# Wenri/taichi_3d_gaussian_splatting

Measured on AMD Instinct MI355X. Metric: fps fwd+bwd @1920x1080 (run as 1920x1088), 5e5 Gaussians, higher is better.
Workload: dtype f32; 1 GPU; cfg3_headline: synth(N=500000, 1920x1088, sigma0=0.02, sh_deg=3, seed 0), fwd+bwd, 1 view(s) per GPU per step, the 8 poses of BASELINE config 4 cycled (rank r, step k: pose (r + k) mod 8); points=500000, parallelism=view-parallel x1, 1 view(s) per rank per step, all-reduce per step, views_per_rank=1, poses_cycled=8, forward_sizing=predicted, rehearsal=False, backward_hook=True

## Files before the change

### taichi_3d_gaussian_splatting_amd/csrc/gs_api.hip

```cpp
#include "../../include/gs_channels.h"
#include "../../include/gs_sparse.h"
#include "gs_host.h"
#include "gs_sort_key.h"

#include <algorithm>
#include <atomic>
#include <chrono>
#include <cstring>
#include <cstdlib>

thread_local std::string g_last_error;

struct FrameBufs {
    DevBuf mask, ids, cam_index, rec, box, ntiles, depth_codes, offsets, keys_a, keys_b, vals_a, vals_b, tile_start, pose, tile_order, cuts, cut_mag;
    void release(int64_t* total)
    {
        DevBuf* all[] = { &mask, &ids, &cam_index, &rec, &box, &ntiles, &depth_codes, &offsets, &keys_a, &keys_b, &vals_a, &vals_b,
                          &tile_start, &pose, &tile_order, &cuts, &cut_mag };
        for (DevBuf* b : all) b->release(total);
    }
};

struct Frame {
    FrameBufs bufs;
    gs_frame_info info{};
    int depth_bits = 0;
    void* keys_sorted = nullptr;
    int key_bytes = 4;
    int32_t* vals_sorted = nullptr;
    bool live = false;
    int cut_cap = 0;
    int bwd_reference_order = 0;
    int n_objects = 0;
    bool rgb_only = false;
    bool max_tiles_known = false;
    uint32_t generation = 0;
    uint64_t bwd_serial = 0;
    int pending_slot = -1;
    int32_t pending_ticket = 0;
    hipStream_t pending_stream = nullptr;
};

int gs_prof_begin(GsProf* p, int kid, hipStream_t s)
{
    if (!p || !((p->mask >> kid) & 1ull)) return -1;
    GsProf::Rec r; r.kid = kid;
    hipEvent_t* ev[2] = { &r.a, &r.b };
    for (hipEvent_t* e : ev) {
        if (!p->spare.empty()) { *e = p->spare.back(); p->spare.pop_back(); }
        else if (hipEventCreate(e) != hipSuccess) return -1;
    }
    (void)hipEventRecord(r.a, s);
    p->recs.push_back(r);
    return (int)p->recs.size() - 1;
}

void gs_prof_end(GsProf* p, int rec, hipStream_t s)
{
    if (!p || rec < 0) return;
    (void)hipEventRecord(p->recs[rec].b, s);
}

extern "C" int gs_abi_version(void) { return GS_ABI_VERSION; }
extern "C" const char* gs_last_error(void) { return g_last_error.c_str(); }

extern "C" const char* gs_kernel_names(void)
{
    return "k_filter,k_scan_tiles_publish,k_project,k_keygen,k_sort_hist,"
           "k_sort_rowscan,k_sort_scatter,k_blend_fwd,k_blend_bwd_tile,k_bwd_points,k_sum_rows,k_tile_order,k_blend_bwd_repair";
}

extern "C" int gs_create(int32_t device, gs_ctx** out)
{
    if (!out) return fail(GS_ERR_INVALID_ARGUMENT, "gs_create: out is NULL");
    int count = 0;
    HIP_TRY(hipGetDeviceCount(&count));
    if (device < 0 || device >= count) return fail(GS_ERR_INVALID_ARGUMENT, "gs_create: no such HIP device");
    HIP_TRY(hipSetDevice(device));
    gs_ctx* c = new gs_ctx();
    c->device = device;
    hipError_t e = hipHostMalloc(reinterpret_cast<void**>(&c->host_counters), sizeof(GsCounters) * GS_COUNTER_SLOTS, hipHostMallocMapped | hipHostMallocCoherent);
    if (e != hipSuccess) { delete c; return fail(GS_ERR_HIP, std::string("hipHostMalloc: ") + hipGetErrorString(e)); }
    std::memset(c->host_counters, 0, sizeof(GsCounters) * GS_COUNTER_SLOTS);
    e = hipHostGetDevicePointer(reinterpret_cast<void**>(&c->host_counters_dev), c->host_counters, 0);
    if (e != hipSuccess) { (void)hipHostFree(c->host_counters); delete c; return fail(GS_ERR_HIP, std::string("hipHostGetDevicePointer: ") + hipGetErrorString(e)); }
    e = c->counters.ensure(sizeof(GsCounters), &c->device_bytes);
    if (e == hipSuccess) e = hipMemset(c->counters.p, 0, sizeof(GsCounters));
    if (e == hipSuccess) e = hipEventCreateWithFlags(&c->switch_event, hipEventDisableTiming);
    if (e != hipSuccess) { c->counters.release(&c->device_bytes); (void)hipHostFree(c->host_counters); delete c; return fail(GS_ERR_OUT_OF_MEMORY, "gs_create: counters"); }
    *out = c;
    return GS_OK;
}

extern "C" int gs_destroy(gs_ctx* c)
{
    if (!c) return GS_OK;
    (void)hipSetDevice(c->device);
    (void)hipDeviceSynchronize();
    for (Frame* f : c->frames) { f->bufs.release(&c->device_bytes); delete f; }
    DevBuf* all[] = { &c->block_counts, &c->block_offsets, &c->tile_block_sums, &c->hist, &c->scan_tmp, &c->first_hist,
                      &c->counters, &c->partial, &c->visited, &c->zero_row, &c->sums, &c->loss_ws, &c->order_hint, &c->pose_scratch,
                      &c->ch_partial, &c->ch_flags, &c->row_block_totals, &c->merge_tags, &c->merge_ids,
                      &c->knn_sort, &c->knn_hist, &c->knn_points, &c->knn_tree, &c->mix_records, &c->mix_sums, &c->mix_partial,
                      &c->mixg_queries, &c->mixg_partial, &c->mixg_sums, &c->mixg_x_partial, &c->mcmc_ws, &c->appearance_ws, &c->bilateral_ws, &c->depth_ws,
                      &c->geometry_ws };
    for (DevBuf* b : all) b->release(&c->device_bytes);
    for (ResampleTable* rt : c->resample_tables) { rt->buf.release(&c->device_bytes); delete rt; }
    for (GsProf::Rec& r : c->prof.recs) { (void)hipEventDestroy(r.a); (void)hipEventDestroy(r.b); }
    for (hipEvent_t e : c->prof.spare) (void)hipEventDestroy(e);
    if (c->switch_event) (void)hipEventDestroy(c->switch_event);
    if (c->host_counters) (void)hipHostFree(c->host_counters);
    delete c;
    return GS_OK;
}

extern "C" int gs_profile_enable(gs_ctx* c, uint64_t kernel_mask)
{
    if (!c) return fail(GS_ERR_INVALID_ARGUMENT, "gs_profile_enable: ctx is NULL");
    std::lock_guard<std::mutex> lock(c->mu);
    c->prof.mask = kernel_mask;
    return GS_OK;
}

extern "C" int gs_profile_read(gs_ctx* c, double* total_ms, int64_t* launches, int32_t n, int32_t reset)
{
    if (!c || !total_ms || !launches) return fail(GS_ERR_INVALID_ARGUMENT, "gs_profile_read: NULL argument");
    std::lock_guard<std::mutex> lock(c->mu);
    HIP_TRY(hipSetDevice(c->device));
    GsProf& p = c->prof;
    for (GsProf::Rec& r : p.recs) {
        HIP_TRY(hipEventSynchronize(r.b));
        float ms = 0.0f;
        HIP_TRY(hipEventElapsedTime(&ms, r.a, r.b));
        p.total_ms[r.kid] += ms; p.launches[r.kid] += 1;
        p.spare.push_back(r.a); p.spare.push_back(r.b);
    }
    p.recs.clear();
    for (int i = 0; i < n && i < KID_COUNT_; ++i) { total_ms[i] = p.total_ms[i]; launches[i] = p.launches[i]; }
    if (reset) for (int i = 0; i < KID_COUNT_; ++i) { p.total_ms[i] = 0.0; p.launches[i] = 0; }
    return GS_OK;
}

extern "C" int64_t gs_ctx_device_bytes(const gs_ctx* c) { return c ? c->device_bytes : 0; }
extern "C" int64_t gs_ctx_counter_wait_ns(const gs_ctx* c) { return c ? c->counter_wait_ns : 0; }
static gs_frame* ticket_of(int slot, uint32_t generation)
{
    return reinterpret_cast<gs_frame*>((uintptr_t)(((uint64_t)generation << 32) | (uint64_t)(uint32_t)(slot + 1)));
}

static Frame* resolve(gs_ctx* c, const gs_frame* h)
{
    const uint64_t v = (uint64_t)(uintptr_t)h;
    const uint32_t lo = (uint32_t)v, gen = (uint32_t)(v >> 32);
    if (lo == 0 || lo > c->frames.size()) return nullptr;
    Frame* f = c->frames[lo - 1];
    if (!f->live || f->generation != gen) return nullptr;
    return f;
}

static Frame* acquire_frame(gs_ctx* c, int* slot)
{
    for (size_t i = 0; i < c->frames.size(); ++i)
        if (!c->frames[i]->live) { Frame* f = c->frames[i]; f->live = true; f->generation += 1; if (f->generation == 0) f->generation = 1; *slot = (int)i; return f; }
    Frame* f = new Frame();
    f->live = true; f->generation = 1;
    c->frames.push_back(f);
    *slot = (int)c->frames.size() - 1;
    return f;
}

static void drop_frame(gs_ctx* c, Frame* f)
{
    if (!f || !f->live) return;
    if (f->pending_slot > 0) c->slots_busy &= ~(1ull << f->pending_slot);
    f->pending_slot = -1;
    f->live = false;
    for (size_t i = 0; i < c->frames.size(); ++i) if (c->frames[i] == f && c->transient == (int)i) c->transient = -1;
}

static Frame* begin_frame(gs_ctx* c, const gs_camera* cam, int T, int keep, int* slot)
{
    if (c->transient >= 0) drop_frame(c, c->frames[c->transient]);
    Frame* f = acquire_frame(c, slot);
    f->info = gs_frame_info{};
    f->bwd_serial = 0;
    f->info.kept_for_backward = keep ? 1 : 0;
    f->info.n_tiles = T; f->info.camera_height = cam->camera_height; f->info.camera_width = cam->camera_width;
    return f;
}

static void finish_frame(gs_ctx* c, Frame* f, int slot, int64_t N, int M, uint32_t K, int stages, gs_frame** frame_out)
{
    f->info.n_points = N; f->info.n_points_in_camera = M; f->info.n_keys = K;
    f->info.stages = stages;
    if (!f->info.kept_for_backward) c->transient = slot;
    *frame_out = ticket_of(slot, f->generation);
}

static GsFrameView frame_view(const Frame& f)
{
    const FrameBufs& B = f.bufs;
    const int T = f.info.n_tiles;
    GsFrameView v{};
    float4* rec = B.rec.as<float4>();
    v.PA = rec; v.PB = rec + 1; v.PC = rec + 2; v.PD = rec + 3;
    v.box = B.box.as<ushort4>(); v.ntiles = B.ntiles.as<int32_t>(); v.depth_codes = B.depth_codes.as<int32_t>(); v.offsets = B.offsets.as<uint32_t>();
    v.ids = B.ids.as<int32_t>(); v.cam_index = B.cam_index.as<int32_t>(); v.mask = B.mask.as<int8_t>(); v.pose = B.pose.as<GsPose>();
    v.T = T;
    int32_t* tiles = B.tile_start.as<int32_t>();
    v.tile_start = tiles; v.tile_end = tiles + T; v.tile_work = tiles + 2 * (size_t)T; v.tile_cut = tiles + 3 * (size_t)T;
    v.max_tiles = tiles + GS_TILE_INTS(T) - GS_TILE_SPARE_MAX_TILES;
    v.tile_ints = (int)GS_TILE_INTS(T);
    v.tile_order = B.tile_order.as<int32_t>(); v.n_heavy = v.tile_order + T;
    v.keys_sorted = f.keys_sorted; v.vals_sorted = f.vals_sorted;
    v.cuts = f.cut_cap > 0 ? B.cuts.as<float4>() : nullptr; v.cut_mag = B.cut_mag.as<float2>();
    return v;
}

static int waves_per_tile(int n_tiles);
static int bits_for(uint32_t v) { int b = 0; while (v) { ++b; v >>= 1; } return b < 1 ? 1 : b; }

static int read_counters(gs_ctx* c, hipStream_t s, int32_t ticket, int slot, GsCounters* out)
{
    volatile GsCounters* hc = c->host_counters + slot;
    const auto t0 = std::chrono::steady_clock::now();
    for (uint32_t spin = 0; hc->reserved != ticket; ++spin) {
        if ((spin & 0xfffu) == 0xfffu) {
            const hipError_t q = hipStreamQuery(s);
            if (q == hipSuccess) {
                if (hc->reserved != ticket) return fail(GS_ERR_HIP, "frame counters were not published");
                break;
            }
            if (q != hipErrorNotReady) return fail(GS_ERR_HIP, std::string("waiting for the frame counters: ") + hipGetErrorString(q));
            if (std::chrono::steady_clock::now() - t0 > std::chrono::seconds(30))
                return fail(GS_ERR_HIP, "timed out waiting for the frame counters");
        }
    }
    std::atomic_thread_fence(std::memory_order_acquire);
    c->counter_wait_ns += std::chrono::duration_cast<std::chrono::nanoseconds>(std::chrono::steady_clock::now() - t0).count();
    *out = c->host_counters[slot];
    if (out->bad_object_ids != 0)
        return fail(GS_ERR_INVALID_ARGUMENT, "point_object_id holds " + std::to_string(out->bad_object_ids) +
                                             " value(s) outside [0, n_objects) on valid rows");
    return GS_OK;
}

static int resolve_pending(gs_ctx* c, Frame* f)
{
    if (f->pending_slot <= 0) return GS_OK;
    HIP_TRY(hipSetDevice(c->device));
    GsCounters hc;
    const int rc = read_counters(c, f->pending_stream, f->pending_ticket, f->pending_slot, &hc);
    if (rc != GS_OK) { drop_frame(c, f); return rc; }
    c->slots_busy &= ~(1ull << f->pending_slot);
    f->pending_slot = -1;
    f->info.n_points_in_camera = hc.M;
    f->info.n_keys = hc.K;
    return GS_OK;
}

static int lookup(gs_ctx* c, const gs_frame* h, const char* who, bool pending, Frame** out)
{
    Frame* f = resolve(c, h);
    if (!f) return fail(GS_ERR_STATE, who, "not a live frame of this context");
    if (pending)
        if (const int rc = resolve_pending(c, f)) return rc;
    *out = f;
    return GS_OK;
}

static int check_geometry(const gs_camera* cam, const gs_config* cfg, const char* who, int* tiles_x, int* tiles_y)
{
    const int H = cam->camera_height, W = cam->camera_width;
    if (W <= 0 || H <= 0 || (!cfg->allow_partial_tiles && (W % GS_TILE != 0 || H % GS_TILE != 0)))
        return fail(GS_ERR_INVALID_ARGUMENT, who, "camera_width and camera_height must be positive multiples of 16 "
                                             "(or set gs_config.allow_partial_tiles)");
    *tiles_x = (W + GS_TILE - 1) / GS_TILE; *tiles_y = (H + GS_TILE - 1) / GS_TILE;
    if (*tiles_x > 65535 || *tiles_y > 65535) return fail(GS_ERR_INVALID_ARGUMENT, who, "image too large");
    return GS_OK;
}

static int check_scene(const gs_scene* sc, const gs_camera* cam, const char* who)
{
    const int64_t N = sc->n_points;
    if (N < 0 || N >= (int64_t)1 << 31) return fail(GS_ERR_INVALID_ARGUMENT, who, "n_points out of range");
    if (cam->n_objects <= 0) return fail(GS_ERR_INVALID_ARGUMENT, who, "n_objects must be >= 1");
    if (N > 0 && (!sc->point_cloud || !sc->point_cloud_features || !sc->point_invalid_mask || !sc->point_object_id))
        return fail(GS_ERR_INVALID_ARGUMENT, who, "NULL scene array");
    if (!cam->q_pointcloud_camera || !cam->t_pointcloud_camera || !cam->camera_intrinsics)
        return fail(GS_ERR_INVALID_ARGUMENT, who, "NULL camera array");
    if (((uintptr_t)sc->point_cloud_features & 15u) != 0)
        return fail(GS_ERR_INVALID_ARGUMENT, who, "point_cloud_features must be 16-byte aligned");
    return GS_OK;
}

static int check_forward_out(const gs_forward_out* out, const gs_config* cfg, int keep, const char* who)
{
    if (!out->rasterized_image) return fail(GS_ERR_INVALID_ARGUMENT, who, "rasterized_image is NULL");
    if (!cfg->rgb_only && (!out->rasterized_depth || !out->pixel_accumulated_alpha ||
                           !out->pixel_offset_of_last_effective_point || !out->pixel_valid_point_count))
        return fail(GS_ERR_INVALID_ARGUMENT, who, "an output is NULL although rgb_only is false");
    if (keep && cfg->rgb_only) return fail(GS_ERR_INVALID_ARGUMENT, who, "rgb_only frames cannot be kept for backward (RAST:478-484)");
    return GS_OK;
}

#define GS_FIRST_PASS_MAX_BLOCKS 4096
static bool sort_first_pass_enabled(int64_t rows)
{
    if ((rows + 255) / 256 > GS_FIRST_PASS_MAX_BLOCKS) return false;
    const char* e = getenv("GS_SORT_FIRST_PASS");
    return !(e && e[0] == '0');
}

#define GS_NARROW_KEYS_DEFAULT 1
enum NarrowKeys { NARROW_OFF, NARROW_ON, NARROW_REQUIRED };
static NarrowKeys sort_narrow_keys()
{
    const char* e = getenv("GS_SORT_NARROW_KEYS");
    if (!e || !e[0]) return GS_NARROW_KEYS_DEFAULT ? NARROW_ON : NARROW_OFF;
    if (e[0] == '0') return NARROW_OFF;
    return strcmp(e, "require") == 0 ? NARROW_REQUIRED : NARROW_ON;
}
static int check_required_key_class(const Frame* f)
{
    if (sort_narrow_keys() == NARROW_REQUIRED && f->key_bytes != 2)
        return fail(GS_ERR_STATE, "GS_SORT_NARROW_KEYS=require: the frame's sort keys are " + std::to_string(f->key_bytes) + " bytes wide");
    return GS_OK;
}

enum CounterWait { WAIT_NOW, WAIT_LATER, WAIT_FRAME };

static int run_project_stage(gs_ctx* c, Frame* f, const gs_scene* sc, const gs_camera* cam, const gs_config* cfg, hipStream_t s,
                             CounterWait wait, GsProjectArgs* pa_out, int* M_out, uint32_t* K_out)
{
    FrameBufs& B = f->bufs;
    const int64_t N = sc->n_points;
    const int T = f->info.n_tiles;
    const size_t nb = (size_t)((N + 255) / 256);
    const size_t Np = (size_t)(N > 0 ? N : 1);
    int rc = grow(c, "forward", { NEED(B.mask, Np), NEED(B.ids, 4 * Np), NEED(B.cam_index, 4 * Np),
                       NEED(B.rec, 64 * Np),
                       NEED(B.box, 8 * Np), NEED(B.ntiles, 4 * Np), NEED(B.depth_codes, 4 * Np), NEED(B.offsets, 4 * Np),
                       NEED(B.tile_start, 4 * GS_TILE_INTS(T)),
                       NEED(B.tile_order, 4 * GS_ORDER_INTS(T)),
                       NEED(B.pose, sizeof(GsPose) * (size_t)cam->n_objects),
                       NEED(c->block_counts, 4 * (nb + 1)), NEED(c->block_offsets, 4 * (nb + 1)),
                       NEED(c->tile_block_sums, 4 * (nb + 1)) });
    if (rc != GS_OK) return rc;
    const bool first_pass = wait == WAIT_LATER && sort_first_pass_enabled(N);
    if (first_pass && (rc = grow(c, "forward", { NEED(c->first_hist, 4 * gs_first_hist_elems(N)) })) != GS_OK) return rc;
    f->n_objects = cam->n_objects;

    GsProjectArgs pa{};
    pa.prof = &c->prof;
    pa.point_cloud = sc->point_cloud; pa.features = sc->point_cloud_features; pa.invalid = sc->point_invalid_mask;
    pa.object_id = sc->point_object_id; pa.N = N; pa.q_pc = cam->q_pointcloud_camera; pa.t_pc = cam->t_pointcloud_camera;
    pa.n_objects = cam->n_objects; pa.Kmat = cam->camera_intrinsics; pa.H = cam->camera_height; pa.W = cam->camera_width;
    pa.near_plane = cfg->near_plane; pa.far_plane = cfg->far_plane; pa.depth_scale = cfg->depth_to_sort_key_scale;
    pa.v = frame_view(*f);
    pa.block_counts = c->block_counts.as<int32_t>(); pa.block_offsets = c->block_offsets.as<int32_t>();
    pa.tile_block_sums = c->tile_block_sums.as<uint32_t>();
    pa.first_hist = first_pass ? c->first_hist.as<uint32_t>() : nullptr;
    pa.counters = c->counters.as<GsCounters>();
    int slot = 0;
    if (wait == WAIT_FRAME && N > 0) {
        const uint64_t free_slots = ~c->slots_busy;
        if (free_slots != 0ull) { slot = __builtin_ctzll(free_slots); c->slots_busy |= 1ull << slot; }
    }
    pa.host_mirror = c->host_counters_dev + slot; pa.ticket = ++c->ticket;
    if (c->ticket == 0x7fffffff) c->ticket = 0;
    gs_launch_project(pa, s, wait != WAIT_LATER);
    f->max_tiles_known = true;
    HIP_TRY(hipGetLastError());
    *pa_out = pa;
    *M_out = 0; *K_out = 0u;
    if (slot > 0) {
        f->pending_slot = slot; f->pending_ticket = pa.ticket; f->pending_stream = s;
        return GS_OK;
    }
    if (N > 0 && wait != WAIT_LATER) {
        GsCounters hc;
        if ((rc = read_counters(c, s, pa.ticket, 0, &hc)) != GS_OK) return rc;
        *M_out = hc.M; *K_out = hc.K;
    }
    return GS_OK;
}

static int run_records_stage(gs_ctx* c, Frame* f, const float* records, int64_t m, const gs_config* cfg, hipStream_t s,
                             GsProjectArgs* pa_out)
{
    FrameBufs& B = f->bufs;
    const int T = f->info.n_tiles;
    const size_t Mp = (size_t)(m > 0 ? m : 1);
    const size_t nb = (size_t)((m + 255) / 256);
    const int rc = grow(c, "forward", { NEED(B.rec, 64 * Mp), NEED(B.box, 8 * Mp), NEED(B.ntiles, 4 * Mp), NEED(B.depth_codes, 4 * Mp), NEED(B.offsets, 4 * Mp),
                             NEED(B.tile_start, 4 * GS_TILE_INTS(T)), NEED(B.tile_order, 4 * GS_ORDER_INTS(T)),
                             NEED(c->tile_block_sums, 4 * (nb + 1)) });
    if (rc != GS_OK) return rc;
    const bool first_pass = sort_first_pass_enabled(m);
    if (first_pass) if (const int rc2 = grow(c, "forward", { NEED(c->first_hist, 4 * gs_first_hist_elems(m)) })) return rc2;
    if (m > 0) HIP_TRY(hipMemcpyAsync(B.rec.p, records, (size_t)m * 64, hipMemcpyDeviceToDevice, s));
    GsProjectArgs pa{};
    pa.prof = &c->prof; pa.N = m; pa.H = f->info.camera_height; pa.W = f->info.camera_width; pa.depth_scale = cfg->depth_to_sort_key_scale;
    pa.v = frame_view(*f);
    pa.tile_block_sums = c->tile_block_sums.as<uint32_t>();
    pa.first_hist = first_pass ? c->first_hist.as<uint32_t>() : nullptr;
    pa.counters = c->counters.as<GsCounters>();
    pa.host_mirror = c->host_counters_dev; pa.ticket = ++c->ticket;
    if (c->ticket == 0x7fffffff) c->ticket = 0;
    gs_launch_boxes_from_records(pa, (int)m, s, false);
    f->max_tiles_known = false;
    HIP_TRY(hipGetLastError());
    *pa_out = pa;
    return GS_OK;
}

static int run_raster_stage(gs_ctx* c, Frame* f, const GsProjectArgs& pa, int64_t n_rows, int M_bound, uint32_t K_bound, int depth_bits,
                            const gs_config* cfg, const gs_forward_out* out, hipStream_t s, bool publish)
{
    FrameBufs& B = f->bufs;
    const int T = f->info.n_tiles, H = f->info.camera_height, W = f->info.camera_width, tiles_x = (W + GS_TILE - 1) / GS_TILE;
    static const int seg_env = []{ const char* e = getenv("GS_BWD_SEGMENTS"); return e ? (e[0] == '0' ? 0 : 1) : -1; }();
    const bool want_cuts = seg_env >= 0 ? seg_env == 1 : (int64_t)T * waves_per_tile(T) < 6144;
    int cut_cap = 0;
    if (want_cuts && f->info.kept_for_backward && !cfg->rgb_only && K_bound > 0) {
        cut_cap = (int)std::min<uint64_t>((uint64_t)K_bound / GS_SEG + (uint64_t)T + 2, 0x7fffffffu);
        if (const int rc = grow(c, "forward", { NEED(B.cuts, (size_t)cut_cap * 256 * sizeof(float4)), NEED(B.cut_mag, (size_t)cut_cap * 256 * sizeof(float2)) }))
            return rc;
    }
    f->cut_cap = cut_cap;
    const int tile_bits = bits_for((uint32_t)(T > 1 ? T - 1 : 1));
    uint32_t* const first_hist = depth_bits >= 8 ? pa.first_hist : nullptr;
    const int key_bytes = gs_key_bytes(depth_bits + tile_bits, depth_bits, first_hist != nullptr, sort_narrow_keys() != NARROW_OFF);
    if (depth_bits + tile_bits > 63) return fail(GS_ERR_INVALID_ARGUMENT, "sort key needs more than 63 bits");
    const size_t Kp = K_bound > 0 ? K_bound : 1;
    const size_t hist_elems = gs_sort_hist_elems(K_bound);
    if (const int rc = grow(c, "forward", { NEED(B.keys_a, (size_t)key_bytes * Kp), NEED(B.keys_b, (size_t)key_bytes * Kp), NEED(B.vals_a, 4 * Kp), NEED(B.vals_b, 4 * Kp),
                                 NEED(c->hist, 4 * hist_elems), NEED(c->scan_tmp, 4 * GS_SORT_DIGITS) }))
        return rc;

    GsBinArgs ba{};
    ba.prof = &c->prof;
    ba.N = n_rows; ba.M = M_bound; ba.K = K_bound; ba.counters = c->counters.as<GsCounters>();
    ba.tiles_x = tiles_x;
    ba.depth_bits = depth_bits; ba.key_bits = depth_bits + tile_bits;
    ba.v = frame_view(*f);
    ba.tile_block_sums = pa.tile_block_sums;
    ba.counters_rw = pa.counters; ba.host_mirror = publish ? pa.host_mirror : nullptr; ba.ticket = pa.ticket;
    ba.block_offsets = pa.block_offsets; ba.block_counts = pa.block_counts;
    ba.keys_a = B.keys_a.p; ba.keys_b = B.keys_b.p; ba.key_bytes = key_bytes;
    ba.vals_a = B.vals_a.as<int32_t>(); ba.vals_b = B.vals_b.as<int32_t>();
    ba.hist = c->hist.as<uint32_t>(); ba.scan_tmp = c->scan_tmp.as<uint32_t>();
    ba.first_hist = first_hist;
    ba.keys_sorted = &f->keys_sorted; ba.vals_sorted = &f->vals_sorted;
    gs_launch_binning(ba, s);
    HIP_TRY(hipGetLastError());

    GsBlendFwdArgs fa{};
    fa.prof = &c->prof;
    fa.H = H; fa.W = W; fa.tiles_x = tiles_x; fa.rgb_only = cfg->rgb_only;
    fa.v = frame_view(*f);
    fa.key_bytes = key_bytes; fa.depth_bits = depth_bits; fa.K = K_bound; fa.counters = ba.counters;
    fa.image = out->rasterized_image; fa.depth = out->rasterized_depth; fa.acc_alpha = out->pixel_accumulated_alpha;
    fa.last = out->pixel_offset_of_last_effective_point; fa.count = out->pixel_valid_point_count;
    fa.cut_cap = cut_cap;
    static const bool use_hint = []{ const char* e = getenv("GS_FWD_ORDER_HINT"); return !(e && e[0] == '0'); }();
    fa.order_hint = (use_hint && c->order_hint_T == T && T > 0) ? c->order_hint.as<int32_t>() : nullptr;
    gs_launch_blend_fwd(fa, s);
    HIP_TRY(hipGetLastError());
    f->depth_bits = depth_bits;
    f->key_bytes = key_bytes;
    f->info.sort_key_bits = depth_bits + tile_bits;
    return GS_OK;
}

static int run_forward_tail(gs_ctx* c, Frame* f, const GsProjectArgs& pa, int64_t n_rows, int M_known, const gs_config* cfg,
                            const gs_forward_out* out, hipStream_t s, int* M_out, uint32_t* K_out)
{
    static const bool predict = []{ const char* e = getenv("GS_PREDICT_SIZES"); return !(e && e[0] == '0'); }();
    const int T = f->info.n_tiles, H = f->info.camera_height, W = f->info.camera_width;
    int rc;
    f->info.sizing = GS_SIZING_EXACT;
    *M_out = 0; *K_out = 0u;
    if (n_rows == 0) {
        rc = run_raster_stage(c, f, pa, 0, 0, 0u, 1, cfg, out, s, false);
        return rc != GS_OK ? rc : check_required_key_class(f);
    }
    const int tile_bits = bits_for((uint32_t)(T > 1 ? T - 1 : 1));
    bool predicted = false;
    int bits_p = 0; uint32_t K_p = 0;
    if (predict && c->seen.valid && c->seen.H == H && c->seen.W == W) {
        bits_p = bits_for((uint32_t)(c->seen.max_code + c->seen.max_code / 4));
        const uint64_t want = (uint64_t)c->seen.K + c->seen.K / 4 + 4096;
        K_p = (uint32_t)std::min<uint64_t>(want, 0x7fffffffu);
        predicted = K_p > 0 && bits_p + tile_bits <= 63;
    }
    if (predicted) {
        if ((rc = run_raster_stage(c, f, pa, n_rows, M_known >= 0 ? M_known : (int)n_rows, K_p, bits_p, cfg, out, s, true)) != GS_OK) return rc;
    } else {
        gs_launch_publish(pa, (int)((n_rows + 255) / 256), s);
        HIP_TRY(hipGetLastError());
    }
    GsCounters hc;
    if ((rc = read_counters(c, s, pa.ticket, 0, &hc)) != GS_OK) return rc;
    if (hc.K >= (1u << 31)) return fail(GS_ERR_INVALID_ARGUMENT, "more than 2^31 sort pairs (tile ranges are int32, RAST:954-957)");
    const int bits = bits_for((uint32_t)(hc.max_depth_code > 0 ? hc.max_depth_code : 0));
    if (predicted && hc.K <= K_p && bits <= bits_p) {
        f->info.sizing = GS_SIZING_PREDICTED;
    } else {
        if (predicted) {
            HIP_TRY(hipMemsetAsync(pa.v.tile_start, 0, sizeof(int32_t) * (size_t)pa.v.tile_ints, s));
            f->max_tiles_known = false;
            f->info.sizing = GS_SIZING_REDONE;
        }
        if ((rc = run_raster_stage(c, f, pa, n_rows, hc.M, hc.K, bits, cfg, out, s, false)) != GS_OK) return rc;
    }
    if (!(c->seen.valid && c->seen.H == H && c->seen.W == W && hc.M == 0)) c->seen.max_code = hc.max_depth_code;
    c->seen.valid = true; c->seen.H = H; c->seen.W = W; c->seen.K = hc.K;
    *M_out = hc.M; *K_out = hc.K;
    return check_required_key_class(f);
}

extern "C" int gs_forward(gs_ctx* c, const gs_scene* sc, const gs_camera* cam, const gs_config* cfg,
                          const gs_forward_out* out, int32_t keep, gs_frame** frame_out, gs_stream stream_)
{
    if (!c || !sc || !cam || !cfg || !out || !frame_out) return fail(GS_ERR_INVALID_ARGUMENT, "gs_forward: NULL argument");
    int tiles_x = 0, tiles_y = 0, rc;
    if ((rc = check_geometry(cam, cfg, "gs_forward", &tiles_x, &tiles_y)) != GS_OK) return rc;
    if ((rc = check_scene(sc, cam, "gs_forward")) != GS_OK) return rc;
    if ((rc = check_forward_out(out, cfg, keep, "gs_forward")) != GS_OK) return rc;
    std::lock_guard<std::mutex> lock(c->mu);
    hipStream_t s;
    if ((rc = enter_call(c, stream_, &s)) != GS_OK) return rc;
    int slot = -1;
    Frame* f = begin_frame(c, cam, tiles_x * tiles_y, keep, &slot);
    GsProjectArgs pa{};
    int M = 0; uint32_t K = 0;
    rc = run_project_stage(c, f, sc, cam, cfg, s, WAIT_LATER, &pa, &M, &K);
    if (rc == GS_OK) rc = run_forward_tail(c, f, pa, sc->n_points, -1, cfg, out, s, &M, &K);
    if (rc != GS_OK) { drop_frame(c, f); return rc; }
    f->bwd_reference_order = cfg->bwd_reference_order;
    f->rgb_only = cfg->rgb_only != 0;
    finish_frame(c, f, slot, sc->n_points, M, K, GS_STAGE_PROJECT | GS_STAGE_RASTER, frame_out);
    return GS_OK;
}

static int copy_projection(const Frame* f, int M, float* records_out, int32_t* ids_out, hipStream_t s)
{
    HIP_TRY(hipMemcpyAsync(records_out, f->bufs.rec.p, (size_t)M * 64, hipMemcpyDeviceToDevice, s));
    if (ids_out) HIP_TRY(hipMemcpyAsync(ids_out, f->bufs.ids.p, (size_t)M * 4, hipMemcpyDeviceToDevice, s));
    return GS_OK;
}

extern "C" int gs_project_shard(gs_ctx* c, const gs_scene* sc, const gs_camera* cam, const gs_config* cfg,
                                float* records_out, int32_t* ids_out, int32_t keep, gs_frame** frame_out, gs_stream stream_)
{
    if (!c || !sc || !cam || !cfg || !frame_out) return fail(GS_ERR_INVALID_ARGUMENT, "gs_project_shard: NULL argument");
    if (sc->n_points > 0 && !records_out) return fail(GS_ERR_INVALID_ARGUMENT, "gs_project_shard: records_out is NULL");
    if (((uintptr_t)records_out & 15u) != 0) return fail(GS_ERR_INVALID_ARGUMENT, "gs_project_shard: records_out must be 16-byte aligned");
    int tiles_x = 0, tiles_y = 0, rc;
    if ((rc = check_geometry(cam, cfg, "gs_project_shard", &tiles_x, &tiles_y)) != GS_OK) return rc;
    if ((rc = check_scene(sc, cam, "gs_project_shard")) != GS_OK) return rc;
    std::lock_guard<std::mutex> lock(c->mu);
    hipStream_t s;
    if ((rc = enter_call(c, stream_, &s)) != GS_OK) return rc;
    int slot = -1;
    Frame* f = begin_frame(c, cam, tiles_x * tiles_y, keep, &slot);
    GsProjectArgs pa{};
    int M = 0; uint32_t K = 0;
    rc = run_project_stage(c, f, sc, cam, cfg, s, WAIT_NOW, &pa, &M, &K);
    if (rc == GS_OK && M > 0) rc = copy_projection(f, M, records_out, ids_out, s);
    if (rc != GS_OK) { drop_frame(c, f); return rc; }
    finish_frame(c, f, slot, sc->n_points, M, K, GS_STAGE_PROJECT, frame_out);
    return GS_OK;
}

extern "C" int gs_project_shard_begin(gs_ctx* c, const gs_scene* sc, const gs_camera* cam, const gs_config* cfg,
                                      int32_t keep, gs_frame** frame_out, gs_stream stream_)
{
    if (!c || !sc || !cam || !cfg || !frame_out) return fail(GS_ERR_INVALID_ARGUMENT, "gs_project_shard_begin: NULL argument");
    int tiles_x = 0, tiles_y = 0, rc;
    if ((rc = check_geometry(cam, cfg, "gs_project_shard_begin", &tiles_x, &tiles_y)) != GS_OK) return rc;
    if ((rc = check_scene(sc, cam, "gs_project_shard_begin")) != GS_OK) return rc;
    std::lock_guard<std::mutex> lock(c->mu);
    hipStream_t s;
    if ((rc = enter_call(c, stream_, &s)) != GS_OK) return rc;
    int slot = -1;
    Frame* f = begin_frame(c, cam, tiles_x * tiles_y, keep, &slot);
    GsProjectArgs pa{};
    int M = 0; uint32_t K = 0;
    rc = run_project_stage(c, f, sc, cam, cfg, s, WAIT_FRAME, &pa, &M, &K);
    if (rc != GS_OK) { drop_frame(c, f); return rc; }
    finish_frame(c, f, slot, sc->n_points, M, K, GS_STAGE_PROJECT, frame_out);
    return GS_OK;
}

extern "C" int gs_forward_projected(gs_ctx* c, const float* records, int64_t m, const gs_camera* cam, const gs_config* cfg,
                                    const gs_forward_out* out, int32_t keep, gs_frame** frame_out, gs_stream stream_)
{
    if (!c || !cam || !cfg || !out || !frame_out) return fail(GS_ERR_INVALID_ARGUMENT, "gs_forward_projected: NULL argument");
    if (m < 0 || m >= (int64_t)1 << 31) return fail(GS_ERR_INVALID_ARGUMENT, "gs_forward_projected: m out of range");
    if (m > 0 && !records) return fail(GS_ERR_INVALID_ARGUMENT, "gs_forward_projected: records is NULL");
    int tiles_x = 0, tiles_y = 0, rc;
    if ((rc = check_geometry(cam, cfg, "gs_forward_projected", &tiles_x, &tiles_y)) != GS_OK) return rc;
    if ((rc = check_forward_out(out, cfg, keep, "gs_forward_projected")) != GS_OK) return rc;
    std::lock_guard<std::mutex> lock(c->mu);
    hipStream_t s;
    if ((rc = enter_call(c, stream_, &s)) != GS_OK) return rc;
    int slot = -1;
    Frame* f = begin_frame(c, cam, tiles_x * tiles_y, keep, &slot);
    GsProjectArgs pa{};
    int M_seen = 0; uint32_t K = 0;
    rc = run_records_stage(c, f, records, m, cfg, s, &pa);
    if (rc == GS_OK) rc = run_forward_tail(c, f, pa, m, (int)m, cfg, out, s, &M_seen, &K);
    if (rc != GS_OK) { drop_frame(c, f); return rc; }
    f->bwd_reference_order = cfg->bwd_reference_order;
    finish_frame(c, f, slot, m, (int)m, K, GS_STAGE_RASTER, frame_out);
    return GS_OK;
}

extern "C" int gs_frame_get_info(gs_ctx* c, const gs_frame* h, gs_frame_info* info)
{
    if (!c || !info) return fail(GS_ERR_INVALID_ARGUMENT, "gs_frame_get_info: NULL argument");
    std::lock_guard<std::mutex> lock(c->mu);
    Frame* f;
    if (const int rc = lookup(c, h, "gs_frame_get_info", true, &f)) return rc;
    *info = f->info;
    return GS_OK;
}

static int64_t export_count(const Frame* f, gs_export what)
{
    const int64_t M = f->info.n_points_in_camera, K = f->info.n_keys, T = f->info.n_tiles, N = f->info.n_points;
    const bool proj = (f->info.stages & GS_STAGE_PROJECT) != 0, rast = (f->info.stages & GS_STAGE_RASTER) != 0;
    switch (what) {
    case GS_X_POINT_ID_IN_CAMERA_LIST: return proj ? M : -1;
    case GS_X_POINT_IN_CAMERA_MASK: return proj ? N : -1;
    case GS_X_POINT_ALPHA_AFTER_ACTIVATION: case GS_X_POINT_RADII: case GS_X_NUM_OVERLAP_TILES: case GS_X_POINT_DEPTH: return M;
    case GS_X_ACCUMULATED_NUM_OVERLAP_TILES: return rast ? M : -1;
    case GS_X_POINT_UV: return 2 * M;
    case GS_X_POINT_IN_CAMERA: case GS_X_POINT_COLOR: return 3 * M;
    case GS_X_POINT_UV_CONIC_AND_RESCALE: return 4 * M;
    case GS_X_RECORDS: return proj ? 16 * M : -1;
    case GS_X_SORT_KEY: case GS_X_POINT_OFFSET_WITH_SORT_KEY: return rast ? K : -1;
    case GS_X_TILE_POINTS_START: case GS_X_TILE_POINTS_END: return rast ? T : -1;
    default: return -1;
    }
}

extern "C" int64_t gs_frame_export_count(gs_ctx* c, const gs_frame* h, gs_export what)
{
    if (!c) return -1;
    std::lock_guard<std::mutex> lock(c->mu);
    Frame* f = resolve(c, h);
    if (f && resolve_pending(c, f) != GS_OK) return -1;
    return f ? export_count(f, what) : -1;
}

extern "C" int gs_frame_export(gs_ctx* c, const gs_frame* h, gs_export what, void* dst, gs_stream stream_)
{
    if (!c) return fail(GS_ERR_INVALID_ARGUMENT, "gs_frame_export: ctx is NULL");
    if (!dst) return fail(GS_ERR_INVALID_ARGUMENT, "gs_frame_export: dst is NULL");
    if (what < 0 || what >= GS_X_COUNT_) return fail(GS_ERR_INVALID_ARGUMENT, "gs_frame_export: unknown export id");
    std::lock_guard<std::mutex> lock(c->mu);
    Frame* f;
    int rc;
    if ((rc = lookup(c, h, "gs_frame_export", true, &f)) != GS_OK) return rc;
    if (export_count(f, what) < 0) return fail(GS_ERR_STATE, "gs_frame_export: this frame does not hold that stage");
    hipStream_t s;
    if ((rc = enter_call(c, stream_, &s)) != GS_OK) return rc;
    const GsFrameView v = frame_view(*f);
    if (what == GS_X_RECORDS) {
        if (f->info.n_points_in_camera > 0)
            HIP_TRY(hipMemcpyAsync(dst, v.PA, (size_t)f->info.n_points_in_camera * 64, hipMemcpyDeviceToDevice, s));
        return GS_OK;
    }
    GsExportArgs a{};
    a.what = (int)what; a.N = f->info.n_points; a.M = (int)f->info.n_points_in_camera; a.K = (uint32_t)f->info.n_keys;
    a.T = v.T; a.depth_bits = f->depth_bits; a.key_bytes = f->key_bytes; a.depth_codes = v.depth_codes;
    a.ids = v.ids; a.PA = v.PA; a.PB = v.PB; a.PC = v.PC; a.PD = v.PD;
    a.ntiles = v.ntiles; a.offsets = v.offsets;
    a.keys_sorted = v.keys_sorted; a.vals_sorted = v.vals_sorted;
    a.tile_start = v.tile_start; a.tile_end = v.tile_end; a.mask = v.mask;
    a.dst = dst;
    gs_launch_export(a, s);
    HIP_TRY(hipGetLastError());
    return GS_OK;
}

static int waves_per_tile(int n_tiles)
{
    int G = 1;
    if (const char* e = getenv("GS_BWD_WAVES_PER_TILE")) G = atoi(e);
    else if (n_tiles < 2000) G = 4;
    else if (n_tiles < 6144) G = 2;
    if (G != 1 && G != 2 && G != 4) G = 1;
    return G;
}

static bool bwd_prefill_enabled()
{
    const char* e = getenv("GS_BWD_PREFILL");
    return !(e && e[0] == '0');
}

static int prepare_backward_blend(gs_ctx* c, Frame* f, const float* grad_image, const float* acc_alpha, const int32_t* last,
                                  float* mag_image, float4* sums_out, int strict, hipStream_t stream, GsBackwardArgs* a_out)
{
    const uint32_t K = (uint32_t)f->info.n_keys;
    const int G = waves_per_tile(f->info.n_tiles);
    const size_t rows = (size_t)(K > 0 ? K : 1) * (size_t)G;
    const size_t flag_bytes = (rows + 15) / 16 * 16;
    hipError_t e = c->partial.ensure(rows * 12 * sizeof(float), &c->device_bytes);
    if (e != hipSuccess) return fail(GS_ERR_OUT_OF_MEMORY, "backward: partial-sum buffer");
    const size_t Mp = (size_t)(f->info.n_points_in_camera > 0 ? f->info.n_points_in_camera : 1);
    const size_t cap_before = c->visited.cap;
    e = c->visited.ensure(flag_bytes + Mp + 16, &c->device_bytes);
    if (e != hipSuccess) return fail(GS_ERR_OUT_OF_MEMORY, "backward: visited buffer");
    if (c->visited.cap != cap_before || c->visit_gen == 255) {
        HIP_TRY(hipMemsetAsync(c->visited.p, 0, c->visited.cap, stream));
        c->visit_gen = 0;
    }
    c->visit_gen += 1;
    c->bwd_serial += 1;
    c->touched_offset = flag_bytes;
    f->bwd_serial = c->bwd_serial;
    if (!c->zero_row.p) {
        if (c->zero_row.ensure(64, &c->device_bytes) != hipSuccess) return fail(GS_ERR_OUT_OF_MEMORY, "backward: zero row");
        HIP_TRY(hipMemsetAsync(c->zero_row.p, 0, c->zero_row.cap, stream));
    }
    if (c->order_hint_T != f->info.n_tiles) {
        c->order_hint_T = 0;
        if (c->order_hint.ensure(4 * (size_t)(f->info.n_tiles > 0 ? f->info.n_tiles : 1), &c->device_bytes) != hipSuccess)
            return fail(GS_ERR_OUT_OF_MEMORY, "backward: tile order buffer");
    }
    GsBackwardArgs a{};
    a.prof = &c->prof;
    a.order_hint = c->order_hint.as<int32_t>();
    a.N = f->info.n_points; a.M = (int)f->info.n_points_in_camera; a.K = K;
    a.H = f->info.camera_height; a.W = f->info.camera_width;
    a.tiles_x = (a.W + GS_TILE - 1) / GS_TILE;
    a.v = frame_view(*f);
    a.grad_image = grad_image; a.acc_alpha = acc_alpha; a.last = last;
    a.partial = c->partial.as<float>();
    a.visited = c->visited.as<uint8_t>();
    a.G = G;
    a.item_cap = f->cut_cap;
    static const int heavy_env = []{ const char* e = getenv("GS_BWD_SPLIT_HEAVY"); if (e && e[0] == '0') return 0;
                                     const char* x = getenv("GS_BWD_HEAVY_X2"); return x ? atoi(x) : -1; }();
    a.heavy_factor_x2 = heavy_env >= 0 ? heavy_env : 4;
    a.strict = strict ? 1 : 0;
    a.gen = c->visit_gen;
    a.touched = c->visited.as<uint8_t>() + flag_bytes;
    a.zero_row = c->zero_row.as<float4>();
    a.max_tiles_hint = f->max_tiles_known ? a.v.max_tiles : nullptr;
    a.sums = sums_out;
    a.mag_image = mag_image;
    a.live_sums = bwd_prefill_enabled() ? 1 : 0;
    *a_out = a;
    return GS_OK;
}

static int prepare_backward_points(const Frame* f, const gs_scene* sc, const gs_camera* cam, const gs_config* cfg,
                                   int32_t sh_band, const gs_backward_out* out, const float4* sums, GsBackwardArgs* a)
{
    a->N = f->info.n_points; a->M = (int)f->info.n_points_in_camera;
    a->v = frame_view(*f);
    a->sums = const_cast<float4*>(sums);
    a->point_cloud = sc->point_cloud; a->features = sc->point_cloud_features; a->object_id = sc->point_object_id;
    a->Kmat = cam->camera_intrinsics;
    a->sh_band = sh_band; a->f_color = cfg->grad_color_factor; a->f_high = cfg->grad_high_order_color_factor;
    a->f_s = cfg->grad_s_factor; a->f_q = cfg->grad_q_factor; a->f_alpha = cfg->grad_alpha_factor;
    a->grad_pc = out->grad_pointcloud; a->grad_feat = out->grad_pointcloud_features; a->grad_uv = out->grad_viewspace;
    a->mag = out->magnitude_grad_viewspace;
    a->n_affected = out->num_affected_pixels;
    a->hook_gpc = out->hook_grad_point_in_camera; a->hook_gfeat = out->hook_grad_pointfeatures_in_camera;
    a->hook_guv = out->hook_grad_viewspace; a->hook_mag = out->hook_magnitude_grad_viewspace;
    a->hook_ids = out->hook_point_id_in_camera_list; a->hook_ntiles = out->hook_num_overlap_tiles;
    a->hook_depth = out->hook_point_depth; a->hook_uv = out->hook_point_uv_in_camera;
    if (const gs_controller_accumulators* ca = out->controller) {
        if (!ca->accumulated_num_in_camera || !ca->accumulated_num_pixels || !ca->accumulated_view_space_position_gradients ||
            !ca->accumulated_view_space_position_gradients_avg || !ca->accumulated_position_gradients || !ca->accumulated_position_gradients_norm)
            return fail(GS_ERR_INVALID_ARGUMENT, "backward: controller accumulators must all be given");
        a->c_num_in_camera = ca->accumulated_num_in_camera; a->c_num_pixels = ca->accumulated_num_pixels;
        a->c_vs_grad = ca->accumulated_view_space_position_gradients; a->c_vs_grad_avg = ca->accumulated_view_space_position_gradients_avg;
        a->c_pos_grad = ca->accumulated_position_gradients; a->c_pos_grad_norm = ca->accumulated_position_gradients_norm;
    }
    return GS_OK;
}

static void launch_backward_blend(gs_ctx* c, const GsBackwardArgs& a, hipStream_t s)
{
    gs_launch_backward_blend(a, s);
    if (a.v.T > 0 && a.K > 0) c->order_hint_T = a.v.T;
}

static int check_backward_points_args(const Frame* f, const gs_scene* sc, const gs_camera* cam, const gs_backward_out* out, const char* who,
                                      bool pose_only = false)
{
    if (sc->n_points > 0 && !pose_only && (!out->grad_pointcloud || !out->grad_pointcloud_features))
        return fail(GS_ERR_INVALID_ARGUMENT, who, "grad_pointcloud / grad_pointcloud_features are mandatory");
    if (sc->n_points != f->info.n_points || cam->camera_height != f->info.camera_height || cam->camera_width != f->info.camera_width)
        return fail(GS_ERR_INVALID_ARGUMENT, who, "scene/camera do not match the frame");
    if (((uintptr_t)out->grad_pointcloud_features & 15u) != 0 || ((uintptr_t)sc->point_cloud_features & 15u) != 0)
        return fail(GS_ERR_INVALID_ARGUMENT, who, "feature arrays must be 16-byte aligned");
    if (out->hook_grad_pointfeatures_in_camera && ((uintptr_t)out->hook_grad_pointfeatures_in_camera & 15u) != 0)
        return fail(GS_ERR_INVALID_ARGUMENT, who, "hook feature array must be 16-byte aligned");
    return GS_OK;
}

static int backward_impl(gs_ctx* c, gs_frame* h, const gs_scene* sc, const gs_camera* cam, const gs_config* cfg,
                         const float* grad_image, const gs_backward_extra* extra, const float* acc_alpha, const int32_t* last,
                         int32_t sh_band, const gs_backward_out* out, gs_stream stream_)
{
    if (!c || !sc || !cam || !cfg || !out) return fail(GS_ERR_INVALID_ARGUMENT, "gs_backward: NULL argument");
    if (!grad_image || !acc_alpha || !last) return fail(GS_ERR_INVALID_ARGUMENT, "gs_backward: NULL image-sized input");
    std::lock_guard<std::mutex> lock(c->mu);
    Frame* f;
    int rc;
    if ((rc = lookup(c, h, "gs_backward", false, &f)) != GS_OK) return rc;
    if (!f->info.kept_for_backward) return fail(GS_ERR_STATE, "gs_backward: frame was not kept for backward");
    if (f->info.stages != (GS_STAGE_PROJECT | GS_STAGE_RASTER)) return fail(GS_ERR_STATE, "gs_backward: frame does not come from gs_forward");
    const bool pose = out->grad_q_pointcloud_camera || out->grad_t_pointcloud_camera;
    if (pose && (!out->grad_q_pointcloud_camera || !out->grad_t_pointcloud_camera))
        return fail(GS_ERR_INVALID_ARGUMENT, "gs_backward: grad_q_pointcloud_camera and grad_t_pointcloud_camera must be given together");
    const bool points = !pose || out->grad_pointcloud || out->grad_pointcloud_features;
    if (pose && cam->n_objects != f->n_objects)
        return fail(GS_ERR_INVALID_ARGUMENT, "gs_backward: camera n_objects does not match the frame's forward");
    if ((rc = check_backward_points_args(f, sc, cam, out, "gs_backward", !points)) != GS_OK) return rc;
    hipStream_t s;
    if ((rc = enter_call(c, stream_, &s)) != GS_OK) return rc;
    if (c->sums.ensure((size_t)(f->info.n_points_in_camera > 0 ? f->info.n_points_in_camera : 1) * 48, &c->device_bytes) != hipSuccess)
        return fail(GS_ERR_OUT_OF_MEMORY, "gs_backward: per-point sums buffer");
    if (pose && c->pose_scratch.ensure(gs_pose_scratch_size((int)f->info.n_points_in_camera, f->n_objects), &c->device_bytes) != hipSuccess)
        return fail(GS_ERR_OUT_OF_MEMORY, "gs_backward: pose-gradient scratch");
    GsBackwardArgs a{};
    if ((rc = prepare_backward_blend(c, f, grad_image, acc_alpha, last, out->magnitude_grad_viewspace_on_image, c->sums.as<float4>(), cfg->bwd_reference_order, s, &a)) != GS_OK) return rc;
    if ((rc = prepare_backward_points(f, sc, cam, cfg, sh_band, out, c->sums.as<float4>(), &a)) != GS_OK) return rc;
    if (extra) {
        a.grad_depth = extra->grad_rasterized_depth; a.depth = extra->rasterized_depth;
        a.grad_alpha = extra->grad_pixel_accumulated_alpha;
        a.aux = 1;
        a.v.cuts = nullptr;
    }
    a.prefill = points && a.grad_feat && a.v.T > 0 && a.K > 0 && bwd_prefill_enabled();
    launch_backward_blend(c, a, s);
    if (points) gs_launch_backward_points(a, s);
    if (pose) gs_launch_pose_grad(a, f->n_objects, c->pose_scratch.p, out->grad_q_pointcloud_camera, out->grad_t_pointcloud_camera, s);
    HIP_TRY(hipGetLastError());
    return GS_OK;
}

extern "C" int gs_backward(gs_ctx* c, gs_frame* h, const gs_scene* sc, const gs_camera* cam, const gs_config* cfg,
                           const float* grad_image, const float* acc_alpha, const int32_t* last,
                           int32_t sh_band, const gs_backward_out* out, gs_stream stream_)
{
    return backward_impl(c, h, sc, cam, cfg, grad_image, nullptr, acc_alpha, last, sh_band, out, stream_);
}

extern "C" int gs_backward_ex(gs_ctx* c, gs_frame* h, const gs_scene* sc, const gs_camera* cam, const gs_config* cfg,
                              const float* grad_image, const gs_backward_extra* extra, const float* acc_alpha, const int32_t* last,
                              int32_t sh_band, const gs_backward_out* out, gs_stream stream_)
{
    if (extra && extra->grad_rasterized_depth && !extra->rasterized_depth)
        return fail(GS_ERR_INVALID_ARGUMENT, "gs_backward_ex: grad_rasterized_depth needs rasterized_depth (the forward's output)");
    if (extra && !extra->grad_rasterized_depth && !extra->grad_pixel_accumulated_alpha) extra = nullptr;
    return backward_impl(c, h, sc, cam, cfg, grad_image, extra, acc_alpha, last, sh_band, out, stream_);
}

extern "C" int gs_backward_projected(gs_ctx* c, gs_frame* h, const float* grad_image, const float* acc_alpha, const int32_t* last,
                                     float* splat_sums_out, float* mag_image, gs_stream stream_)
{
    if (!c) return fail(GS_ERR_INVALID_ARGUMENT, "gs_backward_projected: ctx is NULL");
    if (!grad_image || !acc_alpha || !last) return fail(GS_ERR_INVALID_ARGUMENT, "gs_backward_projected: NULL image-sized input");
    if (((uintptr_t)splat_sums_out & 15u) != 0) return fail(GS_ERR_INVALID_ARGUMENT, "gs_backward_projected: splat_sums_out must be 16-byte aligned");
    std::lock_guard<std::mutex> lock(c->mu);
    Frame* f;
    int rc;
    if ((rc = lookup(c, h, "gs_backward_projected", false, &f)) != GS_OK) return rc;
    if (!f->info.kept_for_backward) return fail(GS_ERR_STATE, "gs_backward_projected: frame was not kept for backward");
    if (!(f->info.stages & GS_STAGE_RASTER)) return fail(GS_ERR_STATE, "gs_backward_projected: frame holds no raster stage");
    if (f->info.n_points_in_camera > 0 && !splat_sums_out) return fail(GS_ERR_INVALID_ARGUMENT, "gs_backward_projected: splat_sums_out is NULL");
    hipStream_t s;
    if ((rc = enter_call(c, stream_, &s)) != GS_OK) return rc;
    GsBackwardArgs a{};
    if ((rc = prepare_backward_blend(c, f, grad_image, acc_alpha, last, mag_image, reinterpret_cast<float4*>(splat_sums_out), f->bwd_reference_order, s, &a)) != GS_OK) return rc;
    launch_backward_blend(c, a, s);
    HIP_TRY(hipGetLastError());
    return GS_OK;
}

extern "C" int gs_backward_shard(gs_ctx* c, gs_frame* h, const gs_scene* sc, const gs_camera* cam, const gs_config* cfg,
                                 const float* splat_sums, int32_t sh_band, const gs_backward_out* out, gs_stream stream_)
{
    if (!c || !sc || !cam || !cfg || !out) return fail(GS_ERR_INVALID_ARGUMENT, "gs_backward_shard: NULL argument");
    if (((uintptr_t)splat_sums & 15u) != 0) return fail(GS_ERR_INVALID_ARGUMENT, "gs_backward_shard: splat_sums must be 16-byte aligned");
    std::lock_guard<std::mutex> lock(c->mu);
    Frame* f;
    int rc;
    if ((rc = lookup(c, h, "gs_backward_shard", true, &f)) != GS_OK) return rc;
    if (!f->info.kept_for_backward) return fail(GS_ERR_STATE, "gs_backward_shard: frame was not kept for backward");
    if (!(f->info.stages & GS_STAGE_PROJECT)) return fail(GS_ERR_STATE, "gs_backward_shard: frame holds no projection stage");
    if (f->info.n_points_in_camera > 0 && !splat_sums) return fail(GS_ERR_INVALID_ARGUMENT, "gs_backward_shard: splat_sums is NULL");
    if (out->grad_q_pointcloud_camera || out->grad_t_pointcloud_camera)
        return fail(GS_ERR_INVALID_ARGUMENT, "gs_backward_shard: pose gradients are not available on the staged (Gaussian-parallel) path; "
                                             "use gs_backward");
    if ((rc = check_backward_points_args(f, sc, cam, out, "gs_backward_shard")) != GS_OK) return rc;
    hipStream_t s;
    if ((rc = enter_call(c, stream_, &s)) != GS_OK) return rc;
    GsBackwardArgs a{};
    a.prof = &c->prof;
    if ((rc = prepare_backward_points(f, sc, cam, cfg, sh_band, out, reinterpret_cast<const float4*>(splat_sums), &a)) != GS_OK) return rc;
    gs_launch_backward_points(a, s);
    HIP_TRY(hipGetLastError());
    return GS_OK;
}

static int channels_enter(gs_ctx* c, const gs_frame* h, int32_t n_channels, const char* who, gs_stream stream_, Frame** f_out, hipStream_t* s_out)
{
    if (n_channels < 1 || n_channels > GS_CHANNELS_MAX)
        return fail(GS_ERR_INVALID_ARGUMENT, who, "n_channels must be in 1.." + std::to_string(GS_CHANNELS_MAX));
    Frame* f;
    if (const int rc = lookup(c, h, who, true, &f)) return rc;
    if (f->info.stages != (GS_STAGE_PROJECT | GS_STAGE_RASTER))
        return fail(GS_ERR_INVALID_ARGUMENT, who, "the frame must come from gs_forward (frames made from records or shards are not supported)");
    if (f->rgb_only) return fail(GS_ERR_INVALID_ARGUMENT, who, "an rgb_only frame has no pixel_offset_of_last_effective_point");
    if (const int rc = enter_call(c, stream_, s_out)) return rc;
    *f_out = f;
    return GS_OK;
}

static GsChannelsArgs channels_args(const Frame* f, int32_t n_channels, const int32_t* last)
{
    GsChannelsArgs a{};
    a.v = frame_view(*f);
    a.M = (int)f->info.n_points_in_camera; a.K = (uint32_t)f->info.n_keys;
    a.H = f->info.camera_height; a.W = f->info.camera_width; a.tiles_x = (a.W + GS_TILE - 1) / GS_TILE;
    a.C = n_channels; a.last = last;
    return a;
}

extern "C" int gs_channels_forward(gs_ctx* c, const gs_frame* h, const float* values, int32_t n_channels,
                                   const int32_t* last, float* out, gs_stream stream_)
{
    if (!c || !h || !values || !last || !out) return fail(GS_ERR_INVALID_ARGUMENT, "gs_channels_forward: NULL argument");
    std::lock_guard<std::mutex> lock(c->mu);
    Frame* f;
    hipStream_t s;
    if (const int rc = channels_enter(c, h, n_channels, "gs_channels_forward", stream_, &f, &s)) return rc;
    GsChannelsArgs a = channels_args(f, n_channels, last);
    a.values = values; a.out = out;
    if (a.K == 0u || a.M <= 0) {
        HIP_TRY(hipMemsetAsync(out, 0, (size_t)a.H * (size_t)a.W * (size_t)n_channels * sizeof(float), s));
        return GS_OK;
    }
    gs_launch_channels_fwd(a, s);
    HIP_TRY(hipGetLastError());
    return GS_OK;
}

extern "C" int gs_channels_backward(gs_ctx* c, const gs_frame* h, const float* grad_out, int32_t n_channels,
                                    const int32_t* last, float* grad_values, gs_stream stream_)
{
    if (!c || !h || !grad_out || !last || !grad_values) return fail(GS_ERR_INVALID_ARGUMENT, "gs_channels_backward: NULL argument");
    std::lock_guard<std::mutex> lock(c->mu);
    Frame* f;
    hipStream_t s;
    if (const int rc = channels_enter(c, h, n_channels, "gs_channels_backward", stream_, &f, &s)) return rc;
    GsChannelsArgs a = channels_args(f, n_channels, last);
    a.grad_out = grad_out; a.grad_values = grad_values;
    if (f->info.n_points > 0) HIP_TRY(hipMemsetAsync(grad_values, 0, (size_t)f->info.n_points * (size_t)n_channels * sizeof(float), s));
    if (a.K == 0u || a.M <= 0) return GS_OK;
    const size_t rows = (size_t)a.K * 4, row_flags = (rows + 15) / 16 * 16;
    if (const int rc = grow(c, "gs_channels_backward", { NEED(c->ch_partial, rows * (size_t)gs_channels_chunk(n_channels) * sizeof(float)),
                                 NEED(c->ch_flags, row_flags + (size_t)a.M) }))
        return rc;
    a.partial = c->ch_partial.as<float>(); a.flags = c->ch_flags.as<uint8_t>(); a.touched = a.flags + row_flags;
    a.flag_bytes = row_flags + (size_t)a.M;
    HIP_TRY(gs_launch_channels_bwd(a, s));
    HIP_TRY(hipGetLastError());
    return GS_OK;
}

extern "C" int gs_touched_rows(gs_ctx* c, const gs_frame* h, int32_t* ids_out, int64_t capacity, int32_t* count_out, gs_stream stream_)
{
    if (!c || !h || !ids_out || !count_out) return fail(GS_ERR_INVALID_ARGUMENT, "gs_touched_rows: NULL argument");
    std::lock_guard<std::mutex> lock(c->mu);
    Frame* f;
    int rc;
    if ((rc = lookup(c, h, "gs_touched_rows", false, &f)) != GS_OK) return rc;
    if (!(f->info.stages & GS_STAGE_PROJECT))
        return fail(GS_ERR_INVALID_ARGUMENT, "gs_touched_rows: the frame holds no projection stage (frames made from records are not supported)");
    if (capacity < f->info.n_points_in_camera) return fail(GS_ERR_INVALID_ARGUMENT, "gs_touched_rows: capacity is below the frame's n_points_in_camera");
    if (f->bwd_serial == 0) return fail(GS_ERR_STATE, "gs_touched_rows: no backward has run on this frame");
    if (f->bwd_serial != c->bwd_serial)
        return fail(GS_ERR_STATE, "gs_touched_rows: another backward has run on this context since the frame's (the list describes the latest one only)");
    const int M = (int)f->info.n_points_in_camera;
    const int M_eff = (f->info.n_keys > 0 && f->info.n_tiles > 0) ? M : 0;
    HIP_TRY(hipSetDevice(c->device));
    if ((rc = grow(c, "gs_touched_rows", { NEED(c->row_block_totals, (size_t)(gs_rows_blocks(M_eff) + 1) * sizeof(uint32_t)) })) != GS_OK) return rc;
    hipStream_t s;
    if ((rc = enter_call(c, stream_, &s)) != GS_OK) return rc;
    gs_launch_touched_rows(c->visited.as<uint8_t>() + c->touched_offset, c->visit_gen, frame_view(*f).ids, M_eff,
                           c->row_block_totals.as<uint32_t>(), ids_out, capacity, count_out, s);
    HIP_TRY(hipGetLastError());
    return GS_OK;
}

extern "C" int gs_frame_heavy_tiles(gs_ctx* c, const gs_frame* h, int32_t* n_out, gs_stream stream_)
{
    if (!c || !n_out) return fail(GS_ERR_INVALID_ARGUMENT, "gs_frame_heavy_tiles: NULL argument");
    std::lock_guard<std::mutex> lock(c->mu);
    Frame* f;
    int rc;
    if ((rc = lookup(c, h, "gs_frame_heavy_tiles", false, &f)) != GS_OK) return rc;
    if (f->bwd_serial == 0) return fail(GS_ERR_STATE, "gs_frame_heavy_tiles: no backward has run on this frame");
    if (!(f->info.stages & GS_STAGE_RASTER) || f->info.n_tiles <= 0 || f->info.n_keys <= 0 || !f->bufs.tile_order.p) { n_out[0] = n_out[1] = 0; return GS_OK; }
    hipStream_t s;
    if ((rc = enter_call(c, stream_, &s)) != GS_OK) return rc;
    HIP_TRY(hipMemcpyAsync(n_out, frame_view(*f).n_heavy, 2 * sizeof(int32_t), hipMemcpyDeviceToHost, s));
    HIP_TRY(hipStreamSynchronize(s));
    return GS_OK;
}

extern "C" int gs_frame_release(gs_ctx* c, gs_frame* h)
{
    if (!c || !h) return GS_OK;
    std::lock_guard<std::mutex> lock(c->mu);
    Frame* f = resolve(c, h);
    if (!f) return fail(GS_ERR_STATE, "gs_frame_release: not a live frame of this context (already released?)");
    drop_frame(c, f);
    return GS_OK;
}

#ifdef GS_STATS
__device__ unsigned long long gs_stats_counters[32];
__device__ unsigned long long gs_stats_wave_times[2 * 65536];
extern "C" int gs_debug_wave_times_read(unsigned long long* out, int n_waves)
{
    if (hipDeviceSynchronize() != hipSuccess) return -2;
    if (n_waves > 65536) n_waves = 65536;
    if (hipMemcpyFromSymbol(out, HIP_SYMBOL(gs_stats_wave_times), sizeof(unsigned long long) * 2 * (size_t)n_waves) != hipSuccess) return -2;
    return 0;
}
extern "C" int gs_debug_stats_read(unsigned long long* out32, int reset)
{
    if (hipDeviceSynchronize() != hipSuccess) return -2;
    if (hipMemcpyFromSymbol(out32, HIP_SYMBOL(gs_stats_counters), sizeof(unsigned long long) * 32) != hipSuccess) return -2;
    if (reset) {
        unsigned long long z[32] = {0};
        if (hipMemcpyToSymbol(HIP_SYMBOL(gs_stats_counters), z, sizeof(z)) != hipSuccess) return -2;
    }
    return 0;
}
#endif
```

### taichi_3d_gaussian_splatting_amd/csrc/gs_common.h

```cpp
#pragma once
#include <hip/hip_runtime.h>
#include <stdint.h>

#define GS_TILE_SZ 16

#define gs_ballot(pred) __builtin_amdgcn_ballot_w64(pred)

#ifdef GS_STATS
extern __device__ unsigned long long gs_stats_counters[32];
extern __device__ unsigned long long gs_stats_wave_times[2 * 65536];
#endif
#if defined(GS_STATS) && GS_STATS >= 2
#define GS_STAT(i, n) do { const unsigned long long gs_stat_n = (unsigned long long)(n); if (threadIdx.x % 64 == 0) atomicAdd(&gs_stats_counters[i], gs_stat_n); } while (0)
#else
#define GS_STAT(i, n) do { } while (0)
#endif
#define GS_REC(ptr, i) (ptr)[(size_t)(i) * 4]
#define GS_BOUNDARY_TILES 3
#define GS_ALPHA_EPS 0.00392156862745098f
#define GS_ALPHA_MAX 0.99f
#define GS_T_STOP 0.0001f
#define GS_NFEAT 56
#ifndef GS_SEG
#define GS_SEG 512
#endif
#ifndef GS_CUT_MIN_LEN
#define GS_CUT_MIN_LEN 512
#endif
#define GS_HEAVY_CAP 1024
#define GS_TILE_INTS(T) (4 * (size_t)(T) + 4)
#define GS_TILE_SPARE_MAX_TILES 3
#define GS_ORDER_INTS(T) ((size_t)(T) + 4 + GS_HEAVY_CAP + 4 + GS_HEAVY_CAP)
#define GS_ORDER_REDO_OFFSET (4 + GS_HEAVY_CAP + 4)

struct GsPose {
    float R[9];
    float t[3];
    float origin_fwd[3];
    float origin_bwd[3];
    float q_cp[4];
    float pad[2];
};

__device__ __forceinline__ void gs_pose_grad_chain(const GsPose& P, const float g[15], float gq[4], float gt[3])
{
    float dW[9], dt[3];
#pragma unroll
    for (int k = 0; k < 9; ++k) dW[k] = g[k];
    const float* dO = g + 12;
#pragma unroll
    for (int j = 0; j < 3; ++j) {
#pragma unroll
        for (int i = 0; i < 3; ++i) dW[3 * j + i] -= P.t[j] * dO[i];
        dt[j] = g[9 + j] - ((P.R[3 * j] * dO[0] + P.R[3 * j + 1] * dO[1]) + P.R[3 * j + 2] * dO[2]);
    }
    const float x = P.q_cp[0], y = P.q_cp[1], z = P.q_cp[2], w = P.q_cp[3];
    float gx = 2.0f * (y * (dW[1] + dW[3]) + z * (dW[2] + dW[6]) + w * (dW[7] - dW[5])) - 4.0f * x * (dW[4] + dW[8]);
    float gy = 2.0f * (x * (dW[1] + dW[3]) + w * (dW[2] - dW[6]) + z * (dW[5] + dW[7])) - 4.0f * y * (dW[0] + dW[8]);
    float gz = 2.0f * (w * (dW[3] - dW[1]) + x * (dW[2] + dW[6]) + y * (dW[5] + dW[7])) - 4.0f * z * (dW[0] + dW[4]);
    float gw = 2.0f * (z * (dW[3] - dW[1]) + y * (dW[2] - dW[6]) + x * (dW[7] - dW[5]));
    const float nrm = sqrtf(x * x + y * y + z * z + w * w);
    const float ux = x / nrm, uy = y / nrm, uz = z / nrm, nw = w / nrm;
    const float vx = P.origin_bwd[0], vy = P.origin_bwd[1], vz = P.origin_bwd[2];
    const float hx = -dt[0], hy = -dt[1], hz = -dt[2];
    const float hv = hx * vx + hy * vy + hz * vz, uh = ux * hx + uy * hy + uz * hz, uv = ux * vx + uy * vy + uz * vz;
    const float uu = ux * ux + uy * uy + uz * uz, ww = nw * nw;
    const float gnx = -2.0f * hv * ux + 2.0f * uh * vx + 2.0f * uv * hx + 2.0f * nw * (vy * hz - vz * hy);
    const float gny = -2.0f * hv * uy + 2.0f * uh * vy + 2.0f * uv * hy + 2.0f * nw * (vz * hx - vx * hz);
    const float gnz = -2.0f * hv * uz + 2.0f * uh * vz + 2.0f * uv * hz + 2.0f * nw * (vx * hy - vy * hx);
    const float gnw = 2.0f * nw * hv + 2.0f * (hx * (uy * vz - uz * vy) + hy * (uz * vx - ux * vz) + hz * (ux * vy - uy * vx));
    const float ng = ux * gnx + uy * gny + uz * gnz + nw * gnw;
    gx += (gnx - ux * ng) / nrm; gy += (gny - uy * ng) / nrm; gz += (gnz - uz * ng) / nrm; gw += (gnw - nw * ng) / nrm;
    gq[0] = -gx; gq[1] = -gy; gq[2] = -gz; gq[3] = gw;
    gt[0] = (ww - uu) * hx + 2.0f * uh * ux + 2.0f * nw * (hy * uz - hz * uy);
    gt[1] = (ww - uu) * hy + 2.0f * uh * uy + 2.0f * nw * (hz * ux - hx * uz);
    gt[2] = (ww - uu) * hz + 2.0f * uh * uz + 2.0f * nw * (hx * uy - hy * ux);
}

struct GsCounters {
    int32_t M;
    uint32_t K;
    int32_t max_depth_code;
    int32_t reserved;
    int32_t bad_object_ids;
    int32_t pad[3];
};

__device__ __forceinline__ void gs_publish_counters(GsCounters* __restrict__ counters, uint32_t K, volatile GsCounters* host_mirror, int32_t ticket)
{
    counters->K = K;
    host_mirror->M = counters->M;
    host_mirror->K = K;
    host_mirror->max_depth_code = counters->max_depth_code;
    host_mirror->bad_object_ids = counters->bad_object_ids;
    __threadfence_system();
    host_mirror->reserved = ticket;
    __threadfence_system();
    counters->max_depth_code = 0;
    counters->bad_object_ids = 0;
}

__device__ __forceinline__ float gs_expf(float x)
{
    x = x < -86.0f ? -86.0f : x;
    x = x > 88.0f ? 88.0f : x;
    float fx = x * 1.44269504088896341f;
    float n = (fx + 12582912.0f) - 12582912.0f;
    float r = __builtin_fmaf(n, -0.693359375f, x);
    r = __builtin_fmaf(n, 2.12194440e-4f, r);
    float z = r * r;
    float p = 1.9875691500E-4f;
    p = __builtin_fmaf(p, r, 1.3981999507E-3f);
    p = __builtin_fmaf(p, r, 8.3334519073E-3f);
    p = __builtin_fmaf(p, r, 4.1665795894E-2f);
    p = __builtin_fmaf(p, r, 1.6666665459E-1f);
    p = __builtin_fmaf(p, r, 5.0000001201E-1f);
    float y = __builtin_fmaf(p, z, r);
    y = y + 1.0f;
    int32_t bits = __float_as_int(y) + (((int32_t)n) << 23);
    return __int_as_float(bits);
}

__device__ __forceinline__ float gs_exp_blend(float x)
{
    x = __builtin_amdgcn_fmed3f(x, -86.0f, 88.0f);
    const float L = 1.44269504088896341f;
    const float t = x * L;
    const float m = t + 12582912.0f;
    const float n = m - 12582912.0f;
    const float f = __builtin_fmaf(x, L, -n);
    float q = 0.0013264712179079652f;
    q = __builtin_fmaf(q, f, 0.009671511128544807f);
    q = __builtin_fmaf(q, f, 0.05550733581185341f);
    q = __builtin_fmaf(q, f, 0.24022242426872253f);
    q = __builtin_fmaf(q, f, 0.6931470036506653f);
    const float p = __builtin_fmaf(q, f, 1.0f);
    return __uint_as_float(__float_as_uint(p) + (__float_as_uint(m) << 23));
}

__device__ __forceinline__ float gs_sigmoid(float x) { return 1.0f / (1.0f + gs_expf(-x)); }

template <int R, int K, int C>
__device__ __forceinline__ void gs_mm(const float* A, const float* B, float* Cout)
{
#pragma unroll
    for (int i = 0; i < R; ++i)
#pragma unroll
        for (int j = 0; j < C; ++j) {
            float acc = A[i * K] * B[j];
#pragma unroll
            for (int t = 1; t < K; ++t) acc = acc + A[i * K + t] * B[t * C + j];
            Cout[i * C + j] = acc;
        }
}

__device__ __forceinline__ void gs_tile_box(float u, float v, float radii, int tiles_u, int tiles_v, int box[4])
{
    radii = radii > 1.0f ? radii : 1.0f;
    float min_u = u - radii; min_u = min_u > 0.0f ? min_u : 0.0f;
    float max_u = u + radii;
    float min_v = v - radii; min_v = min_v > 0.0f ? min_v : 0.0f;
    float max_v = v + radii;
    int a = (int)floorf(min_u / 16.0f); a = a < tiles_u ? a : tiles_u;
    int b = (int)floorf(max_u / 16.0f) + 1; b = b > a + 1 ? b : a + 1; b = b < tiles_u ? b : tiles_u;
    int c = (int)floorf(min_v / 16.0f); c = c < tiles_v ? c : tiles_v;
    int d = (int)floorf(max_v / 16.0f) + 1; d = d > c + 1 ? d : c + 1; d = d < tiles_v ? d : tiles_v;
    box[0] = a; box[1] = b; box[2] = c; box[3] = d;
}

template <int CTRL, int ROW_MASK = 0xf, int BANK_MASK = 0xf, bool BOUND = true>
__device__ __forceinline__ float gs_dpp(float v)
{
    return __int_as_float(__builtin_amdgcn_update_dpp(0, __float_as_int(v), CTRL, ROW_MASK, BANK_MASK, BOUND));
}

#define GS_DPP11(ctrl)                                                                              \
    asm volatile("s_nop 1\n\t"                                                                      \
                 "v_add_f32_dpp %0, %0, %0 " ctrl "\n\t"                                            \
                 "v_add_f32_dpp %1, %1, %1 " ctrl "\n\t"                                            \
                 "v_add_f32_dpp %2, %2, %2 " ctrl "\n\t"                                            \
                 "v_add_f32_dpp %3, %3, %3 " ctrl "\n\t"                                            \
                 "v_add_f32_dpp %4, %4, %4 " ctrl "\n\t"                                            \
                 "v_add_f32_dpp %5, %5, %5 " ctrl "\n\t"                                            \
                 "v_add_f32_dpp %6, %6, %6 " ctrl "\n\t"                                            \
                 "v_add_f32_dpp %7, %7, %7 " ctrl "\n\t"                                            \
                 "v_add_f32_dpp %8, %8, %8 " ctrl "\n\t"                                            \
                 "v_add_f32_dpp %9, %9, %9 " ctrl "\n\t"                                            \
                 "v_add_f32_dpp %10, %10, %10 " ctrl "\n\t"                                         \
                 : "+v"(v[0]), "+v"(v[1]), "+v"(v[2]), "+v"(v[3]), "+v"(v[4]), "+v"(v[5]), "+v"(v[6]), \
                   "+v"(v[7]), "+v"(v[8]), "+v"(v[9]), "+v"(v[10]))

__device__ __forceinline__ void gs_wave_sum11_row3(float (&v)[11])
{
    GS_DPP11("quad_perm:[1,0,3,2] row_mask:0xf bank_mask:0xf");
    GS_DPP11("quad_perm:[2,3,0,1] row_mask:0xf bank_mask:0xf");
    GS_DPP11("row_half_mirror row_mask:0xf bank_mask:0xf");
    GS_DPP11("row_mirror row_mask:0xf bank_mask:0xf");
    GS_DPP11("row_bcast:15 row_mask:0xa bank_mask:0xf");
    GS_DPP11("row_bcast:31 row_mask:0xc bank_mask:0xf");
    asm volatile("s_nop 1");
}

__device__ __forceinline__ int gs_wave_sum_i(int v)
{
#pragma unroll
    for (int o = 32; o > 0; o >>= 1) v += __shfl_xor(v, o, 64);
    return v;
}

__device__ __forceinline__ float gs_wave_sum_f(float v)
{
#pragma unroll
    for (int o = 1; o < 64; o <<= 1) v += __shfl_xor(v, o, 64);
    return v;
}

__device__ __forceinline__ int gs_wave_max_i(int v)
{
#pragma unroll
    for (int o = 32; o > 0; o >>= 1) { int w = __shfl_xor(v, o, 64); v = v > w ? v : w; }
    return v;
}

__device__ __forceinline__ uint32_t gs_wave_scan_incl(uint32_t v, int lane)
{
#pragma unroll
    for (int o = 1; o < 64; o <<= 1) { const uint32_t t = __shfl_up(v, o, 64); if (lane >= o) v += t; }
    return v;
}
template <typename T> __device__ __forceinline__ void gs_block_put(T* ws, int wave, int lane, T v) { if (lane == 0) ws[wave] = v; }
__device__ __forceinline__ void gs_block_scan_put(uint32_t* ws, int wave, int lane, uint32_t incl) { if (lane == 63) ws[wave] = incl; }
template <int NW, typename T> __device__ __forceinline__ T gs_block_sum(const T* ws) { if constexpr (NW == 1) return ws[0]; else return gs_block_sum<NW - 1>(ws) + ws[NW - 1]; }
template <int NW> __device__ __forceinline__ int gs_block_max(const int* ws) { if constexpr (NW == 1) return ws[0]; else return max(gs_block_max<NW / 2>(ws), gs_block_max<NW / 2>(ws + NW / 2)); }
__device__ __forceinline__ uint32_t gs_block_scan_excl(const uint32_t* ws, int wave, uint32_t incl, uint32_t v)
{
    uint32_t woff = 0;
    for (int w = 0; w < wave; ++w) woff += ws[w];
    return woff + incl - v;
}
template <int NW>
__device__ __forceinline__ int gs_block_rank(bool pred, int* s_wave, int* total)
{
    const unsigned long long b = gs_ballot(pred);
    const int lane = threadIdx.x & 63, w = threadIdx.x >> 6;
    if (lane == 0) s_wave[w] = __popcll(b);
    __syncthreads();
    int before = 0, all = 0;
#pragma unroll
    for (int i = 0; i < NW; ++i) { const int c = s_wave[i]; before += i < w ? c : 0; all += c; }
    __syncthreads();
    *total = all;
    return before + __popcll(b & ((1ull << lane) - 1ull));
}
template <int NT, typename T> __device__ __forceinline__ T gs_sum_of_blocks_before(const T* __restrict__ counts, int block)
{
    T pre = 0;
    for (int j = threadIdx.x; j < block; j += NT) pre += counts[j];
    return (T)gs_wave_sum_i((int)pre);
}

enum GsKernelId { KID_FILTER = 0, KID_PUBLISH, KID_PROJECT, KID_KEYGEN,
                  KID_SORT_HIST, KID_SORT_ROWSCAN, KID_SORT_SCATTER, KID_BLEND_FWD,
                  KID_BLEND_BWD, KID_BWD_POINTS, KID_SUM_ROWS, KID_TILE_ORDER, KID_BLEND_BWD_REPAIR, KID_COUNT_ };
struct GsProf;
int gs_prof_begin(GsProf* p, int kid, hipStream_t s);
void gs_prof_end(GsProf* p, int rec, hipStream_t s);
#define GS_TIMED(prof, kid, stream, ...)                     \
    do {                                                     \
        int rec__ = gs_prof_begin((prof), (kid), (stream));  \
        __VA_ARGS__;                                         \
        gs_prof_end((prof), rec__, (stream));                \
    } while (0)

struct GsFrameView {
    float4 *PA, *PB, *PC, *PD;
    ushort4* box; int32_t* ntiles;
    int32_t* depth_codes;
    uint32_t* offsets;
    int32_t* ids; int32_t* cam_index; int8_t* mask; GsPose* pose;
    int T;
    int32_t *tile_start, *tile_end;
    int32_t* tile_work;
    int32_t* tile_cut;
    int32_t* max_tiles;
    int tile_ints;
    int32_t* tile_order;
    int32_t* n_heavy;
    const void* keys_sorted; const int32_t* vals_sorted;
    float4* cuts; float2* cut_mag;
};

struct GsProjectArgs {
    GsProf* prof;
    const float* point_cloud; float* features; const int8_t* invalid; const int32_t* object_id;
    int64_t N; const float* q_pc; const float* t_pc; int n_objects; const float* Kmat;
    int H, W; float near_plane, far_plane, depth_scale;
    GsFrameView v;
    int32_t* block_counts; int32_t* block_offsets; uint32_t* tile_block_sums;
    uint32_t* first_hist;
    GsCounters* counters;
    GsCounters* host_mirror; int32_t ticket;
};
void gs_launch_project(const GsProjectArgs& a, hipStream_t s, bool publish);
void gs_launch_publish(const GsProjectArgs& a, int n_blocks, hipStream_t s);
void gs_launch_boxes_from_records(const GsProjectArgs& a, int M, hipStream_t s, bool publish);

struct GsBinArgs {
    GsProf* prof;
    int64_t N; int M; uint32_t K; const GsCounters* counters; int tiles_x; int depth_bits; int key_bits;
    GsFrameView v;
    const uint32_t* tile_block_sums;
    GsCounters* counters_rw; GsCounters* host_mirror; int32_t ticket;
    const int32_t *block_offsets, *block_counts;
    void *keys_a, *keys_b; int32_t *vals_a, *vals_b;
    int key_bytes;
    uint32_t* hist;
    uint32_t* first_hist;
    uint32_t* scan_tmp;
    void** keys_sorted; int32_t** vals_sorted;
};
void gs_launch_binning(const GsBinArgs& a, hipStream_t s);
size_t gs_sort_hist_elems(uint32_t K);
size_t gs_first_hist_elems(int64_t rows);
#define GS_SORT_DIGITS 256

struct GsBlendFwdArgs {
    GsProf* prof;
    int H, W, tiles_x; int rgb_only;
    GsFrameView v;
    int key_bytes, depth_bits; uint32_t K; const GsCounters* counters;
    float* image; float* depth; float* acc_alpha; int32_t* last; int32_t* count;
    int cut_cap;
    const int32_t* order_hint;
};
void gs_launch_blend_fwd(const GsBlendFwdArgs& a, hipStream_t s);

struct GsBackwardArgs {
    GsProf* prof;
    int64_t N; int M; uint32_t K; int H, W, tiles_x;
    GsFrameView v;
    int32_t* order_hint;
    const float* grad_image; const float* acc_alpha; const int32_t* last;
    const float* grad_depth; const float* depth; const float* grad_alpha; int aux;
    int G;
    int item_cap;
    int heavy_factor_x2;
    int strict;
    float* partial;
    uint8_t* visited;
    uint8_t gen;
    uint8_t* touched;
    const float4* zero_row;
    const int32_t* max_tiles_hint;
    float4* sums;
    const float* point_cloud; const float* features; const int32_t* object_id; const float* Kmat;
    int sh_band; float f_color, f_high, f_s, f_q, f_alpha;
    float* grad_pc; float* grad_feat; float* grad_uv; float* mag; float* mag_image; int32_t* n_affected;
    int prefill;
    int live_sums;
    float* hook_gpc; float* hook_gfeat; float* hook_guv; float* hook_mag;
    int32_t* hook_ids; int32_t* hook_ntiles; float* hook_depth; float* hook_uv;
    int32_t* c_num_in_camera; int32_t* c_num_pixels; float* c_vs_grad; float* c_vs_grad_avg; float* c_pos_grad; float* c_pos_grad_norm;
};
void gs_launch_backward_blend(const GsBackwardArgs& a, hipStream_t s);
void gs_launch_backward_points(const GsBackwardArgs& a, hipStream_t s);
size_t gs_pose_scratch_size(int M, int n_objects);
void gs_launch_pose_grad(const GsBackwardArgs& a, int n_objects, void* scratch, float* grad_q, float* grad_t, hipStream_t s);

struct GsChannelsArgs {
    GsFrameView v;
    int M; uint32_t K; int H, W, tiles_x; int C;
    const int32_t* last;
    const float* values; float* out;
    const float* grad_out; float* grad_values;
    float* partial; uint8_t* flags; uint8_t* touched; size_t flag_bytes;
};
int gs_channels_chunk(int C);
void gs_launch_channels_fwd(const GsChannelsArgs& a, hipStream_t s);
hipError_t gs_launch_channels_bwd(const GsChannelsArgs& a, hipStream_t s);

struct GsExportArgs { int what; int64_t N; int M; uint32_t K; int T; int depth_bits; int key_bytes;
    const int32_t* depth_codes;
    const int32_t* ids; const float4 *PA, *PB, *PC, *PD; const int32_t* ntiles; const uint32_t* offsets;
    const void* keys_sorted; const int32_t* vals_sorted; const int32_t *tile_start, *tile_end; const int8_t* mask; void* dst; };
void gs_launch_export(const GsExportArgs& a, hipStream_t s);

struct GsLossImage { const float* p; long long sc, sy, sx; int clamp; };
size_t gs_loss_maps_size(int H, int W);
size_t gs_loss_partials_floats(int H, int W);
void gs_launch_loss_forward(const GsLossImage& X, const GsLossImage& Y, int H, int W, float lambda, float* maps, float* partials, float* terms,
                            hipStream_t s);
void gs_launch_loss_backward(const GsLossImage& X, const GsLossImage& Y, int H, int W, float lambda, const float* maps, const float* upstream,
                             const GsLossImage& G, hipStream_t s);
size_t gs_loss_weighted_partials_floats(int H, int W);
void gs_launch_loss_weighted_forward(const GsLossImage& X, const GsLossImage& Y, const float* weight, int H, int W, float lambda, float* maps,
                                     float* partials, float* terms, hipStream_t s);
void gs_launch_loss_weighted_backward(const GsLossImage& X, const GsLossImage& Y, const float* weight, int H, int W, float lambda,
                                      const float* maps, const float* terms, const float* upstream, const GsLossImage& G, hipStream_t s);
void gs_launch_adam(float* param, const float* grad, float* m, float* v, int64_t n, float lr, float beta1, float beta2, float eps,
                    int64_t step, hipStream_t s);
__device__ __forceinline__ void gs_adam_update(float& p, const float g, float& m_io, float& v_io, const float lr, const float beta1,
                                               const float beta2, const float eps, const float bias1, const float bias2_sqrt)
{
    const float m = beta1 * m_io + (1.0f - beta1) * g;
    const float v = beta2 * v_io + (1.0f - beta2) * (g * g);
    m_io = m; v_io = v;
    const float denom = sqrtf(v) / bias2_sqrt + eps;
    p = p - (lr / bias1) * (m / denom);
}
void gs_adam_bias(float beta1, float beta2, int64_t step, float* bias1, float* bias2_sqrt);
int gs_rows_blocks(int M);
void gs_launch_touched_rows(const uint8_t* touched, uint8_t gen, const int32_t* ids_in, int M, uint32_t* block_totals,
                            int32_t* ids_out, int64_t capacity, int32_t* count_out, hipStream_t s);
void gs_launch_adam_rows(float* param, const float* grad, float* m, float* v, int64_t n_rows, int row_len, const int32_t* ids,
                         const int32_t* count, int64_t max_count, float lr, float beta1, float beta2, float eps, int64_t step, hipStream_t s);
void gs_launch_pack_rows(const float* grad_features, const float* grad_pointcloud, int64_t n_rows, const int32_t* ids, const int32_t* count,
                         int64_t max_count, float* packed_out, hipStream_t s);
size_t gs_merge_tag_bytes(int64_t n_rows);
void gs_launch_merge_rows(const float* packed, const int32_t* counts, int n_lists, int64_t list_stride, int64_t n_rows, float* grad_features_out,
                          float* grad_pointcloud_out, int32_t* union_ids_out, int64_t union_capacity, int32_t* union_count_out, uint8_t* tag,
                          int32_t* ids_all, uint32_t* block_totals, hipStream_t s);
size_t gs_knn_sort_bytes(int64_t n);
size_t gs_knn_hist_bytes(int64_t n);
size_t gs_knn_points_bytes(int64_t n);
size_t gs_knn_tree_bytes(int64_t n);
void gs_launch_knn(const float* xyz, const int8_t* invalid, int64_t n, int k, float* d2_out, int32_t* idx_out,
                   void* sort_ws, void* hist_ws, void* pts_ws, void* tree_ws, hipStream_t s);
size_t gs_mix_record_bytes(int64_t n_points);
size_t gs_mix_sum_bytes(int64_t n_points);
size_t gs_mix_partial_bytes(int64_t n_points, int64_t n_q);
void gs_launch_mixture(const float* point_cloud, const float* features, const int8_t* invalid, int64_t n_points, const float* queries,
                       int64_t n_q, int fourier, const float* centre, float* out, void* record_ws, void* sum_ws, void* partial_ws, hipStream_t s);
const double* gs_launch_mixture_records(const float* point_cloud, const float* features, const int8_t* invalid, int64_t n_points,
                                        int fourier, const float* centre, void* record_ws, void* sum_ws, int64_t* n_pad_out, hipStream_t s);
void gs_launch_mix_total(double* block_sums, int64_t n_blocks, hipStream_t s);
size_t gs_mixg_query_bytes(int64_t n_q);
size_t gs_mixg_partial_bytes(int64_t n_points, int64_t n_q);
size_t gs_mixg_sum_bytes(int64_t n_points, int64_t n_q);
size_t gs_mixg_x_partial_bytes(int64_t n_points, int64_t n_x);
void gs_launch_mixture_grad(const float* point_cloud, const float* features, const int8_t* invalid, int64_t n_points, const float* queries,
                            int64_t n_q, int fourier, const float* centre, const float* log_density, const float* grad_out,
                            float* grad_point_cloud, float* grad_features, float* grad_x, void* record_ws, void* sum_ws, void* query_ws,
                            void* partial_ws, void* gsum_ws, void* x_partial_ws, hipStream_t s);
#define GS_RS_MAX_TAPS 18
#define GS_RS_MAX_SPAN 524
struct GsResampleAxis { const int32_t* start; const int32_t* count; const float* weight; int taps; };
void gs_launch_image_resample(const void* src, int src_format, int channels, int H_in, int W_in, int64_t pitch_bytes, GsResampleAxis ax,
                              GsResampleAxis ay, int h_out, int w_out, float* dst, int dst_channels, hipStream_t s);
struct GsBakeTransform { float m[9]; float t[3]; float q[4]; float log_scale; float sh[84]; };
void gs_launch_scene_bake(const float* xyz_in, const float* feat_in, int64_t n, const GsBakeTransform& A, float* xyz_out, float* feat_out,
                          int64_t row_offset, hipStream_t s);
void gs_launch_frame_to_u8(const float* src, int mode, int h, int w, uint8_t* dst, int64_t pitch, const uint8_t* gt, int gt_channels,
                           int64_t gt_pitch, int64_t* sse, hipStream_t s);
void gs_launch_reg_value(const float* feat, const int8_t* invalid, int64_t N, float* workspace, float* out, hipStream_t s);
void gs_launch_reg_grad(const float* feat, const int8_t* invalid, int64_t N, const float* value_and_count, const float* upstream,
                        float* grad, hipStream_t s);

template <bool IN_CAMERA = true>
__device__ __forceinline__ void gs_controller_add(int64_t n, int32_t npix, float mag, float g0, float g1, float g2,
                                                  int32_t* num_in_camera, int32_t* num_pixels, float* vs_grad, float* vs_grad_avg,
                                                  float* pos_grad, float* pos_grad_norm)
{
    if constexpr (IN_CAMERA) num_in_camera[n] += 1;
    num_pixels[n] += npix;
    vs_grad[n] += mag;
    const float avg = mag / (float)npix;
    vs_grad_avg[n] += (avg != avg) ? 0.0f : avg;
    pos_grad[3 * n] += g0; pos_grad[3 * n + 1] += g1; pos_grad[3 * n + 2] += g2;
    pos_grad_norm[n] += sqrtf(g0 * g0 + g1 * g1 + g2 * g2);
}

#include "../../include/gs_rasterizer.h"
void gs_launch_density_select(const gs_scene& scene, const gs_controller_accumulators& acc, const int32_t* ids, const int32_t* npix,
                              const float* depth, const float* mag, int64_t M, int remove_floaters, const gs_density_config& cfg,
                              const gs_density_plan& plan, hipStream_t s);
void gs_launch_density_apply(const gs_density_scene& scene, const gs_density_config& cfg, const gs_density_plan& plan, uint64_t seed,
                             uint32_t call_index, hipStream_t s);
void gs_launch_controller_accumulate(const int32_t* ids, const int32_t* npix, const float* mag, const float* gpc, int64_t M, int64_t N,
                                     const gs_controller_accumulators& acc, hipStream_t s);
size_t gs_density_scratch_size(int64_t N);

struct gs_mcmc_config;
struct gs_mcmc_plan;
void gs_launch_mcmc_noise(float* pc, const float* feat, const int8_t* mask, int64_t N, float noise_scale, float gate_k, float gate_x0,
                          uint64_t seed, uint32_t step_index, hipStream_t s);
void gs_launch_mcmc_regulariser(const float* feat, const int8_t* mask, int64_t N, float lambda_opacity, float lambda_scale,
                                const float* upstream, float* grad, float* value_and_count, void* ws, hipStream_t s);
void gs_launch_mcmc_relocate(const gs_density_scene& scene, float* const moments[4], const gs_mcmc_config& cfg, const gs_mcmc_plan& plan,
                             uint64_t seed, uint32_t call_index, hipStream_t s);
size_t gs_mcmc_scratch_size(int64_t N);
size_t gs_mcmc_reg_ws_size(int64_t N);

void gs_launch_vq_assign(const float* x, int64_t ldx, int64_t N, int dim, const float* cb, int64_t ldc, int K, int32_t* labels, float* dist,
                         void* scratch, hipStream_t s);
void gs_launch_vq_update(const float* x, int64_t ldx, int64_t N, int dim, const float* weights, const int32_t* labels, float* cb, int64_t ldc,
                         int K, int32_t* counts, double* weight_sums, hipStream_t s);
size_t gs_vq_scratch_size(int64_t n_rows, int n_codes, int dim);

size_t gs_appearance_ws_size(int H, int W);
void gs_launch_appearance_apply(const GsLossImage& X, const float* M, int H, int W, const GsLossImage& C, hipStream_t s);
void gs_launch_appearance_backward(const GsLossImage& X, const GsLossImage& G, const float* M, int H, int W, const GsLossImage& GI,
                                   float* grad_transform, void* ws, hipStream_t s);
void gs_launch_appearance_moments(const GsLossImage& X, const GsLossImage& Y, const float* weight, int H, int W, double* moments, void* ws,
                                  hipStream_t s);
size_t gs_bilateral_ws_size(int Gx, int Gy, int L);
void gs_launch_bilateral_slice(const GsLossImage& X, const float* grid, int Gx, int Gy, int L, int H, int W, const GsLossImage& C, hipStream_t s);
void gs_launch_bilateral_backward(const GsLossImage& X, const GsLossImage& G, const float* grid, int Gx, int Gy, int L, int H, int W,
                                  const GsLossImage& GI, float* grad_grid, void* ws, hipStream_t s);
void gs_launch_bilateral_tv(const float* grid, int Gx, int Gy, int L, float weight, float* grad_grid, float* value, hipStream_t s);
void gs_launch_depth_resample(const void* src, int src_format, int H_in, int W_in, int64_t pitch_bytes, float depth_scale, GsResampleAxis ax,
                              GsResampleAxis ay, int h_out, int w_out, float min_coverage, float* dst, hipStream_t s);
size_t gs_depth_ws_size(int H, int W);
void gs_launch_depth_loss_forward(const float* D, const float* Z, const float* wt, const float* wp, int H, int W, int flags, float* terms, void* ws,
                                  hipStream_t s);
void gs_launch_depth_loss_backward(const float* D, const float* Z, const float* wt, const float* wp, int H, int W, int flags, const float* terms,
                                   const float* upstream, float* G, hipStream_t s);

size_t gs_geometry_ws_size(int H, int W);
void gs_launch_depth_normals(const float* D, int H, int W, float fx, float fy, float cx, float cy, float jump, float* normals, hipStream_t s);
void gs_launch_normal_loss_forward(const float* D, const float* N, const float* wn, const float* wp, int H, int W, float fx, float fy, float cx,
                                   float cy, float jump, int flags, float* terms, void* ws, hipStream_t s);
void gs_launch_normal_loss_backward(const float* D, const float* N, const float* wn, const float* wp, int H, int W, float fx, float fy, float cx,
                                    float cy, float jump, int flags, const float* terms, const float* upstream, float* G, hipStream_t s);
void gs_launch_depth_smooth_forward(const float* D, const float* I, const float* wp, int H, int W, float lambda, int flags, float* terms, void* ws,
                                    hipStream_t s);
void gs_launch_depth_smooth_backward(const float* D, const float* I, const float* wp, int H, int W, float lambda, int flags, const float* terms,
                                     const float* upstream, float* G, hipStream_t s);

void gs_launch_gaussian_normals_forward(const float* pc, const float* feat, const int32_t* obj, const float* q_pc, const float* t_pc, int64_t N,
                                        int K, float* normals, hipStream_t s);
void gs_launch_gaussian_normals_backward(const float* pc, const float* feat, const int32_t* obj, const float* q_pc, const float* t_pc, int64_t N,
                                         int K, const float* grad_normals, float* grad_feat, hipStream_t s);
void gs_launch_normal_consistency_forward(const float* D, const float* R, const float* wp, int H, int W, float fx, float fy, float cx, float cy,
                                          float jump, float min_length, float* terms, void* ws, hipStream_t s);
void gs_launch_normal_consistency_backward(const float* D, const float* R, const float* wp, int H, int W, float fx, float fy, float cx, float cy,
                                           float jump, float min_length, const float* terms, const float* upstream, float* G, float* GR,
                                           hipStream_t s);

struct gs_tsdf_volume;
struct gs_tsdf_view;
struct gs_iso_volume;
void gs_launch_tsdf_integrate(const gs_tsdf_volume& vol, const gs_tsdf_view* views, int n_views, hipStream_t s);
void gs_launch_iso_plan(const gs_iso_volume& vol, void* cell_ws, void* block_ws, int64_t* totals, hipStream_t s);
void gs_launch_iso_emit(const gs_iso_volume& vol, const void* cell_ws, const void* block_ws, void* voxel_ws, int64_t n_vertices,
                        int64_t n_faces, float* vertices, float* colours, int32_t* faces, hipStream_t s);
```

### taichi_3d_gaussian_splatting_amd/csrc/gs_host.h

```cpp
#pragma once
#include "../../include/gs_rasterizer.h"
#include "gs_common.h"

#include <initializer_list>
#include <mutex>
#include <string>
#include <vector>

extern thread_local std::string g_last_error __attribute__((visibility("hidden")));

static int fail(int code, const std::string& msg)
{
    g_last_error = msg;
    return code;
}

static int fail(int code, const char* who, const std::string& msg)
{
    g_last_error.assign(who).append(": ").append(msg);
    return code;
}

#define HIP_TRY(expr)                                                                              \
    do {                                                                                           \
        hipError_t e__ = (expr);                                                                   \
        if (e__ != hipSuccess)                                                                     \
            return fail(e__ == hipErrorOutOfMemory ? GS_ERR_OUT_OF_MEMORY : GS_ERR_HIP,            \
                        std::string(#expr) + ": " + hipGetErrorString(e__));                       \
    } while (0)

struct DevBuf {
    void* p = nullptr;
    size_t cap = 0;
    hipError_t ensure(size_t bytes, int64_t* total)
    {
        if (bytes <= cap) return hipSuccess;
        size_t want = bytes + bytes / 4 + 256;
        if (p) { (void)hipFree(p); *total -= (int64_t)cap; p = nullptr; cap = 0; }
        hipError_t e = hipMalloc(&p, want);
        if (e != hipSuccess) { p = nullptr; return e; }
        cap = want; *total += (int64_t)want;
        return hipSuccess;
    }
    void release(int64_t* total) { if (p) { (void)hipFree(p); *total -= (int64_t)cap; } p = nullptr; cap = 0; }
    template <typename T> T* as() const { return reinterpret_cast<T*>(p); }
};

struct GsProf {
    uint64_t mask = 0;
    struct Rec { int kid; hipEvent_t a, b; };
    std::vector<Rec> recs;
    std::vector<hipEvent_t> spare;
    double total_ms[KID_COUNT_] = {};
    int64_t launches[KID_COUNT_] = {};
};

struct ResampleTable {
    int H_in = 0, W_in = 0, h_full = 0, w_full = 0;
    DevBuf buf;
    GsResampleAxis ax{}, ay{};
    std::vector<unsigned char> host;
};

struct Frame;

#define GS_COUNTER_SLOTS 64
struct gs_ctx {
    int device = 0;
    GsProf prof;
    std::mutex mu;
    int64_t device_bytes = 0;
    std::vector<Frame*> frames;
    int transient = -1;
    DevBuf block_counts, block_offsets, tile_block_sums, hist, scan_tmp, counters, partial, visited, zero_row, sums, loss_ws;
    DevBuf first_hist;
    DevBuf pose_scratch;
    DevBuf mcmc_ws;
    DevBuf appearance_ws;
    DevBuf bilateral_ws;
    DevBuf depth_ws;
    DevBuf geometry_ws;
    DevBuf ch_partial, ch_flags;
    uint8_t visit_gen = 0;
    uint64_t bwd_serial = 0;
    size_t touched_offset = 0;
    DevBuf row_block_totals;
    DevBuf merge_tags, merge_ids;
    DevBuf knn_sort, knn_hist, knn_points, knn_tree;
    DevBuf mix_records, mix_sums, mix_partial;
    DevBuf mixg_queries, mixg_partial, mixg_sums, mixg_x_partial;
    std::vector<struct ResampleTable*> resample_tables;
    GsCounters* host_counters = nullptr;
    GsCounters* host_counters_dev = nullptr;
    uint64_t slots_busy = 1ull;
    int32_t ticket = 0;
    int64_t counter_wait_ns = 0;
    struct { bool valid = false; int H = 0, W = 0; uint32_t K = 0; int max_code = 0; } seen;
    DevBuf order_hint;
    int order_hint_T = 0;
    bool has_stream = false;
    hipStream_t last_stream = nullptr;
    hipEvent_t switch_event = nullptr;
};

static hipError_t enter_stream(gs_ctx* c, hipStream_t s)
{
    if (c->has_stream && c->last_stream != s) {
        hipError_t e = hipEventRecord(c->switch_event, c->last_stream);
        if (e != hipSuccess) return e;
        e = hipStreamWaitEvent(s, c->switch_event, 0);
        if (e != hipSuccess) return e;
    }
    c->has_stream = true; c->last_stream = s;
    return hipSuccess;
}

static int enter_call(gs_ctx* c, gs_stream stream_, hipStream_t* s_out)
{
    const hipStream_t s = reinterpret_cast<hipStream_t>(stream_);
    HIP_TRY(hipSetDevice(c->device));
    HIP_TRY(enter_stream(c, s));
    *s_out = s;
    return GS_OK;
}

struct Need { DevBuf* buf; size_t bytes; const char* name; };
#define NEED(buf, bytes) Need{ &(buf), (bytes), #buf }

static int grow(gs_ctx* c, const char* who, std::initializer_list<Need> needs)
{
    for (const Need& n : needs)
        if (n.buf->ensure(n.bytes, &c->device_bytes) != hipSuccess)
            return fail(GS_ERR_OUT_OF_MEMORY, who, std::string("device allocation failed: ") + n.name);
    return GS_OK;
}

template <typename Launch>
static int queued_call(gs_ctx* c, gs_stream stream_, const char* who, std::initializer_list<Need> needs, Launch&& launch)
{
    std::lock_guard<std::mutex> lock(c->mu);
    HIP_TRY(hipSetDevice(c->device));
    if (const int rc = grow(c, who, needs)) return rc;
    hipStream_t s;
    if (const int rc = enter_call(c, stream_, &s)) return rc;
    launch(s);
    HIP_TRY(hipGetLastError());
    return GS_OK;
}
```

### taichi_3d_gaussian_splatting_amd/csrc/k_backward.hip

```cpp
#include "gs_point_math.h"
#include "gs_cull.h"
#include <cstdlib>

#define RED_STRIDE 68
#define PW 12

#define ORDER_BINS 2048
#define ORDER_BIN_WIDTH 4
#define ORDER_PER 8
#ifndef HEAVY_MIN_WORK
#define HEAVY_MIN_WORK 512
#endif
#define HEAVY_CAP GS_HEAVY_CAP
__host__ __device__ inline int gs_heavy_cap(int T) { return T / 8 < HEAVY_CAP ? T / 8 : HEAVY_CAP; }
#define GS_FILL_ZERO_RANGES 9
struct GsFillRange { float* dst = nullptr; unsigned long long n = 0; };
struct GsZeroFill { unsigned first_block = ~0u, n_blocks = 0; GsFillRange zero[GS_FILL_ZERO_RANGES];
                    unsigned M = 0;
                    const int32_t* ids = nullptr; const int32_t* ntiles = nullptr; const float4* PA = nullptr; const float4* PB = nullptr;
                    int32_t* hook_ids = nullptr; int32_t* hook_ntiles = nullptr; float* hook_depth = nullptr; float* hook_uv = nullptr;
                    int32_t* c_num_in_camera = nullptr; };
#define GS_FILL_BLOCK_BYTES (100u << 10)
__device__ __forceinline__ void gs_store_zero(float4* p)
{
    typedef float gs_v4f __attribute__((ext_vector_type(4)));
    __builtin_nontemporal_store(gs_v4f{0.0f, 0.0f, 0.0f, 0.0f}, reinterpret_cast<gs_v4f*>(p));
}
template <typename T> __device__ __forceinline__ void gs_store_nt(T* p, const T v) { __builtin_nontemporal_store(v, p); }
__device__ __forceinline__ void gs_zero_fill(const GsZeroFill& z)
{
    const unsigned long long stride = (unsigned long long)z.n_blocks * 256;
    const unsigned long long first = (unsigned long long)(blockIdx.x - z.first_block) * 256 + threadIdx.x;
#pragma unroll
    for (int r = 0; r < GS_FILL_ZERO_RANGES; ++r) {
        float* dst = z.zero[r].dst;
        const unsigned long long n = z.zero[r].n;
        if (n == 0ull) continue;
        unsigned long long head = ((16u - (unsigned)(reinterpret_cast<uintptr_t>(dst) & 15u)) & 15u) / 4u;
        head = head < n ? head : n;
        const unsigned long long n4 = (n - head) / 4ull, tail = (n - head) & 3ull;
        float4* body = reinterpret_cast<float4*>(dst + head);
        for (unsigned long long i = first; i < n4; i += stride) gs_store_zero(body + i);
        if (first < head) gs_store_nt(dst + first, 0.0f);
        if (first < tail) gs_store_nt(dst + head + 4ull * n4 + first, 0.0f);
    }
    for (unsigned long long m = first; m < z.M; m += stride) {
        const int32_t n = z.ids[m];
        if (z.hook_ids) gs_store_nt(z.hook_ids + m, n);
        if (z.hook_ntiles) gs_store_nt(z.hook_ntiles + m, z.ntiles[m]);
        if (z.hook_depth) gs_store_nt(z.hook_depth + m, GS_REC(z.PB, m).w);
        if (z.hook_uv) { const float4 pa = GS_REC(z.PA, m); gs_store_nt(z.hook_uv + 2 * m, pa.x); gs_store_nt(z.hook_uv + 2 * m + 1, pa.y); }
        if (z.c_num_in_camera) z.c_num_in_camera[n] += 1;
    }
}
__global__ __launch_bounds__(1024) void k_tile_order(const int32_t* __restrict__ tile_work, int T, int32_t* __restrict__ order, int32_t* __restrict__ hint,
                                                     int32_t* __restrict__ n_heavy_out, int heavy_factor_x2,
                                                     const int32_t* __restrict__ tile_start, const int32_t* __restrict__ tile_end,
                                                     const int32_t* __restrict__ tile_cut, int item_cap)
{
    __shared__ uint32_t bins[ORDER_BINS];
    __shared__ int32_t sHeavy[HEAVY_CAP];
    __shared__ int32_t sNHeavy;
    __shared__ uint32_t wsum[16];
    __shared__ unsigned long long wtot[16];
    const int t = threadIdx.x, lane = t & 63, wave = t >> 6;
    for (int i = t; i < ORDER_BINS; i += 1024) bins[i] = 0;
    if (t < HEAVY_CAP) n_heavy_out[GS_ORDER_REDO_OFFSET + t] = 0;
    __syncthreads();
    unsigned long long total = 0ull;
    for (int base = 0; base < T; base += 1024 * ORDER_PER) {
        int work[ORDER_PER];
#pragma unroll
        for (int k = 0; k < ORDER_PER; ++k) { const int i = base + k * 1024 + t; work[k] = i < T ? tile_work[i] : -1; }
#pragma unroll
        for (int k = 0; k < ORDER_PER; ++k) {
            if (base + k * 1024 + t >= T) continue;
            total += (unsigned long long)(work[k] > 0 ? work[k] : 0);
            int w = work[k] / ORDER_BIN_WIDTH; w = w < 0 ? 0 : (w > ORDER_BINS - 1 ? ORDER_BINS - 1 : w);
            atomicAdd(&bins[ORDER_BINS - 1 - w], 1u);
        }
    }
#pragma unroll
    for (int o = 32; o > 0; o >>= 1) total += __shfl_xor(total, o, 64);
    if (lane == 0) wtot[wave] = total;
    __syncthreads();
    uint32_t a = bins[2 * t], b = bins[2 * t + 1];
    const uint32_t incl = gs_wave_scan_incl(a + b, lane);
    if (lane == 63) wsum[wave] = incl;
    __syncthreads();
    uint32_t woff = 0;
    for (int w = 0; w < wave; ++w) woff += wsum[w];
    const uint32_t excl = woff + incl - (a + b);
    __syncthreads();
    bins[2 * t] = excl; bins[2 * t + 1] = excl + a;
    __syncthreads();
    if (t == 0) {
        unsigned long long sum = 0ull;
        for (int w = 0; w < 16; ++w) sum += wtot[w];
        const unsigned long long mean = T > 0 ? sum / (unsigned long long)T : 0ull;
        unsigned long long thr = (unsigned long long)heavy_factor_x2 * mean / 2ull;
        if (thr < HEAVY_MIN_WORK) thr = HEAVY_MIN_WORK;
        unsigned long long bw = (thr + ORDER_BIN_WIDTH - 1) / ORDER_BIN_WIDTH;
        if (bw > ORDER_BINS - 1) bw = ORDER_BINS - 1;
        int n = 0;
        if (heavy_factor_x2 > 0) n = (int)bins[ORDER_BINS - (int)bw];
        const int cap = gs_heavy_cap(T);
        if (n > cap) {
            int lo = 0, hi = ORDER_BINS - (int)bw;
            while (lo < hi) { const int mid = (lo + hi + 1) / 2; if ((int)bins[mid] <= cap) lo = mid; else hi = mid - 1; }
            n = (int)bins[lo];
        }
        sNHeavy = n;
        *n_heavy_out = sNHeavy;
    }
    __syncthreads();
    for (int base = 0; base < T; base += 1024 * ORDER_PER) {
        int work[ORDER_PER];
#pragma unroll
        for (int k = 0; k < ORDER_PER; ++k) { const int i = base + k * 1024 + t; work[k] = i < T ? tile_work[i] : -1; }
#pragma unroll
        for (int k = 0; k < ORDER_PER; ++k) {
            const int i = base + k * 1024 + t;
            if (i >= T) continue;
            int w = work[k] / ORDER_BIN_WIDTH; w = w < 0 ? 0 : (w > ORDER_BINS - 1 ? ORDER_BINS - 1 : w);
            const uint32_t pos = atomicAdd(&bins[ORDER_BINS - 1 - w], 1u);
            order[pos] = i;
            if (hint) hint[pos] = i;
            if (pos < HEAVY_CAP) sHeavy[pos] = i;
        }
    }
    __syncthreads();
    const int n_heavy = sNHeavy;
    int nseg = 0;
    if (t < n_heavy) {
        const int tile = sHeavy[t];
        const int L = tile_end[tile] - tile_start[tile];
        nseg = (tile_cut && tile_cut[tile] > 0 && L > 0) ? (L - 1) / GS_SEG + 1 : 1;
    }
    auto block_scan = [&](uint32_t x, uint32_t& excl, uint32_t& total_out) {
        const uint32_t inc = gs_wave_scan_incl(x, lane);
        __syncthreads();
        if (lane == 63) wsum[wave] = inc;
        __syncthreads();
        uint32_t wo = 0, tt = 0;
        for (int w = 0; w < 16; ++w) { if (w < wave) wo += wsum[w]; tt += wsum[w]; }
        excl = wo + inc - x; total_out = tt;
    };
    uint32_t ibase = 0, total_items = 0;
    block_scan((uint32_t)nseg, ibase, total_items);
    if (t < n_heavy && (int)(ibase + (uint32_t)nseg) + (n_heavy - 1 - t) > item_cap) nseg = 1;
    block_scan((uint32_t)nseg, ibase, total_items);
    if (t < n_heavy) n_heavy_out[4 + t] = (int32_t)ibase;
    if (t == 0) { n_heavy_out[4 + n_heavy] = (int32_t)total_items; n_heavy_out[1] = (int32_t)total_items; }
}

struct QuadState { float T, W, gr, gg, gb, tot0, tot1; int last; };

struct BwdAux { const float* grad_depth; const float* depth; const float* grad_alpha; };
struct AuxState { float kD, kA, D, R; };

__device__ __forceinline__ float gs_clamp_alpha(float prod_alpha)
{
    return __int_as_float(min(__float_as_int(prod_alpha), __float_as_int(GS_ALPHA_MAX)));
}
template <bool FIRST> __device__ __forceinline__ float gs_acc(float a, float b, float acc) { return FIRST ? a * b : __builtin_fmaf(a, b, acc); }
template <bool FIRST> __device__ __forceinline__ float gs_acc1(float a, float acc)
{
#pragma clang fp contract(fast)
    return FIRST ? a : acc + a;
}
template <bool STRICT, bool AUX, bool FIRST, int NV>
__device__ __forceinline__ void gs_bwd_contribution(QuadState& Q, AuxState& X, float (&v)[NV], const float alpha, const float g,
                                                    const float cix, const float ciy, const float m00, const float m01, const float m11,
                                                    const float4 c4, const float depth, const float apt)
{
#pragma clang fp contract(fast)
    const float one_m = 1.0f - alpha;
    const float inv = __builtin_amdgcn_rcpf(one_m);
    const float Tn = Q.T * inv;
    const float cg = c4.x * Q.gr + c4.y * Q.gg + c4.z * Q.gb;
    float ag = Tn * cg - inv * Q.W;
    const float d_rgb = alpha * Tn;
    if constexpr (AUX) {
        const float dd = depth - X.D;
        ag += X.kD * (Tn * dd - inv * X.R) + X.kA * inv;
        v[10] = gs_acc<FIRST>(X.kD, d_rgb, v[10]);
        X.R = __builtin_fmaf(d_rgb, dd, X.R);
    }
    const float agg = ag * g;
    const float vs0 = agg * cix, vs1 = agg * ciy;
    v[0] = gs_acc1<FIRST>(vs0, v[0]); v[1] = gs_acc1<FIRST>(vs1, v[1]);
    if (STRICT) {
        v[2] = gs_acc<FIRST>(agg, m00, v[2]); v[3] = gs_acc<FIRST>(agg, m01, v[3]); v[4] = gs_acc<FIRST>(agg, m11, v[4]);
    } else {
        v[2] = gs_acc<FIRST>(vs0, cix, v[2]);
        v[3] = gs_acc<FIRST>(vs0, ciy, v[3]);
        v[4] = gs_acc<FIRST>(vs1, ciy, v[4]);
    }
    v[5] = gs_acc<FIRST>(d_rgb, Q.gr, v[5]);
    v[6] = gs_acc<FIRST>(d_rgb, Q.gg, v[6]);
    v[7] = gs_acc<FIRST>(d_rgb, Q.gb, v[7]);
    v[8] = gs_acc1<FIRST>(agg, v[8]);
    v[9] = gs_acc1<FIRST>(__builtin_amdgcn_sqrtf(vs0 * vs0 + vs1 * vs1), v[9]);
    Q.T = Tn;
    Q.W = __builtin_fmaf(cg, d_rgb, Q.W);
    Q.tot0 = __builtin_fmaf(fabsf(vs0), apt, Q.tot0);
    Q.tot1 = __builtin_fmaf(fabsf(vs1), apt, Q.tot1);
}

struct BwdCoop { unsigned long long* done; int32_t* slot; int32_t* point; int32_t* tile_last; float (*slab)[64][12];
                 int seg, nseg; const float4* cut_rec; float2* mag_part;
                 int32_t* redo; };

template <int NQ, bool STRICT, bool COOP, bool AUX = false>
__device__ __forceinline__ void gs_bwd_tile_body(const int tile, const int grp, const int G_rows, float4 (*sRec)[3], float* sRed, const BwdCoop coop,
                                                 const int32_t* __restrict__ tile_start, const int32_t* __restrict__ tile_end,
                                                 const int32_t* __restrict__ sorted_vals,
                                                 const float4* __restrict__ PA, const float4* __restrict__ PB,
                                                 const float4* __restrict__ PC, const ushort4* __restrict__ boxes,
                                                 const uint32_t* __restrict__ offsets,
                                                 const float* __restrict__ grad_image, const float* __restrict__ acc_alpha,
                                                 const int32_t* __restrict__ last_in, int W, int H, int tiles_x,
                                                 float* __restrict__ partial, uint8_t* __restrict__ visited, uint8_t* __restrict__ touched,
                                                 const uint8_t gen, float* __restrict__ mag_image, const BwdAux aux = BwdAux{})
{
    constexpr int NV = AUX ? 11 : 10;
#ifdef GS_STATS
    const unsigned long long gs_t0 = wall_clock64();
#endif
    const int lane = threadIdx.x & 63;
    const int tile_u = tile % tiles_x, tile_v = tile / tiles_x;
    const int start = tile_start[tile], end = tile_end[tile];
    const int seg_lo = (COOP && coop.nseg > 1) ? start + coop.seg * GS_SEG : start;
    const int seg_hi = (COOP && coop.nseg > 1 && coop.seg < coop.nseg - 1) ? start + (coop.seg + 1) * GS_SEG : end;
    const int lx = lane & 7, ly = lane >> 3;
    QuadState Q[NQ];
    AuxState X[AUX ? NQ : 1];
    float t_end[COOP ? NQ : 1];
    int qlast[NQ];
    float rx0[NQ], ry0[NQ];
#pragma unroll
    for (int qi = 0; qi < NQ; ++qi) {
        const int q = grp * NQ + qi;
        const int pu = tile_u * 16 + (q & 1) * 8 + lx, pv = tile_v * 16 + (q >> 1) * 8 + ly;
        const bool inside = pu < W && pv < H;
        const size_t o = inside ? (size_t)pv * (size_t)W + (size_t)pu : 0;
        Q[qi].last = inside ? last_in[o] : start;
        Q[qi].T = 1.0f - acc_alpha[o];
        if constexpr (COOP) t_end[qi] = Q[qi].T;
        if constexpr (AUX) {
            const float A = inside ? acc_alpha[o] : 0.0f;
            const float gD = inside && aux.grad_depth ? aux.grad_depth[o] : 0.0f;
            X[qi].kD = gD / (A > 1e-6f ? A : 1e-6f);
            X[qi].kA = inside && aux.grad_alpha ? aux.grad_alpha[o] * Q[qi].T : 0.0f;
            X[qi].D = inside && aux.grad_depth ? aux.depth[o] : 0.0f;
            X[qi].R = 0.0f;
        }
        Q[qi].W = 0.0f;
        Q[qi].gr = grad_image[3 * o]; Q[qi].gg = grad_image[3 * o + 1]; Q[qi].gb = grad_image[3 * o + 2];
        Q[qi].tot0 = Q[qi].tot1 = 0.0f;
        if constexpr (COOP) {
            if (coop.nseg > 1 && coop.seg < coop.nseg - 1 && Q[qi].last >= seg_hi) {
                const float4* rec = coop.cut_rec + grp * 64 + lane;
                float br = 0.0f, bg = 0.0f, bb = 0.0f, t_final = 1.0f;
                for (int k = coop.nseg - 1; k > coop.seg; --k) {
                    const float4 r = rec[(size_t)k * 256];
                    if (k == coop.nseg - 1) t_final = r.x;
                    br += r.y; bg += r.z; bb += r.w;
                }
                const float ratio = t_final > 0.0f ? Q[qi].T / t_final : 1.0f;
                Q[qi].T = rec[(size_t)coop.seg * 256].x * ratio;
                Q[qi].W = ((Q[qi].gr * br + Q[qi].gg * bg) + Q[qi].gb * bb) * ratio;
            }
        }
        qlast[qi] = gs_wave_max_i(Q[qi].last);
        rx0[qi] = (float)(tile_u * 16 + (q & 1) * 8) + 0.5f;
        ry0[qi] = (float)(tile_v * 16 + (q >> 1) * 8) + 0.5f;
    }
    int tile_last = qlast[0];
#pragma unroll
    for (int qi = 1; qi < NQ; ++qi) tile_last = max(tile_last, qlast[qi]);
    if constexpr (COOP) {
        if (lane == 0) coop.tile_last[grp] = tile_last;
        __syncthreads();
        tile_last = max(max(coop.tile_last[0], coop.tile_last[1]), max(coop.tile_last[2], coop.tile_last[3]));
    }
    bool pixels_finite;
    {
        float t = 0.0f;
#pragma unroll
        for (int qi = 0; qi < NQ; ++qi) t += ((Q[qi].gr + Q[qi].gg) + Q[qi].gb) + Q[qi].T;
        if constexpr (AUX) {
#pragma unroll
            for (int qi = 0; qi < NQ; ++qi) t += (X[qi].kD + X[qi].kA) + X[qi].D;
        }
        pixels_finite = gs_ballot(!(t - t == 0.0f)) == 0ull;
    }
    float pxq[NQ], pyq[NQ];
#pragma unroll
    for (int qi = 0; qi < NQ; ++qi) { pxq[qi] = rx0[qi] + (float)lx; pyq[qi] = ry0[qi] + (float)ly; }

    for (int hi = min(seg_hi, tile_last); hi > seg_lo; hi -= 64) {
        const int lo = max(seg_lo, hi - 64);
        const int i = lo + lane;
        const bool valid = i < hi;
        const int p = valid ? sorted_vals[i] : 0;
        {
            const float4 A = GS_REC(PA, p), B = GS_REC(PB, p), C = GS_REC(PC, p);
            const CullSplat cs = gs_cull_prepare(A, B, C);
            unsigned long long mq[NQ];
            unsigned long long U = 0ull;
#pragma unroll
            for (int qi = 0; qi < NQ; ++qi) {
                const unsigned long long inq = gs_ballot(Q[qi].last > lo);
                if (inq == 0ull) { mq[qi] = 0ull; continue; }
                const CullRect lr = gs_live_rect(inq, rx0[qi], ry0[qi]);
                mq[qi] = gs_ballot(valid && i < qlast[qi] && !gs_cull(cs, lr.x0, lr.y0, lr.wx, lr.wy));
                U |= mq[qi];
            }
            GS_STAT(8, 1);
            float fsum = ((A.x + A.y) + (A.z + A.w)) + ((B.x + B.y) + B.z) + ((C.x + C.y) + C.z);
            fsum = valid ? fsum : 0.0f;
#pragma unroll
            for (int qi = 0; qi < NQ; ++qi) fsum += Q[qi].W;
            if constexpr (AUX) {
                fsum += valid ? B.w : 0.0f;
#pragma unroll
                for (int qi = 0; qi < NQ; ++qi) fsum += X[qi].R;
            }
            const bool clean = pixels_finite && gs_ballot(!(fsum - fsum == 0.0f)) == 0ull;
            unsigned long long done = 0ull;
            if (U) {
                uint32_t slot = 0;
                if ((U >> lane) & 1ull) {
                    const ushort4 bx = boxes[p];
                    slot = (offsets[p] + (uint32_t)(((int)bx.w - (int)bx.z) * (tile_u - (int)bx.x) + (tile_v - (int)bx.z))) * (uint32_t)G_rows
                           + (COOP ? 0u : (uint32_t)grp);
                    if constexpr (COOP) { coop.slot[lane] = (int32_t)slot; coop.point[lane] = p; }
                }
                sRec[lane][0] = A; sRec[lane][1] = B; sRec[lane][2] = C;
                __builtin_amdgcn_wave_barrier();
                while (U) {
                    const int j = 63 - __builtin_clzll(U);
                    U &= ~(1ull << j);
                    GS_STAT(9, 1);
                    const float4 a4 = sRec[j][0], b4 = sRec[j][1], c4 = sRec[j][2];
                    const float a = a4.z, b = a4.w, c = b4.x, apt = b4.z;
                    float v[NV];
#pragma unroll
                    for (int k = 0; k < NV; ++k) v[k] = 0.0f;
                    int n_use = 0;
#pragma unroll
                    for (int qi = 0; qi < NQ; ++qi) {
                        if (!((mq[qi] >> j) & 1ull)) continue;
                        GS_STAT(10, 1);
                        const unsigned long long inr_m = gs_ballot((lo + j) < Q[qi].last);
                        GS_STAT(11, 1);
                        const float dx = pxq[qi] - a4.x, dy = pyq[qi] - a4.y;
                        float cix, ciy, g, prod_alpha;
                        float m00 = 0.0f, m01 = 0.0f, m11 = 0.0f;
                        unsigned long long use_m;
                        if (STRICT) {
                            cix = a * dx + b * dy; ciy = b * dx + c * dy;
                            g = gs_exp_blend(-0.5f * (dx * cix + dy * ciy)) * b4.y;
                            const float oxx = dx * dx, oxy = dx * dy, oyx = dy * dx, oyy = dy * dy;
                            const float io00 = a * oxx + b * oyx, io01 = a * oxy + b * oyy;
                            const float io10 = b * oxx + c * oyx, io11 = b * oxy + c * oyy;
                            m00 = io00 * a + io01 * b; m01 = io00 * b + io01 * c; m11 = io10 * b + io11 * c;
                            prod_alpha = g * apt;
                            use_m = gs_ballot(prod_alpha >= GS_ALPHA_EPS) & inr_m;
                        } else {
                            cix = __builtin_fmaf(a, dx, b * dy); ciy = __builtin_fmaf(b, dx, c * dy);
                            g = __builtin_amdgcn_exp2f(__builtin_fmaf(dx, cix, dy * ciy) * -0.72134752044448170f) * b4.y;
                            prod_alpha = g * apt;
                            use_m = gs_ballot(prod_alpha >= GS_ALPHA_EPS + 4.0e-8f) & inr_m;
                            if (use_m != (gs_ballot(prod_alpha >= GS_ALPHA_EPS - 4.0e-8f) & inr_m)) {
                                const float sx = a * dx + b * dy, sy = b * dx + c * dy;
                                g = gs_exp_blend(-0.5f * (dx * sx + dy * sy)) * b4.y;
                                prod_alpha = g * apt;
                                use_m = gs_ballot(prod_alpha >= GS_ALPHA_EPS) & inr_m;
                                GS_STAT(14, 1);
                            }
                        }
                        n_use += __popcll(use_m);
                        GS_STAT(12, __popcll(use_m)); GS_STAT(15, use_m != 0ull ? 1 : 0);
                        if (qi == 0 && clean) {
                            const bool use = __builtin_amdgcn_inverse_ballot_w64(use_m);
                            gs_bwd_contribution<STRICT, AUX, true>(Q[qi], X[AUX ? qi : 0], v, use ? gs_clamp_alpha(prod_alpha) : 0.0f, use ? g : 0.0f,
                                                                   cix, ciy, m00, m01, m11, c4, b4.w, apt);
                        } else if (__builtin_amdgcn_inverse_ballot_w64(use_m)) {
                            gs_bwd_contribution<STRICT, AUX, false>(Q[qi], X[AUX ? qi : 0], v, gs_clamp_alpha(prod_alpha), g,
                                                                    cix, ciy, m00, m01, m11, c4, b4.w, apt);
                        }
                    }
                    if (n_use == 0) continue;
                    GS_STAT(13, 1);
#pragma unroll
                    for (int k = 0; k < NV; ++k) sRed[k * RED_STRIDE + lane] = v[k];
                    __builtin_amdgcn_wave_barrier();
                    float t = 0.0f;
                    if (AUX ? (lane < 40 || (lane >= 44 && lane < 48)) : lane < 40) {
                        const int krow = AUX && lane >= 44 ? 10 : (lane >> 2);
                        const float4* src = reinterpret_cast<const float4*>(sRed + krow * RED_STRIDE + 16 * (lane & 3));
                        const float4 x0 = src[0], x1 = src[1], x2 = src[2], x3 = src[3];
                        t = (((x0.x + x0.y) + (x0.z + x0.w)) + ((x1.x + x1.y) + (x1.z + x1.w))) +
                            (((x2.x + x2.y) + (x2.z + x2.w)) + ((x3.x + x3.y) + (x3.z + x3.w)));
                    }
                    t += gs_dpp<0xB1>(t);
                    t += gs_dpp<0x4E>(t);
                    if (lane == 40) t = __int_as_float(n_use);
                    if constexpr (COOP) {
                        if ((lane & 3) == 0 && lane < 48) reinterpret_cast<float*>(&sRec[j][0])[lane >> 2] = t;
                        done |= 1ull << j;
                    } else {
                        const uint32_t sj = (uint32_t)__builtin_amdgcn_readlane((int)slot, j);
                        float* row = partial + (size_t)sj * PW;
                        if ((lane & 3) == 0 && lane < 48) row[lane >> 2] = t;
                        if (lane == 63) { visited[sj] = gen; touched[__builtin_amdgcn_readlane(p, j)] = gen; }
                    }
                    __builtin_amdgcn_wave_barrier();
                }
                __builtin_amdgcn_wave_barrier();
            }
            if constexpr (COOP) {
                if (lane == 0) coop.done[grp] = done;
                __syncthreads();
                const int tj = (int)(threadIdx.x >> 2), part = (int)(threadIdx.x & 3);
                float r0 = 0.0f, r1 = 0.0f, r2 = 0.0f;
                int cnt = 0;
                bool any = false;
#pragma unroll
                for (int w = 0; w < 4; ++w) {
                    if ((coop.done[w] >> tj) & 1ull) {
                        const float* src = &coop.slab[w][tj][3 * part];
                        r0 += src[0];
// ... 409 lines not shown
        gs_sum_point_block<AUX>(partial, visited, gen, zero_row, sOff[li], sCnt[li], sPart, sums + 3 * (size_t)(m0 + li));
    }
}

template <bool AUX, bool LIVE>
__global__ __launch_bounds__(256, 7) void k_sum_rows(int M, int G, const uint32_t* __restrict__ offsets, const int32_t* __restrict__ ntiles,
                                                  const float* __restrict__ partial, const uint8_t* __restrict__ visited, const uint8_t* __restrict__ touched,
                                                  const uint8_t gen, const float4* __restrict__ zero_row, float4* __restrict__ sums, const GsMagFold fold,
                                                  const int32_t* __restrict__ max_tiles_hint)
{
    if (blockIdx.x >= fold.first_block) { gs_fold_mag(fold); return; }
    if constexpr (LIVE) gs_sum_rows_live<AUX>(M, G, offsets, ntiles, partial, visited, touched, gen, zero_row, sums, max_tiles_hint);
    else gs_sum_rows_all<AUX>(M, G, offsets, ntiles, partial, visited, touched, gen, zero_row, sums, max_tiles_hint);
}

#define ROW_LDS 60
template <bool AUX, bool PREZEROED>
__global__ __launch_bounds__(256) void k_bwd_points(
    int64_t N, const int32_t* __restrict__ cam_index, const float4* __restrict__ sums, const float4* __restrict__ PD,
    const float* __restrict__ pc, const float* __restrict__ feat, const int32_t* __restrict__ obj,
    const float* __restrict__ Kmat, const GsPose* __restrict__ pose,
    int keep, float f_color, float f_high, float f_s, float f_q, float f_alpha,
    float* __restrict__ grad_pc, float* __restrict__ grad_feat, float* __restrict__ grad_uv, float* __restrict__ mag,
    int32_t* __restrict__ n_affected,
    float* __restrict__ hook_gpc, float* __restrict__ hook_gfeat, float* __restrict__ hook_guv, float* __restrict__ hook_mag,
    int32_t* __restrict__ hook_ids, int32_t* __restrict__ hook_ntiles, float* __restrict__ hook_depth, float* __restrict__ hook_uv,
    const float4* __restrict__ PA, const float4* __restrict__ PB, const int32_t* __restrict__ ntiles,
    int32_t* __restrict__ c_num_in_camera, int32_t* __restrict__ c_num_pixels, float* __restrict__ c_vs_grad,
    float* __restrict__ c_vs_grad_avg, float* __restrict__ c_pos_grad, float* __restrict__ c_pos_grad_norm,
    int M, const int32_t* __restrict__ ids, const uint8_t* __restrict__ touched_tag, const uint8_t gen)
{
    int64_t n;
    int m;
    bool touched;
    float out[GS_NFEAT];
#pragma unroll
    for (int k = 0; k < GS_NFEAT; ++k) out[k] = 0.0f;
    float s[PW];
    if constexpr (!PREZEROED) {
    n = (int64_t)blockIdx.x * 256 + threadIdx.x;
    const bool valid = n < N;
    m = valid ? cam_index[n] : -1;
    if (valid && m < 0) {
        grad_pc[3 * n] = 0.0f; grad_pc[3 * n + 1] = 0.0f; grad_pc[3 * n + 2] = 0.0f;
        if (grad_uv) { grad_uv[2 * n] = 0.0f; grad_uv[2 * n + 1] = 0.0f; }
        if (mag) mag[n] = 0.0f;
    }
#pragma unroll
    for (int k = 0; k < PW; ++k) s[k] = 0.0f;
    if (m >= 0) {
        const float4 r0 = sums[3 * (size_t)m], r1 = sums[3 * (size_t)m + 1], r2 = sums[3 * (size_t)m + 2];
        s[0] = r0.x; s[1] = r0.y; s[2] = r0.z; s[3] = r0.w; s[4] = r1.x; s[5] = r1.y; s[6] = r1.z; s[7] = r1.w;
        s[8] = r2.x; s[9] = r2.y; s[10] = r2.z; s[11] = r2.w;
    }
    touched = m >= 0 && __float_as_int(s[10]) != 0;
    if (m >= 0 && !touched) {
        grad_pc[3 * n] = 0.0f; grad_pc[3 * n + 1] = 0.0f; grad_pc[3 * n + 2] = 0.0f;
        if (grad_uv) { grad_uv[2 * n] = 0.0f; grad_uv[2 * n + 1] = 0.0f; }
        if (mag) mag[n] = 0.0f;
        if (n_affected) n_affected[m] = 0;
        if (hook_gpc) { hook_gpc[3 * (size_t)m] = 0.0f; hook_gpc[3 * (size_t)m + 1] = 0.0f; hook_gpc[3 * (size_t)m + 2] = 0.0f; }
        if (hook_guv) { hook_guv[2 * (size_t)m] = 0.0f; hook_guv[2 * (size_t)m + 1] = 0.0f; }
        if (hook_mag) hook_mag[m] = 0.0f;
        if (hook_ids) hook_ids[m] = (int32_t)n;
        if (hook_ntiles) hook_ntiles[m] = ntiles[m];
        if (hook_depth) hook_depth[m] = GS_REC(PB, m).w;
        if (hook_uv) { const float4 pa = GS_REC(PA, m); hook_uv[2 * (size_t)m] = pa.x; hook_uv[2 * (size_t)m + 1] = pa.y; }
        if (c_num_in_camera) c_num_in_camera[n] += 1;
    }
    } else {
        const int mt = (int)blockIdx.x * 256 + (int)threadIdx.x;
        touched = mt < M && touched_tag[mt] == gen;
        __shared__ int sCount[4];
        __shared__ int sTouched[256];
        const int wave = threadIdx.x >> 6, lane = threadIdx.x & 63;
        const unsigned long long tb = gs_ballot(touched);
        if (lane == 0) sCount[wave] = __popcll(tb);
        __syncthreads();
        int first = 0, total = 0;
#pragma unroll
        for (int w = 0; w < 4; ++w) { const int c = sCount[w]; first += w < wave ? c : 0; total += c; }
        if (touched) sTouched[first + __popcll(tb & ((1ull << lane) - 1ull))] = (int)threadIdx.x;
        __syncthreads();
        touched = (int)threadIdx.x < total;
        if (!touched) return;
        m = (int)blockIdx.x * 256 + sTouched[threadIdx.x];
        n = ids[m];
        const float4 r0 = sums[3 * (size_t)m], r1 = sums[3 * (size_t)m + 1], r2 = sums[3 * (size_t)m + 2];
        s[0] = r0.x; s[1] = r0.y; s[2] = r0.z; s[3] = r0.w; s[4] = r1.x; s[5] = r1.y; s[6] = r1.z; s[7] = r1.w;
        s[8] = r2.x; s[9] = r2.y; s[10] = r2.z; s[11] = r2.w;
    }
    if (touched) {
        {
            const float apt = GS_REC(PB, m).z;
            s[0] *= apt; s[1] *= apt; s[9] *= apt;
            const float h = 0.5f * apt;
            s[2] *= h; s[3] *= h; s[4] *= h;
            s[8] *= (1.0f - apt) * apt;
        }
        const float guv0 = s[0], guv1 = s[1];
        const float g00 = s[2], g01 = s[3], g11 = s[4];
        const float4* row4 = reinterpret_cast<const float4*>(feat + (size_t)GS_NFEAT * n);
        float row[GS_NFEAT];
        gs_load_feat_row(row4, row);
        const GsPose& P = pose[obj[n]];
        float Km[9];
#pragma unroll
        for (int k = 0; k < 9; ++k) Km[k] = Kmat[k];
        const float x = pc[3 * n], y = pc[3 * n + 1], z = pc[3 * n + 2];
        float tx = ((P.R[0] * x + P.R[1] * y) + P.R[2] * z) + P.t[0];
        float ty = ((P.R[3] * x + P.R[4] * y) + P.R[5] * z) + P.t[1];
        float tz = ((P.R[6] * x + P.R[7] * y) + P.R[8] * z) + P.t[2];
        float d[6] = { Km[0] / tz, Km[1] / tz, (-Km[0] * tx - Km[1] * ty) / (tz * tz),
                       Km[3] / tz, Km[4] / tz, (-Km[3] * tx - Km[4] * ty) / (tz * tz) };
        float gt[3];
#pragma unroll
        for (int j = 0; j < 3; ++j) {
            const float j0 = (d[0] * P.R[j] + d[1] * P.R[3 + j]) + d[2] * P.R[6 + j];
            const float j1 = (d[3] * P.R[j] + d[4] * P.R[3 + j]) + d[5] * P.R[6 + j];
            gt[j] = guv0 * j0 + guv1 * j1;
        }
        if constexpr (AUX) {
#pragma unroll
            for (int j = 0; j < 3; ++j) gt[j] += s[11] * P.R[6 + j];
        }
        const float4 pd = GS_REC(PD, m);
        float J[6];
        gs_projection_jacobian(Km[0], Km[4], pd.x, pd.y, pd.z, J);
        float U[6];
#pragma unroll
        for (int j = 0; j < 3; ++j) {
            U[j] = J[0] * P.R[j] + J[2] * P.R[6 + j];
            U[3 + j] = J[4] * P.R[3 + j] + J[5] * P.R[6 + j];
        }
        const float qx = row[0], qy = row[1], qz = row[2], qw = row[3];
        float R[9];
        rotation_from_quaternion(row, R);
        const float es[3] = { gs_expf(row[4]), gs_expf(row[5]), gs_expf(row[6]) };
        float Mm[9];
#pragma unroll
        for (int i = 0; i < 3; ++i)
#pragma unroll
            for (int j = 0; j < 3; ++j) Mm[3 * i + j] = R[3 * i + j] * es[j];
        const float sx = es[0], sy = es[1], sz = es[2];
        const float dMdq[36] = {
            0.0f, -4 * sx * qy, -4 * sx * qz, 0.0f,
            2 * sy * qy, 2 * sy * qx, -2 * sy * qw, -2 * sy * qz,
            2 * sz * qz, 2 * sz * qw, 2 * sz * qx, 2 * sz * qy,
            2 * sx * qy, 2 * sx * qx, 2 * sx * qw, 2 * sx * qz,
            -4 * sy * qx, 0.0f, -4 * sy * qz, 0.0f,
            -2 * sz * qw, 2 * sz * qz, 2 * sz * qy, -2 * sz * qx,
            2 * sx * qz, -2 * sx * qw, 2 * sx * qx, -2 * sx * qy,
            2 * sy * qw, 2 * sy * qz, 2 * sy * qy, 2 * sy * qx,
            -4 * sz * qx, -4 * sz * qy, 0.0f, 0.0f };
        const float gcov[4] = { g00, g01, g01, g11 };
        float gq[4], gs_[3];
#pragma unroll
        for (int i = 0; i < 4; ++i) {
            float D[9];
#pragma unroll
            for (int a = 0; a < 3; ++a)
#pragma unroll
                for (int bb = 0; bb < 3; ++bb)
                    D[3 * a + bb] = i == 2 ? U[bb] * U[3 + a] : U[3 * (i >> 1) + a] * U[3 * (i & 1) + bb];
            float Pm[9];
#pragma unroll
            for (int bb = 0; bb < 3; ++bb) {
                const float m0 = Mm[bb], m1 = Mm[3 + bb], m2 = Mm[6 + bb];
                Pm[bb] = (((D[0] * (2.0f * m0) + D[1] * m1) + D[2] * m2) + D[3] * m1) + D[6] * m2;
                Pm[3 + bb] = (((D[1] * m0 + D[3] * m0) + D[4] * (2.0f * m1)) + D[5] * m2) + D[7] * m2;
                Pm[6 + bb] = (((D[2] * m0 + D[5] * m1) + D[6] * m0) + D[7] * m1) + D[8] * (2.0f * m2);
            }
#pragma unroll
            for (int k = 0; k < 4; ++k) {
                float acc = 0.0f;
                bool first = true;
#pragma unroll
                for (int e = 0; e < 9; ++e) {
                    const bool zero = (e == 0 && (k == 0 || k == 3)) || (e == 4 && (k == 1 || k == 3)) || (e == 8 && k >= 2);
                    if (zero) continue;
                    const float term = Pm[e] * dMdq[4 * e + k];
                    acc = first ? term : acc + term;
                    first = false;
                }
                gq[k] = i == 0 ? gcov[0] * acc : gq[k] + gcov[i] * acc;
            }
#pragma unroll
            for (int c = 0; c < 3; ++c) {
                const float acc = ((Pm[c] * R[c] + Pm[3 + c] * R[3 + c]) + Pm[6 + c] * R[6 + c]) * es[c];
                gs_[c] = i == 0 ? gcov[0] * acc : gs_[c] + gcov[i] * acc;
            }
        }
        float dx = x - P.origin_bwd[0], dy = y - P.origin_bwd[1], dz = z - P.origin_bwd[2];
        float dn = sqrtf(dx * dx + dy * dy + dz * dz);
        float ux = dx / dn, uy = dy / dn, uz = dz / dn;
        float sh[16];
        gs_sh16(ux, uy, uz, sh);
        out[0] = gq[0] * f_q; out[1] = gq[1] * f_q; out[2] = gq[2] * f_q; out[3] = gq[3] * f_q;
        out[4] = gs_[0] * f_s; out[5] = gs_[1] * f_s; out[6] = gs_[2] * f_s;
        out[7] = s[8] * f_alpha;
#pragma unroll
        for (int ch = 0; ch < 3; ++ch) {
            const float* f = row + 8 + 16 * ch;
            float accd = f[0] * sh[0];
#pragma unroll
            for (int k = 1; k < 16; ++k) accd = accd + f[k] * sh[k];
            float sg = gs_sigmoid(accd);
            float jac = sg * (1.0f - sg);
            float gc = s[5 + ch];
#pragma unroll
            for (int k = 0; k < 16; ++k) {
                float v = gc * (jac * sh[k]);
                v = k < keep ? v * (k == 0 ? f_color : f_high) : 0.0f;
                out[8 + 16 * ch + k] = v;
            }
        }
        grad_pc[3 * n] = gt[0]; grad_pc[3 * n + 1] = gt[1]; grad_pc[3 * n + 2] = gt[2];
        if (grad_uv) { grad_uv[2 * n] = guv0; grad_uv[2 * n + 1] = guv1; }
        if (mag) mag[n] = s[9];
        if (n_affected) n_affected[m] = __float_as_int(s[10]);
        if (hook_gpc) { hook_gpc[3 * (size_t)m] = gt[0]; hook_gpc[3 * (size_t)m + 1] = gt[1]; hook_gpc[3 * (size_t)m + 2] = gt[2]; }
        if (hook_guv) { hook_guv[2 * (size_t)m] = guv0; hook_guv[2 * (size_t)m + 1] = guv1; }
        if (hook_mag) hook_mag[m] = s[9];
        if constexpr (!PREZEROED) {
            if (hook_ids) hook_ids[m] = (int32_t)n;
            if (hook_ntiles) hook_ntiles[m] = ntiles[m];
            if (hook_depth) hook_depth[m] = GS_REC(PB, m).w;
            if (hook_uv) { const float4 pa = GS_REC(PA, m); hook_uv[2 * (size_t)m] = pa.x; hook_uv[2 * (size_t)m + 1] = pa.y; }
        }
        if (c_num_in_camera)
            gs_controller_add<!PREZEROED>(n, __float_as_int(s[10]), s[9], gt[0], gt[1], gt[2],
                                          c_num_in_camera, c_num_pixels, c_vs_grad, c_vs_grad_avg, c_pos_grad, c_pos_grad_norm);
    }

    if constexpr (PREZEROED) {
        if (touched) {
            float4* dst = reinterpret_cast<float4*>(grad_feat + (size_t)GS_NFEAT * n);
#pragma unroll
            for (int k = 0; k < GS_NFEAT / 4; ++k) dst[k] = make_float4(out[4 * k], out[4 * k + 1], out[4 * k + 2], out[4 * k + 3]);
            if (hook_gfeat) {
                float4* hdst = reinterpret_cast<float4*>(hook_gfeat + (size_t)GS_NFEAT * m);
#pragma unroll
                for (int k = 0; k < GS_NFEAT / 4; ++k) hdst[k] = make_float4(out[4 * k], out[4 * k + 1], out[4 * k + 2], out[4 * k + 3]);
            }
        }
    } else {
    __shared__ __attribute__((aligned(16))) float sRows[4][64 * ROW_LDS + 64];
    const int wave = threadIdx.x >> 6, lane = threadIdx.x & 63;
    float* mine = sRows[wave] + lane * ROW_LDS;
#pragma unroll
    for (int k = 0; k < GS_NFEAT / 4; ++k)
        *reinterpret_cast<float4*>(mine + 4 * k) = make_float4(out[4 * k], out[4 * k + 1], out[4 * k + 2], out[4 * k + 3]);
    const unsigned long long cam_m = gs_ballot(m >= 0);
    int* rank_to_lane = reinterpret_cast<int*>(sRows[wave] + 64 * ROW_LDS);
    if (m >= 0) rank_to_lane[__popcll(cam_m & ((1ull << lane) - 1ull))] = lane;
    __builtin_amdgcn_wave_barrier();
    const int64_t n0 = (int64_t)blockIdx.x * 256 + wave * 64;
    const int rows = (int)(N - n0 < 64 ? N - n0 : 64);
    if (rows > 0) {
        float4* dst = reinterpret_cast<float4*>(grad_feat + (size_t)GS_NFEAT * n0);
        for (int e = lane; e < rows * (GS_NFEAT / 4); e += 64) {
            const int r = e / (GS_NFEAT / 4), c = e - r * (GS_NFEAT / 4);
            dst[e] = *reinterpret_cast<const float4*>(sRows[wave] + r * ROW_LDS + 4 * c);
        }
    }
    if (hook_gfeat && cam_m != 0ull) {
        const int m_first = __builtin_amdgcn_readlane(m, __builtin_ctzll(cam_m));
        const int cnt = __popcll(cam_m);
        float4* dst = reinterpret_cast<float4*>(hook_gfeat + (size_t)GS_NFEAT * m_first);
        for (int e = lane; e < cnt * (GS_NFEAT / 4); e += 64) {
            const int r = e / (GS_NFEAT / 4), c = e - r * (GS_NFEAT / 4);
            dst[e] = *reinterpret_cast<const float4*>(sRows[wave] + rank_to_lane[r] * ROW_LDS + 4 * c);
        }
    }
    }
}

void gs_launch_backward_blend(const GsBackwardArgs& a, hipStream_t s)
{
    const GsFrameView& v = a.v;
    const BwdAux aux{a.grad_depth, a.depth, a.grad_alpha};
    if (v.T > 0 && a.K > 0) {
        const unsigned groups = (unsigned)(v.cuts ? a.item_cap : gs_heavy_cap(v.T)) + (unsigned)(((size_t)v.T * (size_t)a.G + 3) / 4);
        GsZeroFill fill{};
        if (a.prefill) {
            const unsigned long long N = (unsigned long long)a.N, M = (unsigned long long)a.M;
            int r = 0;
            unsigned long long bytes = 0;
            auto zero = [&](void* p, unsigned long long n) { if (p && n) { fill.zero[r].dst = static_cast<float*>(p); fill.zero[r].n = n; ++r; bytes += 4 * n; } };
            zero(a.grad_feat, GS_NFEAT * N); zero(a.hook_gfeat, GS_NFEAT * M);
            zero(a.grad_pc, 3 * N); zero(a.grad_uv, 2 * N); zero(a.mag, N);
            zero(a.n_affected, M); zero(a.hook_gpc, 3 * M); zero(a.hook_guv, 2 * M); zero(a.hook_mag, M);
            if (a.hook_ids || a.hook_ntiles || a.hook_depth || a.hook_uv || a.c_num_in_camera) {
                fill.M = (unsigned)a.M;
                fill.ids = v.ids; fill.ntiles = v.ntiles; fill.PA = v.PA; fill.PB = v.PB;
                fill.hook_ids = a.hook_ids; fill.hook_ntiles = a.hook_ntiles; fill.hook_depth = a.hook_depth; fill.hook_uv = a.hook_uv;
                fill.c_num_in_camera = a.c_num_in_camera;
                bytes += 4 * M * ((a.hook_ids != nullptr) + (a.hook_ntiles != nullptr) + (a.hook_depth != nullptr) + 2 * (a.hook_uv != nullptr) +
                                  (a.c_num_in_camera != nullptr));
            }
            fill.first_block = groups;
            fill.n_blocks = (unsigned)((bytes + GS_FILL_BLOCK_BYTES - 1) / GS_FILL_BLOCK_BYTES);
        }
        GS_TIMED(a.prof, KID_TILE_ORDER, s, k_tile_order<<<1, 1024, 0, s>>>(v.tile_work, v.T, v.tile_order, a.order_hint, v.n_heavy, a.heavy_factor_x2,
                                                                              v.tile_start, v.tile_end, v.cuts ? v.tile_cut : nullptr, v.cuts ? a.item_cap : gs_heavy_cap(v.T)));
#define GS_BWD_LAUNCH_(NQ_, STRICT_, AUX_)                                                                                             \
        GS_TIMED(a.prof, KID_BLEND_BWD, s, k_blend_bwd_tile<NQ_, STRICT_, AUX_><<<groups + fill.n_blocks, 256, 0, s>>>(v.tile_order, v.n_heavy, v.T,      \
                 v.tile_start, v.tile_end, v.vals_sorted, v.PA, v.PB, v.PC, v.box, v.offsets, a.grad_image, a.acc_alpha, a.last, a.W,     \
                 a.H, a.tiles_x, a.partial, a.visited, a.touched, a.gen, a.mag_image, v.cuts, v.cut_mag, v.tile_cut, aux, fill))
#define GS_BWD_LAUNCH(NQ_, STRICT_) { if (a.aux) GS_BWD_LAUNCH_(NQ_, STRICT_, true); else GS_BWD_LAUNCH_(NQ_, STRICT_, false); }
        if (a.G == 1) { if (a.strict) GS_BWD_LAUNCH(4, true) else GS_BWD_LAUNCH(4, false) }
        else if (a.G == 2) { if (a.strict) GS_BWD_LAUNCH(2, true) else GS_BWD_LAUNCH(2, false) }
        else { if (a.strict) GS_BWD_LAUNCH(1, true) else GS_BWD_LAUNCH(1, false) }
#undef GS_BWD_LAUNCH
#undef GS_BWD_LAUNCH_
        if (v.cuts && gs_heavy_cap(v.T) > 0) {
#define GS_BWD_REPAIR(STRICT_)                                                                                                          \
            GS_TIMED(a.prof, KID_BLEND_BWD_REPAIR, s, k_blend_bwd_repair<STRICT_><<<(unsigned)gs_heavy_cap(v.T), 256, 0, s>>>(v.tile_order, v.n_heavy, a.G, \
                     v.tile_start, v.tile_end, v.vals_sorted, v.PA, v.PB, v.PC, v.box, v.offsets, a.grad_image, a.acc_alpha, a.last, a.W, a.H,  \
                     a.tiles_x, a.partial, a.visited, a.touched, a.gen, a.mag_image))
            if (a.strict) GS_BWD_REPAIR(true); else GS_BWD_REPAIR(false);
#undef GS_BWD_REPAIR
        }
    }
    else if (a.mag_image)
        (void)hipMemsetAsync(a.mag_image, 0, sizeof(float) * 2 * (size_t)a.H * (size_t)a.W, s);
    if (a.M > 0 && v.T > 0 && a.K > 0) {
        GsMagFold fold{};
        fold.first_block = a.live_sums ? (unsigned)((a.M + 255) / 256) : (unsigned)(((size_t)a.M * 4 + 255) / 256);
        fold.n_heavy = v.n_heavy; fold.tile_order = v.tile_order; fold.tile_cut = v.tile_cut; fold.cut_mag = v.cut_mag;
        fold.mag_image = v.cuts ? a.mag_image : nullptr; fold.W = a.W; fold.H = a.H; fold.tiles_x = a.tiles_x;
        const unsigned fold_blocks = fold.mag_image ? (unsigned)gs_heavy_cap(v.T) : 0u;
#define GS_SUM_ROWS(AUX_, LIVE_)                                                                                                        \
        GS_TIMED(a.prof, KID_SUM_ROWS, s, k_sum_rows<AUX_, LIVE_><<<fold.first_block + fold_blocks, 256, 0, s>>>(a.M, a.G, v.offsets, v.ntiles, a.partial, \
                                                                                  a.visited, a.touched, a.gen, a.zero_row, a.sums, fold, a.max_tiles_hint))
        if (a.live_sums) { if (a.aux) GS_SUM_ROWS(true, true); else GS_SUM_ROWS(false, true); }
        else { if (a.aux) GS_SUM_ROWS(true, false); else GS_SUM_ROWS(false, false); }
#undef GS_SUM_ROWS
    }
    else if (a.M > 0)
        (void)hipMemsetAsync(a.sums, 0, sizeof(float) * PW * (size_t)a.M, s);
}

void gs_launch_backward_points(const GsBackwardArgs& a, hipStream_t s)
{
    const GsFrameView& v = a.v;
    const int nb = a.prefill ? (a.M + 255) / 256 : (int)((a.N + 255) / 256);
    if (nb == 0) return;
    int keep = a.sh_band <= 0 ? 1 : a.sh_band == 1 ? 4 : a.sh_band == 2 ? 9 : 16;
#define GS_BWD_POINTS(AUX_, PRE_)                                                                                                       \
    GS_TIMED(a.prof, KID_BWD_POINTS, s, k_bwd_points<AUX_, PRE_><<<nb, 256, 0, s>>>(a.N, v.cam_index, a.sums, v.PD, a.point_cloud, a.features,   \
                                                                    a.object_id, a.Kmat, v.pose, keep, a.f_color, a.f_high, a.f_s, a.f_q, a.f_alpha, \
                                                                    a.grad_pc, a.grad_feat, a.grad_uv, a.mag, a.n_affected,                \
                                                                    a.hook_gpc, a.hook_gfeat, a.hook_guv, a.hook_mag,                      \
                                                                    a.hook_ids, a.hook_ntiles, a.hook_depth, a.hook_uv, v.PA, v.PB, v.ntiles, \
                                                                    a.c_num_in_camera, a.c_num_pixels, a.c_vs_grad, a.c_vs_grad_avg, a.c_pos_grad, a.c_pos_grad_norm, \
                                                                    a.M, v.ids, a.touched, a.gen))
    if (a.prefill) { if (a.aux) GS_BWD_POINTS(true, true); else GS_BWD_POINTS(false, true); }
    else { if (a.aux) GS_BWD_POINTS(true, false); else GS_BWD_POINTS(false, false); }
#undef GS_BWD_POINTS
}
```

### taichi_3d_gaussian_splatting_amd/csrc/k_blend_fwd.hip

```cpp
#include "gs_common.h"
#include "gs_cull.h"
#include "gs_sort_key.h"
#ifndef GS_WORK_PER_BATCH
#define GS_WORK_PER_BATCH 8
#endif

template <typename KeyT>
__device__ __forceinline__ int gs_first_key_of_tile(const KeyT* __restrict__ keys, uint32_t K, int tile_shift, uint32_t tile, int lane)
{
    uint32_t lo = 0, hi = K;
    while (lo < hi) {
        const uint32_t span = hi - lo, step = (span + 63u) / 64u;
        const uint32_t mine = (uint32_t)(lane + 1) * step;
        const uint32_t p = lo + (mine < span ? mine : span) - 1u;
        const unsigned long long b = gs_ballot((uint32_t)(keys[p] >> tile_shift) >= tile);
        if (b == 0ull) { lo = hi; break; }
        const uint32_t f = (uint32_t)__builtin_ctzll(b);
        const uint32_t pf = lo + ((f + 1u) * step < span ? (f + 1u) * step : span) - 1u;
        if (f > 0u) lo = lo + (f * step < span ? f * step : span);
        hi = pf;
    }
    return (int)lo;
}

template <bool RGB_ONLY>
__global__ __launch_bounds__(256) void k_blend_fwd(int32_t* __restrict__ tile_start, int32_t* __restrict__ tile_end,
                                                   const void* __restrict__ sorted_keys, int key_bytes, int tile_shift,
                                                   const GsCounters* __restrict__ ctr, uint32_t K_cap,
                                                   const int32_t* __restrict__ sorted_vals,
                                                   const float4* __restrict__ PA, const float4* __restrict__ PB,
                                                   const float4* __restrict__ PC, int W, int H, int tiles_x,
                                                   float* __restrict__ image, float* __restrict__ depth_out,
                                                   float* __restrict__ acc_alpha, int32_t* __restrict__ last_out,
                                                   int32_t* __restrict__ count_out, int32_t* __restrict__ tile_work,
                                                   const int32_t* __restrict__ order_hint,
                                                   float4* __restrict__ cuts, int32_t* __restrict__ tile_cut, int cut_cap)
{
    __shared__ float4 sRec[4][64][3];
    const uint32_t K = min(ctr->K, K_cap);
    const int tile = order_hint ? order_hint[blockIdx.x] : (int)blockIdx.x;
    const int wave = __builtin_amdgcn_readfirstlane((int)(threadIdx.x >> 6)), lane = threadIdx.x & 63;
    const GsQuadPixel qp = gs_quad_pixel(tile, wave, lane, tiles_x, W, H);
    __shared__ int sRange[2];
    if (wave < 2) {
        const uint32_t want = (uint32_t)tile + (uint32_t)wave;
        const int r = K == 0u ? 0
                    : key_bytes == 2 ? gs_first_key_of_tile(reinterpret_cast<const uint16_t*>(sorted_keys), K, tile_shift, want, lane)
                    : key_bytes == 8 ? gs_first_key_of_tile(reinterpret_cast<const uint64_t*>(sorted_keys), K, tile_shift, want, lane)
                                     : gs_first_key_of_tile(reinterpret_cast<const uint32_t*>(sorted_keys), K, tile_shift, want, lane);
        if (lane == 0) sRange[wave] = r;
    }
    __syncthreads();
    const bool occupied = sRange[1] > sRange[0];
    const int start = occupied ? sRange[0] : 0, end = occupied ? sRange[1] : 0;
    if (threadIdx.x == 0) { tile_start[tile] = start; tile_end[tile] = end; }
    const bool long_list = end - start > GS_CUT_MIN_LEN;
    int cut_base = -1;
    if (!RGB_ONLY && cut_cap > 0 && long_list) {
        const int n_rec = (end - start - 1) / GS_SEG + 1;
        const int b = start / GS_SEG + tile;
        if (b + n_rec <= cut_cap) cut_base = b;
        if (threadIdx.x == 0) tile_cut[tile] = cut_base + 1;
    }
    int next_rec = 0;
    float tot_r = 0.0f, tot_g = 0.0f, tot_b = 0.0f;
#ifdef GS_STATS
    const unsigned long long gs_t0 = wall_clock64();
#endif

    float T_i = 1.0f, cr = 0.0f, cg = 0.0f, cb = 0.0f, acc_d = 0.0f, norm = 0.0f;
    int last = start, count = 0;
    int evals = 0;
    unsigned long long alive = gs_ballot(qp.inside);

    for (int base = start; base < end; base += 64) {
        if (alive == 0ull) break;
        if (long_list && base > start && ((base - start) & (GS_SEG - 1)) == 0) {
            if (cut_base >= 0) { cuts[(size_t)(cut_base + next_rec) * 256 + threadIdx.x] = make_float4(T_i, cr, cg, cb); next_rec += 1; }
            tot_r += cr; tot_g += cg; tot_b += cb;
            cr = 0.0f; cg = 0.0f; cb = 0.0f;
        }
        evals += GS_WORK_PER_BATCH;
        const int i = base + lane;
        const bool valid = i < end;
        const int p = valid ? sorted_vals[i] : 0;
        float4 A = GS_REC(PA, p), B = GS_REC(PB, p), C = GS_REC(PC, p);
        const CullRect lr = gs_live_rect(alive, qp.rx0, qp.ry0);
        bool keep = valid && !gs_cull(gs_cull_prepare(A, B, C), lr.x0, lr.y0, lr.wx, lr.wy);
        unsigned long long mask = gs_ballot(keep);
        GS_STAT(0, 1); GS_STAT(1, __popcll(mask));
        if (mask == 0ull) continue;
        evals += __popcll(mask);
        sRec[wave][lane][0] = A; sRec[wave][lane][1] = B; sRec[wave][lane][2] = C;
        if (__popcll(mask) & 1) {
            const int jz = __builtin_ctzll(~mask);
            if (lane == jz) {
                sRec[wave][lane][0] = make_float4(0.0f, 0.0f, 1.0f, 0.0f);
                sRec[wave][lane][1] = make_float4(1.0f, 0.0f, 0.0f, 0.0f);
                sRec[wave][lane][2] = make_float4(0.0f, 0.0f, 0.0f, 0.0f);
            }
            mask |= 1ull << jz;
        }
        __builtin_amdgcn_wave_barrier();
        int lj = -1;
        while (mask) {
            const int j0 = __builtin_ctzll(mask);
            asm("s_bitset0_b64 %0, %1" : "+s"(mask) : "s"(j0));
            const int j1 = __builtin_ctzll(mask);
            asm("s_bitset0_b64 %0, %1" : "+s"(mask) : "s"(j1));
            const float4 a40 = sRec[wave][j0][0], b40 = sRec[wave][j0][1], c40 = sRec[wave][j0][2];
            const float4 a41 = sRec[wave][j1][0], b41 = sRec[wave][j1][1], c41 = sRec[wave][j1][2];
            const float e0 = gs_splat_exponent(qp.px, qp.py, a40, b40), e1 = gs_splat_exponent(qp.px, qp.py, a41, b41);
            float alpha0 = gs_alpha_of_exponent(e0, b40);
            float alpha1 = gs_alpha_of_exponent(e1, b41);
            asm volatile("" : "+v"(alpha0), "+v"(alpha1));
#define GS_FWD_STEP(ALPHA, A4, B4, C4, J, LIVE)                                                                                        \
            {                                                                                                                    \
                GS_STAT(2, 1);                                                                                                   \
                unsigned long long use_m = gs_ballot(!((ALPHA) < GS_ALPHA_EPS)) & (LIVE);                           \
                const float alpha = gs_alpha_clamp(ALPHA);                                                          \
                const float next_T = T_i * (1.0f - alpha);                                                          \
                const unsigned long long sat_m = gs_ballot(next_T < GS_T_STOP) & use_m;                         \
                alive &= ~sat_m;                                                                                                 \
                use_m &= ~sat_m;                                                                                                 \
                GS_STAT(3, __popcll(use_m)); GS_STAT(5, __popcll(alive));                                                        \
                if (__builtin_amdgcn_inverse_ballot_w64(use_m)) {                                                                \
                    lj = (J);                                   \
                     \
                     \
                    const float w = alpha * T_i;                                                                                 \
                    cr = __builtin_fmaf((C4).x, w, cr); cg = __builtin_fmaf((C4).y, w, cg); cb = __builtin_fmaf((C4).z, w, cb);   \
                    if (!RGB_ONLY) { acc_d = __builtin_fmaf((B4).w, w, acc_d); norm += w; count += 1; }         \
                    T_i = next_T;                                                                                                \
                }                                                                                                                \
            }
            GS_FWD_STEP(alpha0, a40, b40, c40, j0, alive)
            GS_FWD_STEP(alpha1, a41, b41, c41, j1, alive)
#undef GS_FWD_STEP
            if (alive == 0ull) break;
        }
        last = lj >= 0 ? base + lj + 1 : last;
        __builtin_amdgcn_wave_barrier();
    }
#ifdef GS_STATS
    if (lane == 0 && blockIdx.x * 4 + wave < 65536) { gs_stats_wave_times[2 * (blockIdx.x * 4 + wave)] = gs_t0; gs_stats_wave_times[2 * (blockIdx.x * 4 + wave) + 1] = wall_clock64(); }
#endif
    if (cut_base >= 0) {
        const int n_rec = (end - start - 1) / GS_SEG + 1;
        for (int k = next_rec; k < n_rec - 1; ++k) cuts[(size_t)(cut_base + k) * 256 + threadIdx.x] = make_float4(T_i, 0.0f, 0.0f, 0.0f);
        cuts[(size_t)(cut_base + n_rec - 1) * 256 + threadIdx.x] = make_float4(T_i, cr, cg, cb);
    }
    cr += tot_r; cg += tot_g; cb += tot_b;
    if (!qp.inside) return;
    const size_t o = qp.o;
    image[3 * o] = cr; image[3 * o + 1] = cg; image[3 * o + 2] = cb;
    if (!RGB_ONLY) {
        depth_out[o] = acc_d / (norm > 1e-6f ? norm : 1e-6f);
        acc_alpha[o] = 1.0f - T_i;
        last_out[o] = last;
        count_out[o] = count;
        if (lane == 0 && evals > 0) atomicAdd(&tile_work[tile], evals);
    }
}

void gs_launch_blend_fwd(const GsBlendFwdArgs& a, hipStream_t s)
{
    const GsFrameView& v = a.v;
    if (v.T <= 0) return;
    auto launch = [&](auto kernel) {
        GS_TIMED(a.prof, KID_BLEND_FWD, s, kernel<<<v.T, 256, 0, s>>>(v.tile_start, v.tile_end, v.keys_sorted, a.key_bytes, a.depth_bits - gs_key_dropped_bits(a.key_bytes), a.counters, a.K, v.vals_sorted, v.PA, v.PB, v.PC, a.W, a.H,
                                                                   a.tiles_x, a.image, a.depth, a.acc_alpha, a.last, a.count, v.tile_work, a.order_hint, v.cuts, v.tile_cut, a.cut_cap));
    };
    if (a.rgb_only) launch(k_blend_fwd<true>);
    else launch(k_blend_fwd<false>);
}
```

### taichi_3d_gaussian_splatting_amd/csrc/k_project.hip

```cpp
#include "gs_point_math.h"

#ifndef GS_RADIUS_FROM_PREBLUR_COV
#define GS_RADIUS_FROM_PREBLUR_COV 1
#endif

__device__ __forceinline__ void quat_mul(const float a[4], const float b[4], float o[4])
{
    float x0 = a[0], y0 = a[1], z0 = a[2], w0 = a[3];
    float x1 = b[0], y1 = b[1], z1 = b[2], w1 = b[3];
    o[0] = w0 * x1 + x0 * w1 + y0 * z1 - z0 * y1;
    o[1] = w0 * y1 - x0 * z1 + y0 * w1 + z0 * x1;
    o[2] = w0 * z1 + x0 * y1 - y0 * x1 + z0 * w1;
    o[3] = w0 * w1 - x0 * x1 - y0 * y1 - z0 * z1;
}

__device__ __forceinline__ GsPose make_pose(const float* __restrict__ q_pc, const float* __restrict__ t_pc, int i)
{
    float qc[4] = { -q_pc[4 * i], -q_pc[4 * i + 1], -q_pc[4 * i + 2], q_pc[4 * i + 3] };
    float nrm = sqrtf(qc[0] * qc[0] + qc[1] * qc[1] + qc[2] * qc[2] + qc[3] * qc[3]);
    float qn[4] = { qc[0] / nrm, qc[1] / nrm, qc[2] / nrm, qc[3] / nrm };
    float v4[4] = { t_pc[3 * i], t_pc[3 * i + 1], t_pc[3 * i + 2], 0.0f };
    float qn_conj[4] = { -qn[0], -qn[1], -qn[2], qn[3] };
    float tmp[4], rot[4];
    quat_mul(qn, v4, tmp);
    quat_mul(tmp, qn_conj, rot);
    GsPose p;
    rotation_from_quaternion(qc, p.R);
    p.t[0] = -rot[0]; p.t[1] = -rot[1]; p.t[2] = -rot[2];
    float RTn[9] = { -p.R[0], -p.R[3], -p.R[6], -p.R[1], -p.R[4], -p.R[7], -p.R[2], -p.R[5], -p.R[8] };
    gs_mm<3, 3, 1>(RTn, p.t, p.origin_fwd);
    p.origin_bwd[0] = t_pc[3 * i]; p.origin_bwd[1] = t_pc[3 * i + 1]; p.origin_bwd[2] = t_pc[3 * i + 2];
    p.q_cp[0] = qc[0]; p.q_cp[1] = qc[1]; p.q_cp[2] = qc[2]; p.q_cp[3] = qc[3];
    p.pad[0] = p.pad[1] = 0.0f;
    return p;
}

__device__ __forceinline__ void project_point(const float* __restrict__ R, const float* __restrict__ t, const float* __restrict__ Km,
                                              float x, float y, float z, float uv[2], float pc[3])
{
    pc[0] = ((R[0] * x + R[1] * y) + R[2] * z) + t[0] * 1.0f;
    pc[1] = ((R[3] * x + R[4] * y) + R[5] * z) + t[1] * 1.0f;
    pc[2] = ((R[6] * x + R[7] * y) + R[8] * z) + t[2] * 1.0f;
    float u1 = (Km[0] * pc[0] + Km[1] * pc[1]) + Km[2] * pc[2];
    float v1 = (Km[3] * pc[0] + Km[4] * pc[1]) + Km[5] * pc[2];
    uv[0] = u1 / pc[2];
    uv[1] = v1 / pc[2];
}

#define FILTER_POSE_CACHE 8
__global__ __launch_bounds__(256) void k_filter(const float* __restrict__ pc, const int8_t* __restrict__ invalid,
                                                const int32_t* __restrict__ obj, const float* __restrict__ Kmat,
                                                const float* __restrict__ q_pc, const float* __restrict__ t_pc, int n_objects,
                                                GsPose* __restrict__ pose, GsCounters* __restrict__ counters,
                                                int64_t N, int W, int H, float near_plane, float far_plane,
                                                int8_t* __restrict__ mask, int32_t* __restrict__ block_counts,
                                                int32_t* __restrict__ tile_arrays, int tile_ints)
{
    __shared__ int wave_cnt[4];
    __shared__ GsPose sp[FILTER_POSE_CACHE];
    int64_t i = (int64_t)blockIdx.x * 256 + threadIdx.x;
    for (int64_t k = i; k < tile_ints; k += (int64_t)gridDim.x * 256) tile_arrays[k] = 0;
    const bool cached = n_objects <= FILTER_POSE_CACHE;
    if (cached && threadIdx.x < n_objects) sp[threadIdx.x] = make_pose(q_pc, t_pc, threadIdx.x);
    if (blockIdx.x == 0) {
        for (int o = threadIdx.x; o < n_objects; o += 256) pose[o] = make_pose(q_pc, t_pc, o);
    }
    __syncthreads();
    bool in = false;
    const int oid = (i < N && invalid[i] != 1) ? obj[i] : 0;
    const bool bad_id = oid < 0 || oid >= n_objects;
    if (bad_id) atomicAdd(&counters->bad_object_ids, 1);
    if (i < N && invalid[i] != 1 && !bad_id) {
        const GsPose P = cached ? sp[oid] : make_pose(q_pc, t_pc, oid);
        float Km[9];
#pragma unroll
        for (int k = 0; k < 9; ++k) Km[k] = Kmat[k];
        float uv[2], p3[3];
        project_point(P.R, P.t, Km, pc[3 * i], pc[3 * i + 1], pc[3 * i + 2], uv, p3);
        float z = p3[2];
        in = z > near_plane && z < far_plane &&
             uv[0] >= (float)(-GS_TILE_SZ * GS_BOUNDARY_TILES) && uv[0] < (float)(W + GS_TILE_SZ * GS_BOUNDARY_TILES) &&
             uv[1] >= (float)(-GS_TILE_SZ * GS_BOUNDARY_TILES) && uv[1] < (float)(H + GS_TILE_SZ * GS_BOUNDARY_TILES);
    }
    if (i < N) mask[i] = in ? 1 : 0;
    unsigned long long b = gs_ballot(in);
    int lane = threadIdx.x & 63, wave = threadIdx.x >> 6;
    gs_block_put(wave_cnt, wave, lane, (int)__popcll(b));
    __syncthreads();
    if (threadIdx.x == 0) block_counts[blockIdx.x] = gs_block_sum<4>(wave_cnt);
}

__device__ __forceinline__ void gs_bin_point(float u, float v, float radius, float depth, int W, int H, float depth_scale, int idx, ushort4* __restrict__ boxes,
                                             int32_t* __restrict__ ntiles, int32_t* __restrict__ depth_codes, int& count, int& depth_code)
{
    int box[4];
    gs_tile_box(u, v, radius, (W + GS_TILE_SZ - 1) / GS_TILE_SZ, (H + GS_TILE_SZ - 1) / GS_TILE_SZ, box);
    count = (box[1] - box[0]) * (box[3] - box[2]);
    depth_code = (int)(depth * depth_scale);
    boxes[idx] = make_ushort4((unsigned short)box[0], (unsigned short)box[1], (unsigned short)box[2], (unsigned short)box[3]);
    ntiles[idx] = count;
    depth_codes[idx] = depth_code;
}
__device__ __forceinline__ void gs_bin_block_put(int* wave_sum, int* wave_max, int wave, int lane, int count, int depth_code)
{
    const int s = gs_wave_sum_i(count), mx = gs_wave_max_i(depth_code);
    gs_block_put(wave_sum, wave, lane, s); gs_block_put(wave_max, wave, lane, mx);
}
__device__ __forceinline__ void gs_bin_block_publish(const int* wave_sum, const int* wave_max, uint32_t* __restrict__ tile_block_sums, GsCounters* counters)
{
    tile_block_sums[blockIdx.x] = (uint32_t)gs_block_sum<4>(wave_sum);
    const int m = gs_block_max<4>(wave_max);
    if (m > 0) atomicMax(&counters->max_depth_code, m);
}
__device__ __forceinline__ void gs_bin_digits_clear(uint32_t* dig) { dig[threadIdx.x] = 0u; }
__device__ __forceinline__ void gs_bin_digits_add(uint32_t* dig, int count, int depth_code)
{
    if (count > 0) atomicAdd(&dig[(uint32_t)depth_code & 255u], (uint32_t)count);
}
__device__ __forceinline__ void gs_bin_digits_store(const uint32_t* dig, uint32_t* __restrict__ first_hist)
{
    if (first_hist) first_hist[(size_t)threadIdx.x * gridDim.x + blockIdx.x] = dig[threadIdx.x];
}

__global__ __launch_bounds__(256) void k_project(const float* __restrict__ pc, float* __restrict__ feat,
                                                 const int32_t* __restrict__ obj, const float* __restrict__ Kmat,
                                                 const GsPose* __restrict__ pose, const int8_t* __restrict__ mask,
                                                 const int32_t* __restrict__ block_counts, int64_t N,
                                                 int32_t* __restrict__ ids, int32_t* __restrict__ cam_index,
                                                 int32_t* __restrict__ block_offsets,
                                                 int W, int H, float depth_scale,
                                                 float4* __restrict__ PA, float4* __restrict__ PB, float4* __restrict__ PC,
                                                 float4* __restrict__ PD, ushort4* __restrict__ boxes,
                                                 int32_t* __restrict__ ntiles, uint32_t* __restrict__ tile_block_sums,
                                                 GsCounters* counters, int32_t* __restrict__ depth_codes, int32_t* __restrict__ max_tiles_hint,
                                                 uint32_t* __restrict__ first_hist)
{
    __shared__ int wave_sum[4], wave_max[4], wave_maxn[4];
    __shared__ uint32_t dig[256];
    gs_bin_digits_clear(dig);
    __shared__ float4 sOut[4][4 * 64];
    __shared__ int sIds[256];
    __shared__ int wave_cnt[4], wave_pre[4];
    int block_offset, cnt;
    {
        const int64_t i = (int64_t)blockIdx.x * 256 + threadIdx.x;
        const bool in = i < N && mask[i] != 0;
        const unsigned long long b = gs_ballot(in);
        const int lane_ = threadIdx.x & 63, wave_ = threadIdx.x >> 6;
        const int pre = gs_sum_of_blocks_before<256>(block_counts, (int)blockIdx.x);
        gs_block_put(wave_cnt, wave_, lane_, (int)__popcll(b)); gs_block_put(wave_pre, wave_, lane_, pre);
        __syncthreads();
        block_offset = gs_block_sum<4>(wave_pre);
        cnt = gs_block_sum<4>(wave_cnt);
        int woff = 0;
        for (int w = 0; w < wave_; ++w) woff += wave_cnt[w];
        const int r = woff + __popcll(b & ((1ull << lane_) - 1ull));
        if (in) { sIds[r] = (int)i; ids[block_offset + r] = (int32_t)i; }
        if (i < N) cam_index[i] = in ? block_offset + r : -1;
        if (threadIdx.x == 0) {
            block_offsets[blockIdx.x] = block_offset;
            if (blockIdx.x == gridDim.x - 1) counters->M = block_offset + cnt;
        }
        __syncthreads();
    }
    const int idx = block_offset + threadIdx.x;
    int count = 0, depth_code = 0;
    float4 recA = make_float4(0.f, 0.f, 0.f, 0.f), recB = recA, recC = recA, recD = recA;
    if ((int)threadIdx.x < cnt) {
        int pid = sIds[threadIdx.x];
        float4* row4 = reinterpret_cast<float4*>(feat + (size_t)GS_NFEAT * pid);
        float row[GS_NFEAT];
#pragma unroll
        for (int k = 0; k < GS_NFEAT / 4; ++k) {
            float4 v = row4[k];
            row[4 * k] = v.x; row[4 * k + 1] = v.y; row[4 * k + 2] = v.z; row[4 * k + 3] = v.w;
        }
        {
            float n = sqrtf(row[0] * row[0] + row[1] * row[1] + row[2] * row[2] + row[3] * row[3]);
            const float q0 = row[0] / n, q1 = row[1] / n, q2 = row[2] / n, q3 = row[3] / n;
            const bool changed = __float_as_int(q0) != __float_as_int(row[0]) || __float_as_int(q1) != __float_as_int(row[1]) ||
                                 __float_as_int(q2) != __float_as_int(row[2]) || __float_as_int(q3) != __float_as_int(row[3]);
            row[0] = q0; row[1] = q1; row[2] = q2; row[3] = q3;
            if (changed) row4[0] = make_float4(q0, q1, q2, q3);
        }
        const GsPose& P = pose[obj[pid]];
        float Km[9];
#pragma unroll
        for (int k = 0; k < 9; ++k) Km[k] = Kmat[k];
        float x = pc[3 * (size_t)pid], y = pc[3 * (size_t)pid + 1], z = pc[3 * (size_t)pid + 2];
        float uv[2], pcam[3];
        project_point(P.R, P.t, Km, x, y, z, uv, pcam);
        float J[6], Sigma[9];
        gs_projection_jacobian(Km[0], Km[4], pcam[0], pcam[1], pcam[2], J);
        gs_sigma_from_row(row, Sigma);
        float Wt[9] = { P.R[0], P.R[3], P.R[6], P.R[1], P.R[4], P.R[7], P.R[2], P.R[5], P.R[8] };
        float Jt[6] = { J[0], J[3], J[1], J[4], J[2], J[5] };
        float Wm[9];
#pragma unroll
        for (int k = 0; k < 9; ++k) Wm[k] = P.R[k];
        float JW[6], JWS[6], JWSW[6], cov[4];
        gs_mm<2, 3, 3>(J, Wm, JW);
        gs_mm<2, 3, 3>(JW, Sigma, JWS);
        gs_mm<2, 3, 3>(JWS, Wt, JWSW);
        gs_mm<2, 3, 2>(JWSW, Jt, cov);
        float c00 = cov[0], c01 = cov[1], c10 = cov[2], c11 = cov[3];
        float det_pre = c00 * c11 - c01 * c10;
        float b00 = c00 + 0.3f, b11 = c11 + 0.3f;
        float det = b00 * b11 - c01 * c10;
        float ratio = det_pre / det;
        float rescale = sqrtf(0.0f > ratio ? 0.0f : ratio);
        float inv_det = 1.0f / det;
        float conic_a = inv_det * b11, conic_b = inv_det * (-c01), conic_c = inv_det * b00;
        float alpha = 1.0f / (1.0f + gs_expf(-row[7]));
        float dx = x - P.origin_fwd[0], dy = y - P.origin_fwd[1], dz = z - P.origin_fwd[2];
        float dn = sqrtf(dx * dx + dy * dy + dz * dz);
        float sx = dx / dn, sy = dy / dn, sz = dz / dn;
        float sh[16];
        gs_sh16(sx, sy, sz, sh);
        float col[3];
#pragma unroll
        for (int ch = 0; ch < 3; ++ch) {
            const float* f = row + 8 + 16 * ch;
            float acc = f[0] * sh[0];
#pragma unroll
            for (int k = 1; k < 16; ++k) acc = acc + f[k] * sh[k];
            col[ch] = gs_sigmoid(acc);
        }
#if GS_RADIUS_FROM_PREBLUR_COV
        const float e00 = c00, e11 = c11;
#else
        const float e00 = b00, e11 = b11;
#endif
        float large_eigen = (e00 + e11 + sqrtf((e00 - e11) * (e00 - e11) + 4.0f * c01 * c10)) / 2.0f;
        float radii = sqrtf(large_eigen) * 3.0f;
        float ra = rescale * alpha;
        float cut = ra > 0.0f ? __logf(GS_ALPHA_EPS / ra) : (ra == 0.0f ? 3.0e38f : -3.0e38f);
        recA = make_float4(uv[0], uv[1], conic_a, conic_b);
        recB = make_float4(conic_c, rescale, alpha, pcam[2]);
        recC = make_float4(col[0], col[1], col[2], cut);
        recD = make_float4(pcam[0], pcam[1], pcam[2], radii);
        gs_bin_point(uv[0], uv[1], radii, pcam[2], W, H, depth_scale, idx, boxes, ntiles, depth_codes, count, depth_code);
        gs_bin_digits_add(dig, count, depth_code);
    }
    int lane = threadIdx.x & 63, wave = threadIdx.x >> 6;
    {
        float4* mine = sOut[wave];
        mine[lane] = recA; mine[64 + lane] = recB; mine[128 + lane] = recC; mine[192 + lane] = recD;
        __builtin_amdgcn_wave_barrier();
        const int wave_first = block_offset + wave * 64;
        const int n_rec = cnt - wave * 64 < 64 ? cnt - wave * 64 : 64;
        float4* dst = PA + (size_t)wave_first * 4;
#pragma unroll
        for (int k = 0; k < 4; ++k) {
            const int e = k * 64 + lane;
            if ((e >> 2) < n_rec) dst[e] = mine[(e & 3) * 64 + (e >> 2)];
        }
    }
    const int mn = gs_wave_max_i(count);
    gs_bin_block_put(wave_sum, wave_max, wave, lane, count, depth_code);
    gs_block_put(wave_maxn, wave, lane, mn);
    __syncthreads();
    gs_bin_digits_store(dig, first_hist);
    if (threadIdx.x == 0) {
        gs_bin_block_publish(wave_sum, wave_max, tile_block_sums, counters);
        const int mt = gs_block_max<4>(wave_maxn);
        if (max_tiles_hint && mt > 64) atomicMax(max_tiles_hint, mt);
    }
}

__global__ __launch_bounds__(256) void k_boxes_from_records(const float4* __restrict__ PA, const float4* __restrict__ PB,
                                                            const float4* __restrict__ PD, int M, int W, int H, float depth_scale,
                                                            ushort4* __restrict__ boxes, int32_t* __restrict__ ntiles,
                                                            uint32_t* __restrict__ tile_block_sums, GsCounters* counters,
                                                            int32_t* __restrict__ depth_codes, int32_t* __restrict__ tile_arrays, int tile_ints,
                                                            uint32_t* __restrict__ first_hist)
{
    __shared__ int wave_sum[4], wave_max[4];
    __shared__ uint32_t dig[256];
    const int idx = blockIdx.x * 256 + threadIdx.x;
    for (int k = idx; k < tile_ints; k += (int)gridDim.x * 256) tile_arrays[k] = 0;
    gs_bin_digits_clear(dig);
    __syncthreads();
    int count = 0, depth_code = 0;
    if (idx < M) {
        const float4 A = GS_REC(PA, idx);
        gs_bin_point(A.x, A.y, GS_REC(PD, idx).w, GS_REC(PB, idx).w, W, H, depth_scale, idx, boxes, ntiles, depth_codes, count, depth_code);
        gs_bin_digits_add(dig, count, depth_code);
    }
    gs_bin_block_put(wave_sum, wave_max, (int)(threadIdx.x >> 6), threadIdx.x & 63, count, depth_code);
    __syncthreads();
    gs_bin_digits_store(dig, first_hist);
    if (threadIdx.x == 0) {
        gs_bin_block_publish(wave_sum, wave_max, tile_block_sums, counters);
        if (blockIdx.x == 0) counters->M = M;
    }
}

__global__ __launch_bounds__(1024) void k_scan_tiles_publish(const uint32_t* __restrict__ in, int n, GsCounters* __restrict__ counters,
                                                             volatile GsCounters* host_mirror, int32_t ticket)
{
    __shared__ uint32_t wave_tot[16];
    gs_block_put(wave_tot, (int)(threadIdx.x >> 6), threadIdx.x & 63, gs_sum_of_blocks_before<1024>(in, n));
    __syncthreads();
    if (threadIdx.x == 0) gs_publish_counters(counters, gs_block_sum<16>(wave_tot), host_mirror, ticket);
}

void gs_launch_publish(const GsProjectArgs& a, int n_blocks, hipStream_t s)
{
    if (n_blocks <= 0) return;
    GS_TIMED(a.prof, KID_PUBLISH, s, k_scan_tiles_publish<<<1, 1024, 0, s>>>(a.tile_block_sums, n_blocks, a.counters, a.host_mirror, a.ticket));
}

void gs_launch_project(const GsProjectArgs& a, hipStream_t s, bool publish)
{
    const GsFrameView& v = a.v;
    const int nb = (int)((a.N + 255) / 256);
    if (nb == 0) { (void)hipMemsetAsync(v.tile_start, 0, sizeof(int32_t) * (size_t)v.tile_ints, s); return; }
    GS_TIMED(a.prof, KID_FILTER, s, k_filter<<<nb, 256, 0, s>>>(a.point_cloud, a.invalid, a.object_id, a.Kmat, a.q_pc, a.t_pc, a.n_objects,
                                                            v.pose, a.counters, a.N, a.W, a.H, a.near_plane, a.far_plane, v.mask,
                                                            a.block_counts, v.tile_start, v.tile_ints));
    GS_TIMED(a.prof, KID_PROJECT, s, k_project<<<nb, 256, 0, s>>>(a.point_cloud, a.features, a.object_id, a.Kmat, v.pose, v.mask, a.block_counts, a.N,
                                                              v.ids, v.cam_index, a.block_offsets, a.W, a.H,
                                                              a.depth_scale, v.PA, v.PB, v.PC, v.PD, v.box, v.ntiles,
                                                              a.tile_block_sums, a.counters, v.depth_codes, v.max_tiles, a.first_hist));
    if (publish) gs_launch_publish(a, nb, s);
}

void gs_launch_boxes_from_records(const GsProjectArgs& a, int M, hipStream_t s, bool publish)
{
    const GsFrameView& v = a.v;
    const int nb = (M + 255) / 256;
    if (nb == 0) { (void)hipMemsetAsync(v.tile_start, 0, sizeof(int32_t) * (size_t)v.tile_ints, s); return; }
    GS_TIMED(a.prof, KID_PROJECT, s, k_boxes_from_records<<<nb, 256, 0, s>>>(v.PA, v.PB, v.PD, M, a.W, a.H, a.depth_scale, v.box, v.ntiles,
                                                                          a.tile_block_sums, a.counters, v.depth_codes, v.tile_start, v.tile_ints, a.first_hist));
    if (publish) gs_launch_publish(a, nb, s);
}
```

Before: 1658 frames/s.

## Cache per-view tile orders keyed by camera pose for forward blend scheduling

Replaces the single shared tile-order hint with a table of up to 64 slots keyed by camera pose. The filter kernel finds the nearest matching slot, the forward blend uses that view's previous heavy-first tile order, and the backward tile-order kernel writes its order back into the slot. The aim is to schedule heavy tiles first in the forward pass using an order measured for the same viewpoint rather than the previous, different pose. It also stages the order in shared memory and exits early when there are no heavy tiles, at the cost of extra table memory and lookup work in block 0 of the filter kernel.

```diff
diff --git a/include/gs_view_hints.h b/include/gs_view_hints.h
--- /dev/null
+++ b/include/gs_view_hints.h
@@ -0,0 +1,17 @@
+#ifndef GS_VIEW_HINTS_H
+#define GS_VIEW_HINTS_H
+#include "gs_rasterizer.h"
+
+#ifdef __cplusplus
+extern "C" {
+#endif
+
+#define GS_VIEW_KEY_FLOATS 7
+
+int gs_view_hints_read(gs_ctx* ctx, const gs_frame* frame, int32_t slot, int32_t* n_slots, int32_t* n_tiles,
+                       float* keys, int32_t* filled, int32_t slot_cap, int32_t* order, int32_t order_cap, int32_t* frame_slots);
+
+#ifdef __cplusplus
+}
+#endif
+#endif
diff --git a/taichi_3d_gaussian_splatting_amd/csrc/gs_api.hip b/taichi_3d_gaussian_splatting_amd/csrc/gs_api.hip
--- a/taichi_3d_gaussian_splatting_amd/csrc/gs_api.hip
+++ b/taichi_3d_gaussian_splatting_amd/csrc/gs_api.hip
@@ -1,5 +1,6 @@
 #include "../../include/gs_channels.h"
 #include "../../include/gs_sparse.h"
+#include "../../include/gs_view_hints.h"
 #include "gs_host.h"
 #include "gs_sort_key.h"
 
@@ -34,6 +35,8 @@
     int n_objects = 0;
     bool rgb_only = false;
     bool max_tiles_known = false;
+    uint32_t view_epoch = 0;
+    bool view_keyed = false;
     uint32_t generation = 0;
     uint64_t bwd_serial = 0;
     int pending_slot = -1;
@@ -99,7 +102,7 @@
     (void)hipDeviceSynchronize();
     for (Frame* f : c->frames) { f->bufs.release(&c->device_bytes); delete f; }
     DevBuf* all[] = { &c->block_counts, &c->block_offsets, &c->tile_block_sums, &c->hist, &c->scan_tmp, &c->first_hist,
-                      &c->counters, &c->partial, &c->visited, &c->zero_row, &c->sums, &c->loss_ws, &c->order_hint, &c->pose_scratch,
+                      &c->counters, &c->partial, &c->visited, &c->zero_row, &c->sums, &c->loss_ws, &c->view_table, &c->pose_scratch,
                       &c->ch_partial, &c->ch_flags, &c->row_block_totals, &c->merge_tags, &c->merge_ids,
                       &c->knn_sort, &c->knn_hist, &c->knn_points, &c->knn_tree, &c->mix_records, &c->mix_sums, &c->mix_partial,
                       &c->mixg_queries, &c->mixg_partial, &c->mixg_sums, &c->mixg_x_partial, &c->mcmc_ws, &c->appearance_ws, &c->bilateral_ws, &c->depth_ws,
@@ -184,6 +187,7 @@
     Frame* f = acquire_frame(c, slot);
     f->info = gs_frame_info{};
     f->bwd_serial = 0;
+    f->view_epoch = 0; f->view_keyed = false;
     f->info.kept_for_backward = keep ? 1 : 0;
     f->info.n_tiles = T; f->info.camera_height = cam->camera_height; f->info.camera_width = cam->camera_width;
     return f;
@@ -326,6 +330,35 @@
     if (sort_narrow_keys() == NARROW_REQUIRED && f->key_bytes != 2)
         return fail(GS_ERR_STATE, "GS_SORT_NARROW_KEYS=require: the frame's sort keys are " + std::to_string(f->key_bytes) + " bytes wide");
     return GS_OK;
+}
+
+#define GS_VIEW_SLOTS_DEFAULT 64
+#define GS_VIEW_MIN_TILES 4096
+static int view_slots_wanted(int T)
+{
+    const char* e = getenv("GS_VIEW_HINTS");
+    if (!e || !e[0]) return T >= GS_VIEW_MIN_TILES ? GS_VIEW_SLOTS_DEFAULT : 1;
+    const long n = strtol(e, nullptr, 10);
+    return n < 0 ? 0 : (n > GS_VIEW_MAX_SLOTS ? GS_VIEW_MAX_SLOTS : (int)n);
+}
+static int view_table(gs_ctx* c, int T, hipStream_t s, GsViewTable* out)
+{
+    *out = GsViewTable{ nullptr, 0, 0 };
+    const int S = view_slots_wanted(T);
+    if (S == 0 || T <= 0) return GS_OK;
+    if (c->view_T != T || c->view_S != S) {
+        c->view_T = 0; c->view_S = 0;
+        if (const int rc = grow(c, "forward", { NEED(c->view_table, 4 * GS_VIEW_INTS(S, T)) })) return rc;
+        HIP_TRY(hipMemsetAsync(c->view_table.p, 0, 4 * (size_t)(GS_VIEW_HDR_INTS + GS_VIEW_KEY_INTS * S), s));
+        c->view_T = T; c->view_S = S; c->view_epoch += 1;
+    }
+    *out = GsViewTable{ c->view_table.as<int32_t>(), S, T };
+    return GS_OK;
+}
+static GsViewTable backward_views(const gs_ctx* c, const Frame* f)
+{
+    if (f->view_epoch == 0 || f->view_epoch != c->view_epoch || c->view_T != f->info.n_tiles) return GsViewTable{ nullptr, 0, 0 };
+    return GsViewTable{ c->view_table.as<int32_t>(), c->view_S, c->view_T };
 }
 
 enum CounterWait { WAIT_NOW, WAIT_LATER, WAIT_FRAME };
@@ -369,6 +402,11 @@
     }
     pa.host_mirror = c->host_counters_dev + slot; pa.ticket = ++c->ticket;
     if (c->ticket == 0x7fffffff) c->ticket = 0;
+    if (wait == WAIT_LATER && N > 0) {
+        if ((rc = view_table(c, T, s, &pa.views)) != GS_OK) return rc;
+        if (pa.views.S < 2) pa.views = GsViewTable{ nullptr, 0, 0 };
+        f->view_keyed = pa.views.base != nullptr;
+    }
     gs_launch_project(pa, s, wait != WAIT_LATER);
     f->max_tiles_known = true;
     HIP_TRY(hipGetLastError());
@@ -465,7 +503,14 @@
     fa.last = out->pixel_offset_of_last_effective_point; fa.count = out->pixel_valid_point_count;
     fa.cut_cap = cut_cap;
     static const bool use_hint = []{ const char* e = getenv("GS_FWD_ORDER_HINT"); return !(e && e[0] == '0'); }();
-    fa.order_hint = (use_hint && c->order_hint_T == T && T > 0) ? c->order_hint.as<int32_t>() : nullptr;
+    GsViewTable views;
+    if (const int rc = view_table(c, T, s, &views)) return rc;
+    f->view_epoch = views.base ? c->view_epoch : 0;
+    if (views.base && use_hint) {
+        fa.views = views;
+        fa.view_slot = f->view_keyed ? fa.v.n_heavy + GS_ORDER_READ_SLOT : views.base + 1;
+        fa.view_slot_bias = f->view_keyed ? 0 : 1;
+    }
     gs_launch_blend_fwd(fa, s);
     HIP_TRY(hipGetLastError());
     f->depth_bits = depth_bits;
@@ -729,14 +774,10 @@
         if (c->zero_row.ensure(64, &c->device_bytes) != hipSuccess) return fail(GS_ERR_OUT_OF_MEMORY, "backward: zero row");
         HIP_TRY(hipMemsetAsync(c->zero_row.p, 0, c->zero_row.cap, stream));
     }
-    if (c->order_hint_T != f->info.n_tiles) {
-        c->order_hint_T = 0;
-        if (c->order_hint.ensure(4 * (size_t)(f->info.n_tiles > 0 ? f->info.n_tiles : 1), &c->device_bytes) != hipSuccess)
-            return fail(GS_ERR_OUT_OF_MEMORY, "backward: tile order buffer");
-    }
     GsBackwardArgs a{};
     a.prof = &c->prof;
-    a.order_hint = c->order_hint.as<int32_t>();
+    a.views = backward_views(c, f);
+    a.view_slot = f->view_keyed ? frame_view(*f).n_heavy + GS_ORDER_WRITE_SLOT : nullptr;
     a.N = f->info.n_points; a.M = (int)f->info.n_points_in_camera; a.K = K;
     a.H = f->info.camera_height; a.W = f->info.camera_width;
     a.tiles_x = (a.W + GS_TILE - 1) / GS_TILE;
@@ -787,12 +828,6 @@
         a->c_pos_grad = ca->accumulated_position_gradients; a->c_pos_grad_norm = ca->accumulated_position_gradients_norm;
     }
     return GS_OK;
-}
-
-static void launch_backward_blend(gs_ctx* c, const GsBackwardArgs& a, hipStream_t s)
-{
-    gs_launch_backward_blend(a, s);
-    if (a.v.T > 0 && a.K > 0) c->order_hint_T = a.v.T;
 }
 
 static int check_backward_points_args(const Frame* f, const gs_scene* sc, const gs_camera* cam, const gs_backward_out* out, const char* who,
@@ -844,7 +879,7 @@
         a.v.cuts = nullptr;
     }
     a.prefill = points && a.grad_feat && a.v.T > 0 && a.K > 0 && bwd_prefill_enabled();
-    launch_backward_blend(c, a, s);
+    gs_launch_backward_blend(a, s);
     if (points) gs_launch_backward_points(a, s);
     if (pose) gs_launch_pose_grad(a, f->n_objects, c->pose_scratch.p, out->grad_q_pointcloud_camera, out->grad_t_pointcloud_camera, s);
     HIP_TRY(hipGetLastError());
@@ -885,7 +920,7 @@
     if ((rc = enter_call(c, stream_, &s)) != GS_OK) return rc;
     GsBackwardArgs a{};
     if ((rc = prepare_backward_blend(c, f, grad_image, acc_alpha, last, mag_image, reinterpret_cast<float4*>(splat_sums_out), f->bwd_reference_order, s, &a)) != GS_OK) return rc;
-    launch_backward_blend(c, a, s);
+    gs_launch_backward_blend(a, s);
     HIP_TRY(hipGetLastError());
     return GS_OK;
 }
@@ -1054,3 +1089,38 @@
     return 0;
 }
 #endif
+
+extern "C" int gs_view_hints_read(gs_ctx* c, const gs_frame* frame, int32_t slot, int32_t* n_slots, int32_t* n_tiles,
+                                  float* keys, int32_t* filled, int32_t slot_cap, int32_t* order, int32_t order_cap, int32_t* frame_slots)
+{
+    if (!c) return fail(GS_ERR_INVALID_ARGUMENT, "gs_view_hints_read: ctx is NULL");
+    if (slot_cap < 0 || order_cap < 0) return fail(GS_ERR_INVALID_ARGUMENT, "gs_view_hints_read: negative capacity");
+    std::lock_guard<std::mutex> lock(c->mu);
+    HIP_TRY(hipSetDevice(c->device));
+    HIP_TRY(hipDeviceSynchronize());
+    const int S = c->view_S, T = c->view_T;
+    if (slot > S) return fail(GS_ERR_INVALID_ARGUMENT, "gs_view_hints_read: no such slot");
+    if (n_slots) *n_slots = S;
+    if (n_tiles) *n_tiles = T;
+    const GsViewTable tab{ c->view_table.as<int32_t>(), S, T };
+    if (S > 0 && (keys || filled)) {
+        std::vector<int32_t> words((size_t)GS_VIEW_KEY_INTS * S);
+        HIP_TRY(hipMemcpy(words.data(), tab.key(0), 4 * words.size(), hipMemcpyDeviceToHost));
+        for (int i = 0; i < S && i < slot_cap; ++i) {
+            if (keys) std::memcpy(keys + (size_t)GS_VIEW_KEY_FLOATS * i, &words[(size_t)GS_VIEW_KEY_INTS * i], 4 * GS_VIEW_KEY_FLOATS);
+            if (filled) filled[i] = words[(size_t)GS_VIEW_KEY_INTS * i + 7] == T ? 1 : 0;
+        }
+    }
+    if (order && slot >= 0 && S > 0 && T > 0 && order_cap > 0)
+        HIP_TRY(hipMemcpy(order, tab.order(slot), 4 * (size_t)std::min(T, order_cap), hipMemcpyDeviceToHost));
+    if (frame_slots) {
+        frame_slots[0] = frame_slots[1] = -2;
+        if (frame) {
+            Frame* f;
+            if (const int rc = lookup(c, frame, "gs_view_hints_read", false, &f)) return rc;
+            if (f->view_keyed && f->view_epoch != 0 && f->view_epoch == c->view_epoch)
+                HIP_TRY(hipMemcpy(frame_slots, frame_view(*f).n_heavy + GS_ORDER_READ_SLOT, 8, hipMemcpyDeviceToHost));
+        }
+    }
+    return GS_OK;
+}
diff --git a/taichi_3d_gaussian_splatting_amd/csrc/gs_common.h b/taichi_3d_gaussian_splatting_amd/csrc/gs_common.h
--- a/taichi_3d_gaussian_splatting_amd/csrc/gs_common.h
+++ b/taichi_3d_gaussian_splatting_amd/csrc/gs_common.h
@@ -32,6 +32,21 @@
 #define GS_TILE_SPARE_MAX_TILES 3
 #define GS_ORDER_INTS(T) ((size_t)(T) + 4 + GS_HEAVY_CAP + 4 + GS_HEAVY_CAP)
 #define GS_ORDER_REDO_OFFSET (4 + GS_HEAVY_CAP + 4)
+#define GS_ORDER_READ_SLOT 2
+#define GS_ORDER_WRITE_SLOT 3
+
+#define GS_VIEW_HDR_INTS 4
+#define GS_VIEW_KEY_INTS 8
+#define GS_VIEW_MAX_SLOTS 1024
+#define GS_VIEW_INTS(S, T) (GS_VIEW_HDR_INTS + (size_t)GS_VIEW_KEY_INTS * (size_t)(S) + ((size_t)(S) + 1) * (size_t)(T))
+#define GS_VIEW_SAME_D 1.9e-5f
+struct GsViewTable {
+    int32_t* base;
+    int S, T;
+    __host__ __device__ int32_t* key(int slot) const { return base + GS_VIEW_HDR_INTS + GS_VIEW_KEY_INTS * slot; }
+    __host__ __device__ int32_t* order(int slot) const { return base + GS_VIEW_HDR_INTS + GS_VIEW_KEY_INTS * S + (size_t)slot * (size_t)T; }
+    __host__ __device__ int keyless_slot() const { return S > 1 ? S : 0; }
+};
 
 struct GsPose {
     float R[9];
@@ -300,6 +315,7 @@
     uint32_t* first_hist;
     GsCounters* counters;
     GsCounters* host_mirror; int32_t ticket;
+    GsViewTable views;
 };
 void gs_launch_project(const GsProjectArgs& a, hipStream_t s, bool publish);
 void gs_launch_publish(const GsProjectArgs& a, int n_blocks, hipStream_t s);
@@ -331,7 +347,7 @@
     int key_bytes, depth_bits; uint32_t K; const GsCounters* counters;
     float* image; float* depth; float* acc_alpha; int32_t* last; int32_t* count;
     int cut_cap;
-    const int32_t* order_hint;
+    GsViewTable views; const int32_t* view_slot; int view_slot_bias;
 };
 void gs_launch_blend_fwd(const GsBlendFwdArgs& a, hipStream_t s);
 
@@ -339,7 +355,7 @@
     GsProf* prof;
     int64_t N; int M; uint32_t K; int H, W, tiles_x;
     GsFrameView v;
-    int32_t* order_hint;
+    GsViewTable views; const int32_t* view_slot;
     const float* grad_image; const float* acc_alpha; const int32_t* last;
     const float* grad_depth; const float* depth; const float* grad_alpha; int aux;
     int G;
diff --git a/taichi_3d_gaussian_splatting_amd/csrc/gs_host.h b/taichi_3d_gaussian_splatting_amd/csrc/gs_host.h
--- a/taichi_3d_gaussian_splatting_amd/csrc/gs_host.h
+++ b/taichi_3d_gaussian_splatting_amd/csrc/gs_host.h
@@ -96,8 +96,9 @@
     int32_t ticket = 0;
     int64_t counter_wait_ns = 0;
     struct { bool valid = false; int H = 0, W = 0; uint32_t K = 0; int max_code = 0; } seen;
-    DevBuf order_hint;
-    int order_hint_T = 0;
+    DevBuf view_table;
+    int view_T = 0, view_S = 0;
+    uint32_t view_epoch = 0;
     bool has_stream = false;
     hipStream_t last_stream = nullptr;
     hipEvent_t switch_event = nullptr;
diff --git a/taichi_3d_gaussian_splatting_amd/csrc/k_backward.hip b/taichi_3d_gaussian_splatting_amd/csrc/k_backward.hip
--- a/taichi_3d_gaussian_splatting_amd/csrc/k_backward.hip
+++ b/taichi_3d_gaussian_splatting_amd/csrc/k_backward.hip
@@ -8,6 +8,7 @@
 #define ORDER_BINS 2048
 #define ORDER_BIN_WIDTH 4
 #define ORDER_PER 8
+#define ORDER_STAGE 8192
 #ifndef HEAVY_MIN_WORK
 #define HEAVY_MIN_WORK 512
 #endif
@@ -53,25 +54,37 @@
         if (z.c_num_in_camera) z.c_num_in_camera[n] += 1;
     }
 }
-__global__ __launch_bounds__(1024) void k_tile_order(const int32_t* __restrict__ tile_work, int T, int32_t* __restrict__ order, int32_t* __restrict__ hint,
+__global__ __launch_bounds__(1024) void k_tile_order(const int32_t* __restrict__ tile_work, int T, int32_t* __restrict__ order,
+                                                     GsViewTable views, const int32_t* __restrict__ view_slot, const GsPose* __restrict__ pose,
                                                      int32_t* __restrict__ n_heavy_out, int heavy_factor_x2,
                                                      const int32_t* __restrict__ tile_start, const int32_t* __restrict__ tile_end,
                                                      const int32_t* __restrict__ tile_cut, int item_cap)
 {
     __shared__ uint32_t bins[ORDER_BINS];
     __shared__ int32_t sHeavy[HEAVY_CAP];
+    __shared__ int32_t sOrder[ORDER_STAGE];
     __shared__ int32_t sNHeavy;
     __shared__ uint32_t wsum[16];
     __shared__ unsigned long long wtot[16];
     const int t = threadIdx.x, lane = t & 63, wave = t >> 6;
+    const int vslot = views.base ? (view_slot ? *view_slot : views.keyless_slot()) : -1;
+    int32_t* const hint = (vslot >= 0 && vslot <= views.S && views.T == T) ? views.order(vslot) : nullptr;
+    const bool keyed = hint && view_slot && vslot < views.S;
+    GsPose P0{};
+    if (keyed && t == 0) P0 = pose[0];
+    const bool one_round = T <= 1024 * ORDER_PER;
+    int work[ORDER_PER];
+    auto load_work = [&](int base) {
+#pragma unroll
+        for (int k = 0; k < ORDER_PER; ++k) { const int i = base + k * 1024 + t; work[k] = i < T ? tile_work[i] : -1; }
+    };
+    if (one_round) load_work(0);
     for (int i = t; i < ORDER_BINS; i += 1024) bins[i] = 0;
     if (t < HEAVY_CAP) n_heavy_out[GS_ORDER_REDO_OFFSET + t] = 0;
     __syncthreads();
     unsigned long long total = 0ull;
     for (int base = 0; base < T; base += 1024 * ORDER_PER) {
-        int work[ORDER_PER];
-#pragma unroll
-        for (int k = 0; k < ORDER_PER; ++k) { const int i = base + k * 1024 + t; work[k] = i < T ? tile_work[i] : -1; }
+        if (!one_round) load_work(base);
 #pragma unroll
         for (int k = 0; k < ORDER_PER; ++k) {
             if (base + k * 1024 + t >= T) continue;
@@ -114,23 +127,38 @@
         *n_heavy_out = sNHeavy;
     }
     __syncthreads();
+    const bool staged = T <= ORDER_STAGE;
     for (int base = 0; base < T; base += 1024 * ORDER_PER) {
-        int work[ORDER_PER];
-#pragma unroll
-        for (int k = 0; k < ORDER_PER; ++k) { const int i = base + k * 1024 + t; work[k] = i < T ? tile_work[i] : -1; }
+        if (!one_round) load_work(base);
 #pragma unroll
         for (int k = 0; k < ORDER_PER; ++k) {
             const int i = base + k * 1024 + t;
             if (i >= T) continue;
             int w = work[k] / ORDER_BIN_WIDTH; w = w < 0 ? 0 : (w > ORDER_BINS - 1 ? ORDER_BINS - 1 : w);
             const uint32_t pos = atomicAdd(&bins[ORDER_BINS - 1 - w], 1u);
-            order[pos] = i;
-            if (hint) hint[pos] = i;
+            if (staged) sOrder[pos] = i;
+            else { order[pos] = i; if (hint) hint[pos] = i; }
             if (pos < HEAVY_CAP) sHeavy[pos] = i;
         }
     }
     __syncthreads();
+    if (staged)
+        for (int i = t; i < T; i += 1024) { const int32_t v = sOrder[i]; order[i] = v; if (hint) hint[i] = v; }
+    if (hint && t == 0) {
+        int32_t* key = views.key(vslot < views.S ? vslot : 0);
+        if (keyed) {
+            key[0] = __float_as_int(-P0.q_cp[0]); key[1] = __float_as_int(-P0.q_cp[1]); key[2] = __float_as_int(-P0.q_cp[2]); key[3] = __float_as_int(P0.q_cp[3]);
+            key[4] = __float_as_int(P0.origin_bwd[0]); key[5] = __float_as_int(P0.origin_bwd[1]); key[6] = __float_as_int(P0.origin_bwd[2]);
+        }
+        if (vslot < views.S) key[7] = T;
+        views.base[1] = vslot + 1;
+        if (keyed && (uint32_t)views.base[0] % (uint32_t)views.S == (uint32_t)vslot) views.base[0] = (vslot + 1) % views.S;
+    }
     const int n_heavy = sNHeavy;
+    if (n_heavy == 0) {
+        if (t == 0) { n_heavy_out[4] = 0; n_heavy_out[1] = 0; }
+        return;
+    }
     int nseg = 0;
     if (t < n_heavy) {
         const int tile = sHeavy[t];
@@ -1146,7 +1174,7 @@
             fill.first_block = groups;
             fill.n_blocks = (unsigned)((bytes + GS_FILL_BLOCK_BYTES - 1) / GS_FILL_BLOCK_BYTES);
         }
-        GS_TIMED(a.prof, KID_TILE_ORDER, s, k_tile_order<<<1, 1024, 0, s>>>(v.tile_work, v.T, v.tile_order, a.order_hint, v.n_heavy, a.heavy_factor_x2,
+        GS_TIMED(a.prof, KID_TILE_ORDER, s, k_tile_order<<<1, 1024, 0, s>>>(v.tile_work, v.T, v.tile_order, a.views, a.view_slot, v.pose, v.n_heavy, a.heavy_factor_x2,
                                                                               v.tile_start, v.tile_end, v.cuts ? v.tile_cut : nullptr, v.cuts ? a.item_cap : gs_heavy_cap(v.T)));
 #define GS_BWD_LAUNCH_(NQ_, STRICT_, AUX_)                                                                                             \
         GS_TIMED(a.prof, KID_BLEND_BWD, s, k_blend_bwd_tile<NQ_, STRICT_, AUX_><<<groups + fill.n_blocks, 256, 0, s>>>(v.tile_order, v.n_heavy, v.T,      \
diff --git a/taichi_3d_gaussian_splatting_amd/csrc/k_blend_fwd.hip b/taichi_3d_gaussian_splatting_amd/csrc/k_blend_fwd.hip
--- a/taichi_3d_gaussian_splatting_amd/csrc/k_blend_fwd.hip
+++ b/taichi_3d_gaussian_splatting_amd/csrc/k_blend_fwd.hip
@@ -33,12 +33,14 @@
                                                    float* __restrict__ image, float* __restrict__ depth_out,
                                                    float* __restrict__ acc_alpha, int32_t* __restrict__ last_out,
                                                    int32_t* __restrict__ count_out, int32_t* __restrict__ tile_work,
-                                                   const int32_t* __restrict__ order_hint,
+                                                   const int32_t* __restrict__ view_orders, const int32_t* __restrict__ view_slot,
+                                                   int view_slot_bias, int view_slot_max,
                                                    float4* __restrict__ cuts, int32_t* __restrict__ tile_cut, int cut_cap)
 {
     __shared__ float4 sRec[4][64][3];
+    const int slot = view_orders ? *view_slot - view_slot_bias : -1;
     const uint32_t K = min(ctr->K, K_cap);
-    const int tile = order_hint ? order_hint[blockIdx.x] : (int)blockIdx.x;
+    const int tile = (slot >= 0 && slot <= view_slot_max) ? view_orders[(size_t)slot * gridDim.x + blockIdx.x] : (int)blockIdx.x;
     const int wave = __builtin_amdgcn_readfirstlane((int)(threadIdx.x >> 6)), lane = threadIdx.x & 63;
     const GsQuadPixel qp = gs_quad_pixel(tile, wave, lane, tiles_x, W, H);
     __shared__ int sRange[2];
@@ -169,7 +171,8 @@
     if (v.T <= 0) return;
     auto launch = [&](auto kernel) {
         GS_TIMED(a.prof, KID_BLEND_FWD, s, kernel<<<v.T, 256, 0, s>>>(v.tile_start, v.tile_end, v.keys_sorted, a.key_bytes, a.depth_bits - gs_key_dropped_bits(a.key_bytes), a.counters, a.K, v.vals_sorted, v.PA, v.PB, v.PC, a.W, a.H,
-                                                                   a.tiles_x, a.image, a.depth, a.acc_alpha, a.last, a.count, v.tile_work, a.order_hint, v.cuts, v.tile_cut, a.cut_cap));
+                                                                   a.tiles_x, a.image, a.depth, a.acc_alpha, a.last, a.count, v.tile_work, a.views.base ? a.views.order(0) : nullptr, a.view_slot, a.view_slot_bias, a.views.S,
+                                                                   v.cuts, v.tile_cut, a.cut_cap));
     };
     if (a.rgb_only) launch(k_blend_fwd<true>);
     else launch(k_blend_fwd<false>);
diff --git a/taichi_3d_gaussian_splatting_amd/csrc/k_project.hip b/taichi_3d_gaussian_splatting_amd/csrc/k_project.hip
--- a/taichi_3d_gaussian_splatting_amd/csrc/k_project.hip
+++ b/taichi_3d_gaussian_splatting_amd/csrc/k_project.hip
@@ -47,6 +47,54 @@
     uv[1] = v1 / pc[2];
 }
 
+__device__ __forceinline__ void gs_view_lookup(const GsViewTable& views, const float* __restrict__ q_pc, const float* __restrict__ t_pc, int lane,
+                                               int32_t* __restrict__ view_slots)
+{
+    const int S = views.S;
+    float k[7];
+#pragma unroll
+    for (int j = 0; j < 4; ++j) k[j] = q_pc[j];
+#pragma unroll
+    for (int j = 0; j < 3; ++j) k[4 + j] = t_pc[j];
+    const float t_scale = 1.0f / (1.0f + (k[4] * k[4] + k[5] * k[5] + k[6] * k[6]));
+    unsigned long long best = ~0ull;
+    int unfilled = S;
+    for (int slot = lane; slot < S; slot += 64) {
+        const int32_t* key = views.key(slot);
+        if (key[7] != views.T) { unfilled = unfilled < slot ? unfilled : slot; continue; }
+        bool same_bits = true;
+        float dp = 0.0f, dm = 0.0f, dt = 0.0f;
+#pragma unroll
+        for (int j = 0; j < 7; ++j) {
+            const float o = __int_as_float(key[j]);
+            same_bits = same_bits && key[j] == __float_as_int(k[j]);
+            if (j < 4) { dp += (k[j] - o) * (k[j] - o); dm += (k[j] + o) * (k[j] + o); }
+            else dt += (k[j] - o) * (k[j] - o);
+        }
+        float d = (dp < dm ? dp : dm) + dt * t_scale;
+        d = same_bits ? 0.0f : (d >= 0.0f && d < 3.0e38f ? d : 3.0e38f);
+        const unsigned long long cand = ((unsigned long long)(uint32_t)__float_as_int(d) << 32) | (unsigned long long)(uint32_t)slot;
+        best = cand < best ? cand : best;
+    }
+#pragma unroll
+    for (int o = 32; o > 0; o >>= 1) {
+        const unsigned long long ob = __shfl_xor(best, o, 64);
+        const int ou = __shfl_xor(unfilled, o, 64);
+        best = ob < best ? ob : best;
+        unfilled = ou < unfilled ? ou : unfilled;
+    }
+    if (lane != 0) return;
+    const bool found = best != ~0ull;
+    const int nearest = (int)(uint32_t)(best & 0xffffffffull);
+    const float d = __int_as_float((int)(uint32_t)(best >> 32));
+    int write;
+    if (found && d < GS_VIEW_SAME_D) write = nearest;
+    else if (unfilled < S) write = unfilled;
+    else write = (int)((uint32_t)views.base[0] % (uint32_t)S);
+    view_slots[GS_ORDER_READ_SLOT] = found ? nearest : -1;
+    view_slots[GS_ORDER_WRITE_SLOT] = write;
+}
+
 #define FILTER_POSE_CACHE 8
 __global__ __launch_bounds__(256) void k_filter(const float* __restrict__ pc, const int8_t* __restrict__ invalid,
                                                 const int32_t* __restrict__ obj, const float* __restrict__ Kmat,
@@ -54,7 +102,8 @@
                                                 GsPose* __restrict__ pose, GsCounters* __restrict__ counters,
                                                 int64_t N, int W, int H, float near_plane, float far_plane,
                                                 int8_t* __restrict__ mask, int32_t* __restrict__ block_counts,
-                                                int32_t* __restrict__ tile_arrays, int tile_ints)
+                                                int32_t* __restrict__ tile_arrays, int tile_ints,
+                                                GsViewTable views, int32_t* __restrict__ view_slots)
 {
     __shared__ int wave_cnt[4];
     __shared__ GsPose sp[FILTER_POSE_CACHE];
@@ -64,6 +113,7 @@
     if (cached && threadIdx.x < n_objects) sp[threadIdx.x] = make_pose(q_pc, t_pc, threadIdx.x);
     if (blockIdx.x == 0) {
         for (int o = threadIdx.x; o < n_objects; o += 256) pose[o] = make_pose(q_pc, t_pc, o);
+        if (views.base && threadIdx.x < 64) gs_view_lookup(views, q_pc, t_pc, threadIdx.x, view_slots);
     }
     __syncthreads();
     bool in = false;
@@ -318,7 +368,7 @@
     if (nb == 0) { (void)hipMemsetAsync(v.tile_start, 0, sizeof(int32_t) * (size_t)v.tile_ints, s); return; }
     GS_TIMED(a.prof, KID_FILTER, s, k_filter<<<nb, 256, 0, s>>>(a.point_cloud, a.invalid, a.object_id, a.Kmat, a.q_pc, a.t_pc, a.n_objects,
                                                             v.pose, a.counters, a.N, a.W, a.H, a.near_plane, a.far_plane, v.mask,
-                                                            a.block_counts, v.tile_start, v.tile_ints));
+                                                            a.block_counts, v.tile_start, v.tile_ints, a.views, v.n_heavy));
     GS_TIMED(a.prof, KID_PROJECT, s, k_project<<<nb, 256, 0, s>>>(a.point_cloud, a.features, a.object_id, a.Kmat, v.pose, v.mask, a.block_counts, a.N,
                                                               v.ids, v.cam_index, a.block_offsets, a.W, a.H,
                                                               a.depth_scale, v.PA, v.PB, v.PC, v.PD, v.box, v.ntiles,
```

After: 1695 frames/s (median of 6 runs). 2.2% higher.
